# usnistgov/thermoextrap

Hardware: AMD Instinct MI355X
Metric: samples/s for order-4 comoment bootstrap (N_samp x N_obs x nrep resample_vals) (higher is better)
Workload: dtype f64; 1 GPU; north: central-comoment bootstrap, N_samp=1e+08, N_obs=32, order=4, nrep=1000, exact multinomial device sampler; n_samp=100000000, n_obs=32, order=4, nrep=1000, parallelism=state-points x1

## Files before the change

include/txmom.h:

```cpp
#ifndef TXMOM_H
#define TXMOM_H

#include <stddef.h>
#include <stdint.h>

#ifdef __cplusplus
extern "C" {
#endif

#define TXM_ABI_VERSION 2
#define TXM_MAX_ORDER 8
#define TXM_SAMPLER_STREAM_VERSION 3

typedef enum txm_status {
  TXM_OK = 0,
  TXM_ERR_INVALID = -1,
  TXM_ERR_HIP = -2,
  TXM_ERR_WORKSPACE = -3,
  TXM_ERR_UNSUPPORTED = -4,
  TXM_ERR_NO_DEVICE = -5
} txm_status;

typedef void *txm_stream;

int txm_abi_version(void);
int txm_sampler_stream_version(void);
const char *txm_csrc_sha(void);
const char *txm_last_error(void);
int txm_init(int device);
int txm_device_count(int *count_host);
int txm_malloc(void **ptr_host, size_t bytes);
int txm_free(void *ptr);
int txm_memcpy_h2d(void *dst, const void *src_host, size_t bytes, txm_stream stream);
int txm_memcpy_d2h(void *dst_host, const void *src, size_t bytes, txm_stream stream);
int txm_memset(void *dst, int value, size_t bytes, txm_stream stream);
int txm_stream_sync(txm_stream stream);

size_t txm_reduce_vals_ws_bytes(int64_t N, int64_t C, int order);
int txm_reduce_vals(const double *x, int64_t ldx_s, int64_t ldx_c, const double *u,
                    const double *w, int64_t N, int64_t C, int order, double *out, void *ws,
                    size_t ws_bytes, txm_stream stream);

int txm_reduce_vals_pivot(const double *x, int64_t ldx_s, int64_t ldx_c, const double *u, int64_t N, int64_t C,
                          double *pivot, txm_stream stream);
int txm_reduce_vals_sums(const double *x, int64_t ldx_s, int64_t ldx_c, const double *u, const double *w,
                         int64_t N, int64_t C, int order, const double *pivot, double *sums, void *ws,
                         size_t ws_bytes, txm_stream stream);
int txm_sums_to_state(const double *sums, int64_t n, const double *pivot, int64_t C, int order, double *out,
                      txm_stream stream);
size_t txm_push_vals_ws_bytes(int64_t N, int64_t C, int order);
int txm_push_vals(double *state, const double *x, int64_t ldx_s, int64_t ldx_c, const double *u, const double *w,
                  int64_t N, int64_t C, int order, void *ws, size_t ws_bytes, txm_stream stream);

size_t txm_reduce_vals_1d_ws_bytes(int64_t N, int64_t R, int M);
int txm_reduce_vals_1d(const double *u, int64_t ldu_r, int64_t ldu_s, const double *w,
                       int64_t N, int64_t R, int M, double *out, void *ws, size_t ws_bytes,
                       txm_stream stream);

size_t txm_indices_to_freq_ws_bytes(void);
int txm_indices_to_freq(const int64_t *indices, int64_t nrep, int64_t nsamp, int64_t ndat,
                        int64_t *freq, void *ws, size_t ws_bytes, txm_stream stream);

typedef struct txm_sampler_spec {
  uint64_t seed;
  int64_t nrep;
  int64_t ndat;
  int64_t nsamp;
  int64_t rep0;
} txm_sampler_spec;

int64_t txm_sampler_ntiles(int64_t ndat);
size_t txm_sampler_counts_ws_bytes(const txm_sampler_spec *spec_host);
int txm_sampler_tile_counts(const txm_sampler_spec *spec_host, uint32_t *counts, void *ws,
                            size_t ws_bytes, txm_stream stream);
int txm_sampler_freq(const txm_sampler_spec *spec_host, const uint32_t *counts, int64_t *freq,
                     txm_stream stream);

size_t txm_sampler_count_table_bytes(int64_t ndat, int64_t nreps);
int txm_sampler_count_table(const txm_sampler_spec *spec_host, const uint32_t *counts, int64_t rep_begin,
                            int64_t nreps, uint8_t *table, txm_stream stream);

#define TXM_PATH_AUTO (-1)
#define TXM_PATH_FP64 0
#define TXM_PATH_INT8 1
#define TXM_PATH_INT8_FUSED 2
#define TXM_PATH_INT8_TABLE 3
typedef struct txm_resample_opts {
  int32_t path;
  int32_t prep_valid;
  void *prep;
  size_t prep_bytes;
  int64_t *info;
  const double *y;
  int64_t ldy_s;
  double *out_y;
} txm_resample_opts;
int txm_resample_path(int64_t N, int64_t C, int64_t nrep, int order);
#define TXM_KERNEL_WITH_Y 0x100
int txm_resample_kernel(int64_t N, int64_t C, int64_t nrep, int order, int path, int has_y, int aligned);
int txm_resample_operands_aligned(const double *x, int64_t ldx_s, int64_t C, const double *y, int64_t ldy_s);
int txm_set_resample_path(int path);
int txm_resample_vals_info(const void *ws, int64_t N, int64_t C, int64_t nrep, int order,
                           int64_t *info_host, txm_stream stream);
size_t txm_resample_prep_bytes(int64_t N, int64_t C, int64_t nrep, int order);
size_t txm_resample_vals_ws_bytes(int64_t N, int64_t C, int64_t nrep, int order);
size_t txm_resample_vals_ws_bytes_opts(int64_t N, int64_t C, int64_t nrep, int order, int path, int has_y);
size_t txm_resample_y_ws_bytes(int64_t N, int64_t C, int64_t nrep);
int txm_resample_i8_supported(int64_t N, int64_t C, int64_t nrep, int order);
int txm_resample_vals(const double *x, int64_t ldx_s, int64_t ldx_c, const double *u,
                      const double *w, int64_t N, int64_t C, int order, int64_t nrep,
                      const int64_t *freq, const txm_sampler_spec *spec_host,
                      const uint32_t *counts, const double *pivot, double *out,
                      const txm_resample_opts *opts_host, void *ws, size_t ws_bytes, txm_stream stream);

typedef struct txm_state_ptrs {
  const double *x;
  const double *u;
  const double *w;
} txm_state_ptrs;
size_t txm_reduce_vals_batched_ws_bytes(int64_t S, int64_t N, int64_t C, int order);
int txm_reduce_vals_batched(const txm_state_ptrs *states_host, int64_t S, int64_t ldx_s, int64_t N,
                            int64_t C, int order, double *out, void *ws, size_t ws_bytes,
                            txm_stream stream);
size_t txm_resample_vals_batched_ws_bytes(int64_t S, int64_t N, int64_t C, int64_t nrep, int order);
int txm_resample_vals_batched(const txm_state_ptrs *states_host, int64_t S, int64_t ldx_s, int64_t N,
                              int64_t C, int order, int64_t nrep, const int64_t *freq,
                              const txm_sampler_spec *spec_host, const uint32_t *counts, double *out,
                              void *ws, size_t ws_bytes, txm_stream stream);
size_t txm_resample_batched_prep_bytes(int64_t S, int64_t N, int64_t C, int64_t nrep, int order);
int txm_resample_batched_path(int64_t S, int64_t N, int64_t C, int64_t nrep, int order);
int txm_resample_vals_batched_opts(const txm_state_ptrs *states_host, int64_t S, int64_t ldx_s, int64_t N,
                                   int64_t C, int order, int64_t nrep, const int64_t *freq,
                                   const txm_sampler_spec *spec_host, const uint32_t *counts, double *out,
                                   const txm_resample_opts *opts_host, void *ws, size_t ws_bytes, txm_stream stream);

size_t txm_resample_data_ws_bytes(int64_t nrec, int64_t C, int order);
int txm_resample_data(const double *data, const int64_t *freq, int64_t nrec, int64_t C,
                      int64_t nrep, int order, double *out, void *ws, size_t ws_bytes,
                      txm_stream stream);

int txm_convert_cov(const double *in, double *out, int64_t n, int order, int to_central,
                    txm_stream stream);
int txm_convert_1d(const double *in, double *out, int64_t n, int M, int to_central,
                   txm_stream stream);

typedef struct txm_atom {
  int32_t src;
  int32_t pad;
  int64_t offset;
  int64_t s_rep;
  int64_t s_val;
} txm_atom;

#define TXM_FUNC_PLAIN 0
#define TXM_FUNC_MINUS_LOG 1

typedef struct txm_poly_table {
  int32_t n_funcs;
  int32_t n_atoms;
  int32_t n_terms;
  int32_t n_factors;
  int32_t log_atom;
  int32_t pad;
  const txm_atom *atoms;
  const int32_t *func_term0;
  const int32_t *func_flags;
  const double *coef;
  const int32_t *term_fac0;
  const int32_t *fac_atom;
  const int32_t *fac_pow;
} txm_poly_table;

int txm_eval_poly(const txm_poly_table *table_host, const double *const *srcs, int32_t n_srcs,
                  int64_t nrep, int64_t nval, double *out, txm_stream stream);

#define TXM_TAYLOR_SUM 0
#define TXM_TAYLOR_CUMSUM 1
#define TXM_TAYLOR_TERMS 2
int txm_predict_taylor(const double *derivs, int32_t n_ord, int64_t M, const double *dalpha,
                       int64_t n_alpha, int32_t mode, double *out, txm_stream stream);

int txm_cov_over_rep(const double *vals, int32_t n_ord, int64_t nrep, int64_t nval, double *cov,
                     txm_stream stream);

size_t txm_perturb_ws_bytes(int64_t N, int64_t C, int32_t n_alpha, int64_t nrep);
int txm_perturb(const double *x, int64_t ldx_s, const double *u, int64_t N, int64_t C,
                const double *dalpha_host, int32_t n_alpha, const int64_t *freq, int64_t nrep,
                double *out, void *ws, size_t ws_bytes, txm_stream stream);

typedef struct txm_mbar_state {
  const double *x;
  const double *u;
  int64_t n;
  int64_t ldx_s;
} txm_mbar_state;
size_t txm_mbar_ws_bytes(int32_t K, int64_t C, int32_t n_alpha);
int txm_mbar_eval(const txm_mbar_state *states_host, int32_t K, const double *alpha0_host,
                  const double *g_host, double upiv, double *out, double *logD, void *ws,
                  size_t ws_bytes, txm_stream stream);
int txm_mbar_predict(const txm_mbar_state *states_host, int32_t K, int64_t C, double upiv,
                     const double *logD, const double *alpha_host, int32_t n_alpha, double *out,
                     void *ws, size_t ws_bytes, txm_stream stream);

#ifdef __cplusplus
}
#endif
#endif
```

thermoextrap_amd/csrc/txm_resample.hip:

```cpp
#include <type_traits>

#include <stdlib.h>

#include "txm_sampler.h"
#include "txm_pivot.h"
#include "txm_resample_i8.h"
#include "txm_i8g.h"

namespace txm {

typedef double v4f64 __attribute__((ext_vector_type(4)));

constexpr int RS_BLOCK = 256;
constexpr int RS_WAVES = RS_BLOCK / 64;
constexpr int RS_REPS = 16;
constexpr int RS_QUARTER = SM_T / 4;
constexpr int RS_TILE_BYTES = SM_T * RS_REPS;
constexpr int rs_group(int K, int NBLK, bool weighted, bool explicit_, int pack = 1) {
  const int per_step = 2 + 2 * NBLK + (weighted ? 2 : 0) + (explicit_ ? 10 : 0);
  for (int g = 8; g > 2; g >>= 1)
#ifndef TXM_EXP_BUDGET
#define TXM_EXP_BUDGET 160
#endif
    if ((K + pack - 1) / pack * NBLK * 8 + 2 * g * per_step <= TXM_EXP_BUDGET) return g;
// ... 383 lines not shown
  if (colgrp == 0) {
    if constexpr (!WEIGHTED && !EXPLICIT) usum[0] = cnt;
#pragma unroll
    for (int j = 0; j < K; ++j) {
      double v = usum[j];
      v += __shfl_xor(v, 16);
      v += __shfl_xor(v, 32);
      if (kk == 0) PU[((size_t)chunk * a.nrep_pad + rep0 + row) * K + j] = v;
    }
  }
}

template <int K>
__global__ __launch_bounds__(256) void resample_finalize_kernel(
    const double *__restrict__ part_x, const double *__restrict__ part_u, int n_chunks,
    int64_t nrep_pad, int64_t C_pad, int64_t nrep, int64_t C, const double *__restrict__ pivot,
    double *__restrict__ out, int64_t c_off = 0, int64_t C_total = 0) {
  constexpr int NSEG = 8, NOUT = 256 / NSEG;
  __shared__ double sh[NSEG][NOUT][2 * K];
  const int eo = threadIdx.x % NOUT, seg = threadIdx.x / NOUT;
  const int64_t e = (int64_t)blockIdx.x * NOUT + eo;
  const bool live = e < nrep * C;
  const int64_t r = live ? e / C : 0, c = live ? e % C : 0;
  if (C_total == 0) C_total = C;
  const int64_t sidx = blockIdx.y;
  part_x += (size_t)sidx * n_chunks * nrep_pad * C_pad * K;
  part_u += (size_t)sidx * n_chunks * nrep_pad * K;
  pivot += sidx * (1 + C);
  out += (size_t)sidx * nrep * C_total * 2 * K;
  double S0[K], S1[K];
#pragma unroll
  for (int j = 0; j < K; ++j) S0[j] = S1[j] = 0.0;
  if (live)
    for (int ch = seg; ch < n_chunks; ch += NSEG) {
      const double *pu_ = part_u + ((size_t)ch * nrep_pad + r) * K;
      const double *px_ = part_x + (((size_t)ch * nrep_pad + r) * C_pad + c) * K;
#pragma unroll
      for (int j = 0; j < K; ++j) {
        S0[j] += pu_[j];
        S1[j] += px_[j];
      }
    }
#pragma unroll
  for (int j = 0; j < K; ++j) {
    sh[seg][eo][j] = S0[j];
    sh[seg][eo][K + j] = S1[j];
  }
  __syncthreads();
  if (seg != 0 || !live) return;
  for (int g = 1; g < NSEG; ++g)
#pragma unroll
    for (int j = 0; j < K; ++j) {
      S0[j] += sh[g][eo][j];
      S1[j] += sh[g][eo][K + j];
    }
  double st[2 * K];
  pivot_sums_to_state<K>(S0, S1, pivot[0], pivot[1 + c_off + c], st);
  double *o = out + (r * C_total + c_off + c) * 2 * K;
#pragma unroll
  for (int q = 0; q < 2 * K; ++q) o[q] = st[q];
}

template <int K, int CPAD>
__global__ __launch_bounds__(256) void resample_finalize_i8_kernel(
    const double *__restrict__ part_x, const double *__restrict__ part_u, int64_t nwin,
    const uint32_t *__restrict__ wflag, int64_t nrep_pad, int64_t nrep, int64_t C,
    const double *__restrict__ pivot, double *__restrict__ out, int64_t c_off, int64_t C_total,
    const double *__restrict__ fb_x, const double *__restrict__ fb_u, int fb_chunks, int64_t fb_cpad,
    const uint32_t *__restrict__ n_list, const I8State *__restrict__ states = nullptr, const int summed = 0) {
  if (states != nullptr) {
    const I8State e = states[blockIdx.y];
    part_x = e.part_x; part_u = e.part_u; wflag = e.wflag; pivot = e.pivot; out = e.out;
    fb_x = e.fb_x; fb_u = e.fb_u; n_list = e.n_list;
  }
  constexpr int cpad = CPAD;
  __shared__ double sh[256][2 * K];
  constexpr int nseg = 256 / cpad;
  const int64_t r = blockIdx.x;
  const int c = threadIdx.x % cpad, seg = threadIdx.x / cpad;
  double S0[K], S1[K];
#pragma unroll
  for (int j = 0; j < K; ++j) S0[j] = S1[j] = 0.0;
  if (c < C) {
    for (int64_t w = seg; w < nwin; w += nseg) {
      if (wflag[w] != 0u) continue;
      if (summed) {
        const double *px_ = part_x + ((size_t)w * nrep_pad + r) * K * cpad + c;
        if (summed == 1) {
          const double *pu_ = part_u + ((size_t)w * nrep_pad + r) * K;
#pragma unroll
          for (int j = 0; j < K; ++j) {
            S0[j] += pu_[j];
            S1[j] += px_[j * cpad];
          }
        } else {
          const double *pu_ = part_u + ((size_t)w * nrep_pad + r) * K * 8;
#pragma unroll
          for (int j = 0; j < K; ++j) {
            const double4 ua = *reinterpret_cast<const double4 *>(pu_ + j * 8), ub = *reinterpret_cast<const double4 *>(pu_ + j * 8 + 4);
            S0[j] += ((((((ua.x + ua.y) + ua.z) + ua.w) + ub.x) + ub.y) + ub.z);
            S1[j] += px_[j * cpad];
          }
        }
        continue;
      }
      const double *pu_ = part_u + ((size_t)w * nrep_pad + r) * K * 8;
      const double *px_ = part_x + ((size_t)w * nrep_pad + r) * K * 8 * cpad + c;
#pragma unroll
      for (int j = 0; j < K; ++j) {
        const double4 ua = *reinterpret_cast<const double4 *>(pu_ + j * 8), ub = *reinterpret_cast<const double4 *>(pu_ + j * 8 + 4);
        const double *q = px_ + (size_t)j * 8 * cpad;
        S0[j] += ((((((ua.x + ua.y) + ua.z) + ua.w) + ub.x) + ub.y) + ub.z);
        S1[j] += ((((((q[0] + q[cpad]) + q[2 * cpad]) + q[3 * cpad]) + q[4 * cpad]) + q[5 * cpad]) + q[6 * cpad]);
      }
    }
  }
#pragma unroll
  for (int j = 0; j < K; ++j) {
    sh[threadIdx.x][j] = S0[j];
    sh[threadIdx.x][K + j] = S1[j];
  }
  __syncthreads();
  if (seg != 0 || c >= C) return;
  for (int g = 1; g < nseg; ++g)
#pragma unroll
    for (int j = 0; j < K; ++j) {
      S0[j] += sh[g * cpad + c][j];
      S1[j] += sh[g * cpad + c][K + j];
    }
  if (n_list[0] != 0u)
    for (int ch = 0; ch < fb_chunks; ++ch) {
      const double *pu_ = fb_u + ((size_t)ch * nrep_pad + r) * K;
      const double *px_ = fb_x + (((size_t)ch * nrep_pad + r) * fb_cpad + c) * K;
#pragma unroll
      for (int j = 0; j < K; ++j) {
        S0[j] += pu_[j];
        S1[j] += px_[j];
      }
    }
  double st[2 * K];
  pivot_sums_to_state<K>(S0, S1, pivot[0], pivot[1 + c_off + c], st);
  double *o = out + (r * C_total + c_off + c) * 2 * K;
#pragma unroll
  for (int q = 0; q < 2 * K; ++q) o[q] = st[q];
  (void)nrep;
}

__global__ __launch_bounds__(256) void resample_finalize_y_kernel(
    const double *__restrict__ part_y, const double *__restrict__ part_u, int K, int64_t nwin,
    const uint32_t *__restrict__ wflag, int64_t nrep_pad, int64_t C, const double *__restrict__ ypivot,
    double *__restrict__ out_y, int64_t c_off, int64_t C_total, const double *__restrict__ fb_y,
    const double *__restrict__ fb_u, int fb_chunks, int64_t fb_cpad, const uint32_t *__restrict__ n_list) {
  constexpr int NSEG = 8;
  __shared__ double sh[NSEG][32][2];
  const int64_t r = blockIdx.x;
  const int c = threadIdx.x & 31, seg = threadIdx.x >> 5;
  double S0 = 0.0, S1 = 0.0;
  if (c < C) {
    for (int64_t w = seg; w < nwin; w += NSEG) {
      if (wflag[w] != 0u) continue;
      const double *pu_ = part_u + ((size_t)w * nrep_pad + r) * K * 8;
      const double *q = part_y + ((size_t)w * nrep_pad + r) * 8 * I8_CPAD + c;
      const double4 ua = *reinterpret_cast<const double4 *>(pu_), ub = *reinterpret_cast<const double4 *>(pu_ + 4);
      S0 += ((((((ua.x + ua.y) + ua.z) + ua.w) + ub.x) + ub.y) + ub.z);
      S1 += ((((((q[0] + q[I8_CPAD]) + q[2 * I8_CPAD]) + q[3 * I8_CPAD]) + q[4 * I8_CPAD]) + q[5 * I8_CPAD]) + q[6 * I8_CPAD]);
    }
  }
  sh[seg][c][0] = S0;
  sh[seg][c][1] = S1;
  __syncthreads();
  if (seg != 0 || c >= C) return;
  S0 = sh[0][c][0];
  S1 = sh[0][c][1];
  for (int g = 1; g < NSEG; ++g) {
    S0 += sh[g][c][0];
    S1 += sh[g][c][1];
  }
  if (n_list[0] != 0u)
    for (int ch = 0; ch < fb_chunks; ++ch) {
      S0 += fb_u[((size_t)ch * nrep_pad + r) * K];
      S1 += fb_y[((size_t)ch * nrep_pad + r) * fb_cpad + c];
    }
  out_y[r * C_total + c_off + c] = ypivot[1 + c_off + c] + S1 * (1.0 / S0);
}

struct ResamplePlan {
  int nblk, colgroups, n_rbg, n_chunks;
  int64_t tiles_per_chunk, nrep_pad, C_pad, ntiles;
  size_t off_pivot, off_px, off_pu, off_prog, prog_bytes, total;
};

static int64_t resample_chunk_tiles(int64_t ntiles, int64_t div) {
  int64_t nc = ntiles / div;
  if (nc > 1024) nc = 1024;
  if (nc < 8) nc = 8;
  if (nc > ntiles) nc = ntiles;
  nc = cdiv(nc, 8) * 8;
  return cdiv(ntiles, nc);
}

static ResamplePlan plan_resample(int64_t N, int64_t C, int64_t nrep, int K) {
  ResamplePlan p;
  p.nblk = C <= 16 ? 1 : 2;
  p.colgroups = (int)cdiv(C, p.nblk * 16);
  p.C_pad = (int64_t)p.colgroups * p.nblk * 16;
  p.n_rbg = (int)cdiv(nrep, RS_WAVES * RS_REPS);
  p.nrep_pad = (int64_t)p.n_rbg * RS_WAVES * RS_REPS;
  p.ntiles = cdiv(N, SM_T);
  p.tiles_per_chunk = resample_chunk_tiles(p.ntiles, 2);
  const int64_t nc = cdiv(cdiv(p.ntiles, p.tiles_per_chunk), 8) * 8;
  p.n_chunks = (int)nc;
  p.off_pivot = 0;
  p.off_px = align_up((size_t)(1 + C) * sizeof(double), 256);
  p.off_pu = p.off_px + align_up((size_t)p.n_chunks * p.nrep_pad * p.C_pad * K * sizeof(double), 256);
  p.off_prog = p.off_pu + align_up((size_t)p.n_chunks * p.nrep_pad * K * sizeof(double), 256);
  p.prog_bytes = (size_t)p.n_chunks * p.colgroups * 64 * sizeof(uint32_t);
  p.total = p.off_prog + align_up(p.prog_bytes, 256);
  return p;
}

struct I8Plan {
  int n_rbg, n_chunks, ngroups;
  int64_t tiles_per_chunk, nrep_pad, ntiles, nwin, win_tiles;
  size_t off_px, off_pu, total;
  int sub_tiles;
  size_t off_fbx, off_fbu, off_prog, prog_bytes, off_stats, off_prep;
  size_t off_table, table_bytes, off_gprog, total_table;
  size_t off_py, off_fby, prep_ypiv, prep_ywt, prep_yflag;
  size_t prep_wt, prep_flag, prep_list, prep_nlist, prep_group0, prep_group_stride, prep_total;
  ResamplePlan fb;
};

static I8Plan plan_i8(int64_t N, int64_t C, int64_t nrep, int K) {
  I8Plan p;
  p.n_rbg = (int)cdiv(nrep, I8_REPS);
  p.nrep_pad = (int64_t)p.n_rbg * I8_REPS;
  p.ntiles = cdiv(N, SM_T);
  p.ngroups = (int)cdiv(C, I8_CPAD);
  p.win_tiles = I8_WIN_TILES;
#ifndef TXM_WIN_MIN
#define TXM_WIN_MIN 256
#endif
  while (p.win_tiles > 4 && p.ntiles < TXM_WIN_MIN * p.win_tiles) p.win_tiles /= 4;
  p.nwin = cdiv(p.ntiles, p.win_tiles);
  int64_t nc = (int64_t)num_cus() / p.n_rbg / 8 * 8;
  if (nc < 8) nc = 8;
  if (nc > p.nwin) nc = cdiv(p.nwin, 8) * 8;
  p.tiles_per_chunk = cdiv(p.nwin, nc) * p.win_tiles;
  p.n_chunks = (int)(cdiv(cdiv(p.ntiles, p.tiles_per_chunk), 8) * 8);
  p.sub_tiles = p.win_tiles < I8_SUB_TILES ? (int)p.win_tiles : I8_SUB_TILES;
  p.prep_wt = 0;
  p.prep_flag = p.prep_wt + align_up((size_t)p.nwin * I8_WT_STRIDE * sizeof(double) + 2048, 256);
  p.prep_list = p.prep_flag + align_up((size_t)p.nwin * sizeof(uint32_t), 256);
  p.prep_nlist = p.prep_list + align_up((size_t)p.nwin * (size_t)(p.win_tiles / p.sub_tiles) * sizeof(uint32_t), 256);
  p.prep_ywt = p.prep_nlist + 256;
  p.prep_yflag = p.prep_ywt + align_up((size_t)p.nwin * I8_WT_STRIDE * sizeof(double), 256);
  p.prep_group_stride = p.prep_yflag + align_up((size_t)p.nwin * sizeof(uint32_t), 256);
  p.prep_ypiv = align_up((size_t)(1 + C) * sizeof(double), 256);
  p.prep_group0 = 2 * p.prep_ypiv;
  p.prep_total = p.prep_group0 + (size_t)p.ngroups * p.prep_group_stride;
  p.off_px = 0;
  p.off_pu = p.off_px + align_up((size_t)p.nwin * p.nrep_pad * K * I8_CPAD * 8 * sizeof(double), 256);
  p.fb = plan_resample(N, C < I8_CPAD ? C : I8_CPAD, nrep, K);
  p.off_fbx = p.off_pu + align_up((size_t)p.nwin * p.nrep_pad * K * 8 * sizeof(double), 256);
  p.off_fbu = p.off_fbx + align_up((size_t)p.fb.n_chunks * p.fb.nrep_pad * p.fb.C_pad * K * sizeof(double), 256);
  p.off_prog = p.off_fbu + align_up((size_t)p.fb.n_chunks * p.fb.nrep_pad * (K + 1) * sizeof(double), 256);
  p.prog_bytes = (size_t)p.n_chunks * 64 * sizeof(uint32_t);
  p.off_stats = p.off_prog + align_up(p.prog_bytes, 256);
  p.off_py = p.off_stats + align_up((size_t)cdiv(p.ntiles, p.win_tiles < 16 ? p.win_tiles : 16) * 100 * sizeof(double), 256);
  p.off_fby = p.off_py + align_up((size_t)p.nwin * p.nrep_pad * 8 * I8_CPAD * sizeof(double), 256);
  p.off_prep = p.off_fby + align_up((size_t)p.fb.n_chunks * p.fb.nrep_pad * p.fb.C_pad * sizeof(double), 256);
  p.off_gprog = p.off_prep + align_up(p.prep_total, 256);
  p.off_table = p.off_gprog + align_up((size_t)cdiv(p.nwin, 8) * 8 * 16 * sizeof(uint32_t), 256);
  p.table_bytes = (N >= SM_T && (C > 16 || K >= 2)) ? count_table_bytes(p.ntiles, nrep) : 0;
  p.total = p.off_table;
  p.total_table = p.off_table + align_up(p.table_bytes, 256);
  return p;
}

static int g_path_override = -1;
static int path_override() { return g_path_override; }

static constexpr bool throttle_on() {
#ifdef TXM_NO_THROTTLE
  return false;
#else
  return true;
#endif
}

static bool table_kernel_pays(int64_t nrep, int K, bool has_y) {
  const int64_t pad128 = cdiv(nrep, G_REPS) * G_REPS, pad64 = cdiv(nrep, I8_REPS) * I8_REPS;
  if (4 * pad128 > 5 * pad64) return false;
  if (has_y) return true;
  if (K == 4 || K == 5) return pad128 >= 2 * G_REPS;
  return true;
}

static bool narrow_table_pays(int64_t N, int64_t C, int64_t nrep, int K) {
  const int64_t pad128 = cdiv(nrep, G_REPS) * G_REPS, pad64 = cdiv(nrep, I8_REPS) * I8_REPS;
  if (N < 786432 || nrep <= I8_REPS || pad128 > pad64) return false;
  return !(i8t_narrow_nq(C, K) == 4 && K == 5);
}
static bool table_call_rule(size_t table_bytes, int eff, int64_t N, int64_t C, int64_t nrep, int K, bool has_y, bool applicable) {
  if (eff == TXM_PATH_FP64 || eff == TXM_PATH_INT8_FUSED || table_bytes == 0 || !applicable) return false;
  if (eff == TXM_PATH_INT8_TABLE) return true;
  return C > 16 ? table_kernel_pays(nrep, K, has_y) : narrow_table_pays(N, C, nrep, K);
}
static bool table_operands_ok(const double *x, int64_t ldx_s, int64_t C, int K, const double *y, int64_t ldy_s) {
  return C > 16 ? i8g_applicable(x, ldx_s, C, y, ldy_s) : i8gn_applicable(x, ldx_s, C, K);
}

static bool use_i8(int64_t N, int64_t C, int64_t nrep, int K, int call_path = TXM_PATH_AUTO) {
  if (!i8_supported(N, C, nrep, K)) return false;
  const int ov = call_path != TXM_PATH_AUTO ? call_path : path_override();
  if (ov == TXM_PATH_FP64) return false;
  if (ov == TXM_PATH_INT8 || ov == TXM_PATH_INT8_FUSED || ov == TXM_PATH_INT8_TABLE) return true;
  if (C <= 16) return K >= 2 && (N >= 786432 || (N >= 262144 && nrep >= 128));
  const int64_t ctail = C % I8_CPAD;
  const bool long_series = N >= 786432;
  const int64_t min_rep = long_series ? (K >= 2 ? 32 : 100) : (K >= 4 ? 64 : (K >= 2 ? 128 : 384));
  return C > 16 && (ctail == 0 || ctail > 16 || K >= 2) && nrep >= min_rep && N >= 262144;
}

}

using namespace txm;

extern "C" int txm_set_resample_path(int path) {
  TXM_REQUIRE(path == -1 || path == TXM_PATH_FP64 || path == TXM_PATH_INT8 || path == TXM_PATH_INT8_FUSED || path == TXM_PATH_INT8_TABLE, "set_resample_path: %d is not a path", path);
  g_path_override = path;
  return TXM_OK;
}

namespace txm {
__global__ void i8_info_kernel(const unsigned char *prep_groups, size_t group_stride, size_t off_nlist, int ngroups,
                               int64_t nwin, int from_prep, int64_t *info) {
  if (threadIdx.x == 0 && blockIdx.x == 0) {
    int64_t flagged = 0;
    for (int g = 0; g < ngroups; ++g)
      flagged += reinterpret_cast<const uint32_t *>(prep_groups + (size_t)g * group_stride + off_nlist)[1];
    info[0] = TXM_PATH_INT8;
    info[1] = nwin * ngroups;
    info[2] = flagged;
    info[3] = from_prep;
  }
}
__global__ void fp64_info_kernel(int64_t *info) {
  if (threadIdx.x == 0 && blockIdx.x == 0) {
    info[0] = TXM_PATH_FP64;
    info[1] = info[2] = info[3] = 0;
  }
}
}
using namespace txm;

extern "C" int txm_resample_vals_info(const void *ws, int64_t N, int64_t C, int64_t nrep, int order,
                                      int64_t *info_host, txm_stream stream) {
  TXM_REQUIRE(ws && info_host, "resample_vals_info: null pointer");
  TXM_REQUIRE(N >= 1 && C >= 1 && nrep >= 1 && order >= 0 && order <= TXM_MAX_ORDER, "resample_vals_info: bad shape");
  info_host[0] = TXM_PATH_FP64;
  info_host[1] = info_host[2] = 0;
  if (!use_i8(N, C, nrep, order + 1)) return TXM_OK;
  const I8Plan q = plan_i8(N, C, nrep, order + 1);
  int64_t flagged = 0;
  for (int g = 0; g < q.ngroups; ++g) {
    uint32_t nl[2] = {0, 0};
    TXM_HIP(hipMemcpyAsync(nl, (const char *)ws + q.off_prep + q.prep_group0 + (size_t)g * q.prep_group_stride + q.prep_nlist,
                           sizeof(nl), hipMemcpyDeviceToHost, (hipStream_t)stream));
    TXM_HIP(hipStreamSynchronize((hipStream_t)stream));
    flagged += nl[1];
  }
  info_host[0] = TXM_PATH_INT8;
  info_host[1] = q.nwin * q.ngroups;
  info_host[2] = flagged;
  return TXM_OK;
}

extern "C" int txm_resample_path(int64_t N, int64_t C, int64_t nrep, int order) {
  if (N < 1 || C < 1 || nrep < 1 || order < 0 || order > TXM_MAX_ORDER) return TXM_PATH_FP64;
  return use_i8(N, C, nrep, order + 1) ? TXM_PATH_INT8 : TXM_PATH_FP64;
}

extern "C" int txm_resample_kernel(int64_t N, int64_t C, int64_t nrep, int order, int path, int has_y, int aligned) {
  if (N < 1 || C < 1 || nrep < 1 || order < 0 || order > TXM_MAX_ORDER) return TXM_PATH_FP64;
  const int K = order + 1;
  if (!use_i8(N, C, nrep, K, path)) return TXM_PATH_FP64;
  const I8Plan q = plan_i8(N, C, nrep, K);
  const int eff = path != TXM_PATH_AUTO ? path : path_override();
  const bool table = table_call_rule(q.table_bytes, eff, N, C, nrep, K, has_y != 0, aligned != 0);
  const bool with_y = has_y != 0 && ((table && C > 16) || i8t_carries_y(C, K));
  return (table ? TXM_PATH_INT8_TABLE : TXM_PATH_INT8_FUSED) | (with_y ? TXM_KERNEL_WITH_Y : 0);
}

extern "C" int txm_resample_operands_aligned(const double *x, int64_t ldx_s, int64_t C, const double *y, int64_t ldy_s) {
  if (x == nullptr || C < 1) return 0;
  return table_operands_ok(x, ldx_s, C, 2, y, ldy_s) ? 1 : 0;
}

extern "C" size_t txm_resample_prep_bytes(int64_t N, int64_t C, int64_t nrep, int order) {
  if (N < 1 || C < 1 || nrep < 1 || order < 0 || order > TXM_MAX_ORDER) return 0;
  if (!i8_supported(N, C, nrep, order + 1)) return 256;
  return plan_i8(N, C, nrep, order + 1).prep_total;
}

static size_t y_main_bytes(int64_t N, int64_t C, int64_t nrep) {
  size_t n = plan_resample(N, C, nrep, 1).total;
  if (i8_supported(N, C, nrep, 1)) {
    const size_t m = plan_i8(N, C, nrep, 1).total;
    if (m > n) n = m;
  }
  return align_up(n, 256);
}
static size_t y_extra_bytes(int64_t N, int64_t C, int64_t nrep) {
  return align_up((size_t)nrep * C * 2 * sizeof(double), 256) + y_main_bytes(N, C, nrep);
}

extern "C" size_t txm_resample_vals_ws_bytes_opts(int64_t N, int64_t C, int64_t nrep, int order, int path, int has_y) {
  if (N < 1 || C < 1 || nrep < 1 || order < 0 || order > TXM_MAX_ORDER) return 0;
  size_t n = plan_resample(N, C, nrep, order + 1).total;
  if (i8_supported(N, C, nrep, order + 1)) {
    const I8Plan q = plan_i8(N, C, nrep, order + 1);
    const int eff = path != TXM_PATH_AUTO ? path : path_override();
    const bool table = table_call_rule(q.table_bytes, eff, N, C, nrep, order + 1, has_y != 0, true);
    const size_t m = table ? q.total_table : q.total;
    if (m > n) n = m;
  }
  return align_up(n, 256);
}

extern "C" size_t txm_resample_vals_ws_bytes(int64_t N, int64_t C, int64_t nrep, int order) {
  return txm_resample_vals_ws_bytes_opts(N, C, nrep, order, TXM_PATH_AUTO, 0);
}

extern "C" size_t txm_resample_y_ws_bytes(int64_t N, int64_t C, int64_t nrep) {
  if (N < 1 || C < 1 || nrep < 1) return 0;
  return y_extra_bytes(N, C, nrep);
}

extern "C" int txm_resample_i8_supported(int64_t N, int64_t C, int64_t nrep, int order) {
  if (N < 1 || C < 1 || nrep < 1 || order < 0 || order > TXM_MAX_ORDER) return 0;
  return i8_supported(N, C, nrep, order + 1) ? 1 : 0;
}

#define TXM_K_SWITCH(K_, CALL)                          \
  switch (K_) {                                         \
    case 1: { constexpr int KK = 1; CALL; } break;      \
    case 2: { constexpr int KK = 2; CALL; } break;      \
    case 3: { constexpr int KK = 3; CALL; } break;      \
    case 4: { constexpr int KK = 4; CALL; } break;      \
    case 5: { constexpr int KK = 5; CALL; } break;      \
    case 6: { constexpr int KK = 6; CALL; } break;      \
    case 7: { constexpr int KK = 7; CALL; } break;      \
    case 8: { constexpr int KK = 8; CALL; } break;      \
    case 9: { constexpr int KK = 9; CALL; } break;      \
    default: set_error("order out of range"); return TXM_ERR_INVALID; \
  }

namespace txm {
static constexpr bool pack_on() {
#ifdef TXM_NO_PACK
  return false;
#else
  return true;
#endif
}
template <int K>
static int run_resample(ResampleArgs a, const ResamplePlan &p, bool weighted, bool explicit_,
                        double *out, hipStream_t st, int64_t S = 1) {
  dim3 grid((unsigned)(p.n_chunks * p.n_rbg), (unsigned)p.colgroups, (unsigned)S), block(RS_BLOCK);
  const size_t lds = explicit_ ? 0 : (size_t)RS_WAVES * RS_TILE_BYTES;
#define TXM_RS_LAUNCH(NB, WT, EX)                                                                       \
  do {                                                                                                 \
    if (S > 1 || a.batch != nullptr) {                                                                 \
      if (a.N < SM_T)                                                                                  \
        hipLaunchKernelGGL((resample_kernel<K, NB, WT, EX, true, RS_BATCHED>), grid, block, lds, st, a);  \
      else                                                                                             \
        hipLaunchKernelGGL((resample_kernel<K, NB, WT, EX, false, RS_BATCHED>), grid, block, lds, st, a); \
    } else if (a.N < SM_T)                                                                             \
      hipLaunchKernelGGL((resample_kernel<K, NB, WT, EX, true>), grid, block, lds, st, a);             \
    else                                                                                               \
      hipLaunchKernelGGL((resample_kernel<K, NB, WT, EX, false>), grid, block, lds, st, a);            \
  } while (0)
  bool packed = false;
  if constexpr (K >= 2 && K <= 6) {
    if (p.nblk == 1 && p.colgroups == 1 && !explicit_ && a.N >= SM_T && a.C <= 8 && pack_on()) {
      packed = true;
      const bool bat = S > 1 || a.batch != nullptr;
#define TXM_RS_PACKED(PK)                                                                                      \
  do {                                                                                                         \
    if (bat) {                                                                                                 \
      if (weighted) hipLaunchKernelGGL((resample_kernel<K, 1, true, false, false, RS_BATCHED, PK>), grid, block, lds, st, a); \
      else hipLaunchKernelGGL((resample_kernel<K, 1, false, false, false, RS_BATCHED, PK>), grid, block, lds, st, a);         \
    } else {                                                                                                   \
      if (weighted) hipLaunchKernelGGL((resample_kernel<K, 1, true, false, false, RS_PLAIN, PK>), grid, block, lds, st, a);   \
      else hipLaunchKernelGGL((resample_kernel<K, 1, false, false, false, RS_PLAIN, PK>), grid, block, lds, st, a);           \
    }                                                                                                          \
  } while (0)
      if (a.C <= 4 && K >= 3) TXM_RS_PACKED(4);
      else TXM_RS_PACKED(2);
#undef TXM_RS_PACKED
    }
  }
  if (packed) {
  } else if (p.nblk == 1) {
    if (weighted) { if (explicit_) TXM_RS_LAUNCH(1, true, true); else TXM_RS_LAUNCH(1, true, false); }
    else          { if (explicit_) TXM_RS_LAUNCH(1, false, true); else TXM_RS_LAUNCH(1, false, false); }
  } else {
    if (weighted) { if (explicit_) TXM_RS_LAUNCH(2, true, true); else TXM_RS_LAUNCH(2, true, false); }
    else          { if (explicit_) TXM_RS_LAUNCH(2, false, true); else TXM_RS_LAUNCH(2, false, false); }
  }
#undef TXM_RS_LAUNCH
  TXM_LAUNCH_CHECK();
  const int64_t ne = a.nrep * a.C;
  hipLaunchKernelGGL((resample_finalize_kernel<K>), dim3((unsigned)cdiv(ne, 32), (unsigned)S), dim3(256), 0, st,
                     a.part_x, a.part_u, p.n_chunks, p.nrep_pad, p.C_pad, a.nrep, a.C, a.pivot, out);
  TXM_LAUNCH_CHECK();
  return TXM_OK;
}

template <int K>
static int run_listed_k(const ResampleArgs &a, const ResamplePlan &p, bool weighted, hipStream_t st, int64_t S = 1) {
  dim3 grid((unsigned)(p.n_chunks * p.n_rbg), (unsigned)p.colgroups, (unsigned)S), block(RS_BLOCK);
  const size_t lds = (size_t)RS_WAVES * RS_TILE_BYTES;
  if (p.nblk == 1) {
    if (weighted) hipLaunchKernelGGL((resample_kernel<K, 1, true, false, false, RS_LISTED>), grid, block, lds, st, a);
    else hipLaunchKernelGGL((resample_kernel<K, 1, false, false, false, RS_LISTED>), grid, block, lds, st, a);
  } else {
    if (weighted) hipLaunchKernelGGL((resample_kernel<K, 2, true, false, false, RS_LISTED>), grid, block, lds, st, a);
    else hipLaunchKernelGGL((resample_kernel<K, 2, false, false, false, RS_LISTED>), grid, block, lds, st, a);
  }
  TXM_LAUNCH_CHECK();
  return TXM_OK;
}

static int run_listed(const ResampleArgs &a, const ResamplePlan &p0, int K, bool weighted, hipStream_t st, int64_t S = 1) {
  ResamplePlan p = p0;
  if (a.C <= 16) p.nblk = 1;
  p.colgroups = 1;
  TXM_K_SWITCH(K, return run_listed_k<KK>(a, p, weighted, st, S));
  return TXM_OK;
}
}

namespace txm {
__global__ void y_means_kernel(const double *__restrict__ st , int64_t n, double *__restrict__ out) {
  const int64_t e = (int64_t)blockIdx.x * blockDim.x + threadIdx.x;
  if (e < n) out[e] = st[2 * e + 1];
}

static int resample_vals_impl(const double *x, int64_t ldx_s, const double *u, const double *w, int64_t N, int64_t C,
                              int order, int64_t nrep, const int64_t *freq, const txm_sampler_spec *spec,
                              const uint32_t *counts, const double *pivot, double *out, int path, void *prep,
                              size_t prep_bytes, bool prep_valid, int64_t *info, void *ws, size_t ws_bytes,
                              hipStream_t st, const double *y = nullptr, int64_t ldy_s = 0, double *out_y = nullptr,
                              bool *y_done = nullptr) {
  const bool explicit_ = freq != nullptr;
  const int K = order + 1;
  if (y_done) *y_done = false;
  if (!explicit_ && use_i8(N, C, nrep, K, path)) {
    const I8Plan q = plan_i8(N, C, nrep, K);
    const int eff_path = path != TXM_PATH_AUTO ? path : path_override();
    const bool table_call = ws_bytes >= q.total_table &&
                            table_call_rule(q.table_bytes, eff_path, N, C, nrep, K, y != nullptr, table_operands_ok(x, ldx_s, C, K, y, ldy_s));
    const bool with_y = y != nullptr && ((table_call && C > 16) || i8t_carries_y(C, K));
    if (ws_bytes < q.total) {
      set_error("resample_vals: workspace too small (%zu < %zu)", ws_bytes, q.total);
      return TXM_ERR_WORKSPACE;
    }
    TXM_REQUIRE(spec->ndat == N && spec->nrep == nrep, "resample_vals: sampler spec does not match N/nrep");
    TXM_REQUIRE(spec->rep0 >= 0 && spec->rep0 + nrep <= ((int64_t)1 << 32), "resample_vals: sampler rep0 out of range");
    unsigned char *pb = (unsigned char *)ws + q.off_prep;
    bool have_tables = false;
    if (prep != nullptr) {
      if (prep_bytes < q.prep_total) {
        set_error("resample_vals: prep buffer too small (%zu < %zu)", prep_bytes, q.prep_total);
        return TXM_ERR_WORKSPACE;
      }
      pb = (unsigned char *)prep;
      have_tables = prep_valid;
    }
    double *piv = (double *)pb;
    double *ypiv = (double *)(pb + q.prep_ypiv);
    if (!have_tables) {
      if (pivot) {
        TXM_HIP(hipMemcpyAsync(piv, pivot, sizeof(double) * (size_t)(1 + C), hipMemcpyDeviceToDevice, st));
      } else {
        hipLaunchKernelGGL(pivot_kernel, dim3((unsigned)(1 + C)), dim3(256), 0, st, x, ldx_s, (int64_t)1,
                           u, (int64_t)1, N, piv);
        TXM_LAUNCH_CHECK();
      }
      if (with_y) {
        hipLaunchKernelGGL(pivot_kernel, dim3((unsigned)(1 + C)), dim3(256), 0, st, y, ldy_s, (int64_t)1, u, (int64_t)1,
                           N, ypiv);
        TXM_LAUNCH_CHECK();
        TXM_HIP(hipMemcpyAsync(ypiv, piv, sizeof(double), hipMemcpyDeviceToDevice, st));
      }
    }
    I8Args b;
    b.x = x; b.ldx_s = ldx_s; b.u = u; b.w = w; b.N = N; b.nrep = nrep; b.C_call = C;
    b.cpad = i8_cpad(C, K);
    b.counts = counts;
    b.k0 = (uint32_t)spec->seed;
    b.k1 = (uint32_t)(spec->seed >> 32);
    b.rep_base = (uint32_t)spec->rep0;
    b.ntiles = q.ntiles;
    b.last_tile_size = (uint32_t)(N - (q.ntiles - 1) * SM_T);
    b.pivot = piv;
    b.stats = (double *)((char *)ws + q.off_stats);
    b.nwin = q.nwin;
    b.part_x = (double *)((char *)ws + q.off_px);
    b.part_u = (double *)((char *)ws + q.off_pu);
    b.n_chunks = q.n_chunks; b.n_rbg = q.n_rbg; b.tiles_per_chunk = q.tiles_per_chunk;
    b.nrep_pad = q.nrep_pad;
    b.win_tiles = q.win_tiles;
    b.sub_tiles = q.sub_tiles;
    b.y = with_y ? y : nullptr;
    b.ldy_s = ldy_s;
    b.ypivot = ypiv;
    b.part_y = (double *)((char *)ws + q.off_py);
    b.part_summed = i8t_wide_summed(with_y) ? 1 : 0;
    b.progress = (throttle_on() && q.n_rbg > 1) ? (uint32_t *)((char *)ws + q.off_prog) : nullptr;
    ResampleArgs f;
    f.ldx_s = ldx_s; f.u = u; f.w = w; f.N = N; f.nrep = nrep;
    f.freq = nullptr; f.counts = counts;
    f.k0 = b.k0; f.k1 = b.k1; f.rep_base = b.rep_base;
    f.ntiles = q.ntiles; f.last_tile_size = b.last_tile_size;
    f.pivot = piv;
    f.part_x = (double *)((char *)ws + q.off_fbx);
    f.part_u = (double *)((char *)ws + q.off_fbu);
    f.n_chunks = q.fb.n_chunks; f.n_rbg = q.fb.n_rbg; f.tiles_per_chunk = q.fb.tiles_per_chunk;
    f.nrep_pad = q.fb.nrep_pad; f.C_pad = q.fb.C_pad;
    f.sub_tiles = q.sub_tiles; f.batch = nullptr; f.progress = nullptr;
    TXM_REQUIRE(q.fb.nrep_pad == q.nrep_pad, "resample_vals: replicate padding of the two kernels differs");
    int g = 0;
    bool have_table = false;
    for (int64_t col0 = 0; col0 < C; col0 += I8_CPAD, ++g) {
      unsigned char *pg = pb + q.prep_group0 + (size_t)g * q.prep_group_stride;
      b.wtab = (double *)(pg + q.prep_wt);
      b.wflag = (uint32_t *)(pg + q.prep_flag);
      b.list = (uint32_t *)(pg + q.prep_list);
      b.n_list = (uint32_t *)(pg + q.prep_nlist);
      b.ywtab = (double *)(pg + q.prep_ywt);
      b.yflag = (uint32_t *)(pg + q.prep_yflag);
      f.list = b.list; f.n_list = b.n_list;
      b.col0 = col0;
      b.C = C - col0 < I8_CPAD ? C - col0 : I8_CPAD;
      const bool narrow_tail = C > I8_CPAD && b.C <= 16 && K >= 2 && !with_y;
      b.C_call = narrow_tail ? b.C : C;
      b.cpad = i8_cpad(b.C_call, K);
      if (!have_tables) {
        const int rc0 = launch_i8_prepass(b, K, st);
        if (rc0 != TXM_OK) return rc0;
      }
      const bool table_kernel = table_call && !narrow_tail;
      int rc;
      if (table_kernel) {
        unsigned char *table = (unsigned char *)ws + q.off_table;
        if (!have_table) {
          rc = launch_count_table(counts, nrep, N, b.k0, b.k1, b.rep_base, 0, cdiv(nrep, G_REPS), table, st);
          if (rc != TXM_OK) return rc;
          have_table = true;
        }
        I8Args bg = b;
        bg.progress = (throttle_on() && nrep > G_REPS) ? (uint32_t *)((char *)ws + q.off_gprog) : nullptr;
        rc = C > 16 ? launch_resample_i8g(bg, K, w != nullptr, table, 0, (int)cdiv(nrep, G_REPS), st)
                    : launch_resample_i8gn(bg, K, w != nullptr, table, 0, (int)cdiv(nrep, G_REPS), 0, st);
      } else {
        rc = launch_resample_i8(b, K, w != nullptr, q.prog_bytes, st);
      }
      if (rc != TXM_OK) return rc;
      f.x = x + col0; f.C = b.C; f.col_off = col0;
      {
        const int rc2 = run_listed(f, q.fb, K, w != nullptr, st);
        if (rc2 != TXM_OK) return rc2;
      }
      const int fin_summed = table_kernel ? (C <= 16 ? 1 : 2)
                                          : (i8t_narrow_nq(b.C_call, K) != 0 ? (i8t_partials_summed(b.C_call, K) ? 1 : 0) : b.part_summed);
#define TXM_I8_FIN2(KK, CP)                                                                            \
  hipLaunchKernelGGL((resample_finalize_i8_kernel<KK, CP>), dim3((unsigned)nrep), dim3(256), 0, st,      \
                     b.part_x, b.part_u, q.nwin, b.wflag, q.nrep_pad, nrep, b.C, piv, out, col0, C,        \
                     f.part_x, f.part_u, q.fb.n_chunks, q.fb.C_pad, b.n_list, (const I8State *)nullptr, fin_summed)
#define TXM_I8_FIN(KK)                                                                                 \
  do {                                                                                                 \
    if (b.cpad == 32) TXM_I8_FIN2(KK, 32);                                                             \
    else if (b.cpad == 16) TXM_I8_FIN2(KK, 16);                                                        \
    else if (b.cpad == 8) TXM_I8_FIN2(KK, 8);                                                          \
    else TXM_I8_FIN2(KK, 4);                                                                           \
  } while (0)
      switch (K) {
        case 1: TXM_I8_FIN(1); break;
        case 2: TXM_I8_FIN(2); break;
        case 3: TXM_I8_FIN(3); break;
        case 4: TXM_I8_FIN(4); break;
        case 5: TXM_I8_FIN(5); break;
        case 6: TXM_I8_FIN(6); break;
        case 7: TXM_I8_FIN(7); break;
        default: TXM_I8_FIN(8); break;
      }
#undef TXM_I8_FIN
      TXM_LAUNCH_CHECK();
      if (with_y) {
        ResampleArgs fy = f;
        fy.x = y + col0; fy.ldx_s = ldy_s; fy.pivot = ypiv;
        fy.part_x = (double *)((char *)ws + q.off_fby);
        fy.part_u = f.part_u + (size_t)q.fb.n_chunks * q.fb.nrep_pad * K;
        const int rc3 = run_listed(fy, q.fb, 1, w != nullptr, st);
        if (rc3 != TXM_OK) return rc3;
        hipLaunchKernelGGL(resample_finalize_y_kernel, dim3((unsigned)nrep), dim3(256), 0, st, b.part_y, b.part_u, K, q.nwin,
                           b.wflag, q.nrep_pad, b.C, ypiv, out_y, col0, C, fy.part_x, f.part_u, q.fb.n_chunks, q.fb.C_pad,
                           b.n_list);
        TXM_LAUNCH_CHECK();
      }
    }
    if (with_y && y_done) *y_done = true;
    if (prep != nullptr)
      TXM_HIP(hipMemcpyAsync((char *)ws + q.off_prep, pb, q.prep_total, hipMemcpyDeviceToDevice, st));
    if (info != nullptr) {
      hipLaunchKernelGGL(i8_info_kernel, dim3(1), dim3(64), 0, st, pb + q.prep_group0, q.prep_group_stride, q.prep_nlist,
                         q.ngroups, q.nwin, (have_tables ? 1 : 0) | (have_table ? 2 : 0), info);
      TXM_LAUNCH_CHECK();
    }
    return TXM_OK;
  }
  if (info != nullptr) {
    hipLaunchKernelGGL(fp64_info_kernel, dim3(1), dim3(64), 0, st, info);
    TXM_LAUNCH_CHECK();
  }
  const ResamplePlan p = plan_resample(N, C, nrep, K);
  if (ws_bytes < p.total) {
    set_error("resample_vals: workspace too small (%zu < %zu)", ws_bytes, p.total);
    return TXM_ERR_WORKSPACE;
  }
  TXM_REQUIRE((int64_t)p.n_chunks * p.n_rbg < ((int64_t)1 << 31), "resample_vals: grid too large");
  double *piv = (double *)((char *)ws + p.off_pivot);
  if (pivot) {
    TXM_HIP(hipMemcpyAsync(piv, pivot, sizeof(double) * (size_t)(1 + C), hipMemcpyDeviceToDevice, st));
  } else {
    hipLaunchKernelGGL(pivot_kernel, dim3((unsigned)(1 + C)), dim3(256), 0, st, x, ldx_s, (int64_t)1,
                       u, (int64_t)1, N, piv);
    TXM_LAUNCH_CHECK();
  }
  ResampleArgs a;
  a.x = x; a.ldx_s = ldx_s; a.u = u; a.w = w; a.N = N; a.C = C; a.nrep = nrep;
  a.freq = freq; a.counts = counts;
  a.k0 = a.k1 = 0;
  a.rep_base = 0;
  a.ntiles = p.ntiles;
  a.last_tile_size = (uint32_t)(N - (p.ntiles - 1) * SM_T);
  if (!explicit_) {
    TXM_REQUIRE(spec->ndat == N && spec->nrep == nrep, "resample_vals: sampler spec does not match N/nrep");
    TXM_REQUIRE(spec->rep0 >= 0 && spec->rep0 + nrep <= ((int64_t)1 << 32), "resample_vals: sampler rep0 out of range");
    a.k0 = (uint32_t)spec->seed;
    a.k1 = (uint32_t)(spec->seed >> 32);
    a.rep_base = (uint32_t)spec->rep0;
  }
  a.pivot = piv;
  a.part_x = (double *)((char *)ws + p.off_px);
  a.part_u = (double *)((char *)ws + p.off_pu);
  a.n_chunks = p.n_chunks; a.n_rbg = p.n_rbg; a.tiles_per_chunk = p.tiles_per_chunk;
  a.nrep_pad = p.nrep_pad; a.C_pad = p.C_pad;
  a.list = nullptr; a.n_list = nullptr; a.sub_tiles = 0; a.col_off = 0; a.batch = nullptr;
  a.progress = nullptr;
  if (throttle_on() && p.n_rbg > 1 && a.N >= SM_T) {
    a.progress = (uint32_t *)((char *)ws + p.off_prog);
    TXM_HIP(hipMemsetAsync(a.progress, 0, p.prog_bytes, st));
  }
  TXM_K_SWITCH(K, return run_resample<KK>(a, p, w != nullptr, explicit_, out, st));
  return TXM_OK;
}
}

extern "C" int txm_resample_vals(const double *x, int64_t ldx_s, int64_t ldx_c, const double *u,
                                 const double *w, int64_t N, int64_t C, int order, int64_t nrep,
                                 const int64_t *freq, const txm_sampler_spec *spec,
                                 const uint32_t *counts, const double *pivot, double *out,
                                 const txm_resample_opts *opts, void *ws, size_t ws_bytes, txm_stream stream) {
  TXM_REQUIRE(x && u && out && ws, "resample_vals: null pointer");
  TXM_REQUIRE(N >= 1 && C >= 1 && nrep >= 1, "resample_vals: need N, C, nrep >= 1");
  TXM_REQUIRE(order >= 0 && order <= TXM_MAX_ORDER, "resample_vals: order %d outside [0, %d]", order,
              TXM_MAX_ORDER);
  TXM_REQUIRE(ldx_c == 1 && ldx_s >= C, "resample_vals: x must be (rec, val) row-major (ldx_c == 1)");
  const bool explicit_ = freq != nullptr;
  TXM_REQUIRE(explicit_ != (spec != nullptr && counts != nullptr),
              "resample_vals: give either freq or (spec, counts)");
  txm_resample_opts o;
  o.path = TXM_PATH_AUTO; o.prep_valid = 0; o.prep = nullptr; o.prep_bytes = 0; o.info = nullptr;
  o.y = nullptr; o.ldy_s = 0; o.out_y = nullptr;
  if (opts) o = *opts;
  TXM_REQUIRE(o.path == TXM_PATH_AUTO || o.path == TXM_PATH_FP64 || o.path == TXM_PATH_INT8 || o.path == TXM_PATH_INT8_FUSED || o.path == TXM_PATH_INT8_TABLE,
              "resample_vals: opts.path %d is not a path", (int)o.path);
  TXM_REQUIRE((o.y == nullptr) == (o.out_y == nullptr), "resample_vals: opts.y and opts.out_y go together");
  TXM_REQUIRE(o.y == nullptr || o.ldy_s >= C, "resample_vals: opts.ldy_s < C");
  hipStream_t st = (hipStream_t)stream;
  const size_t main_bytes = txm_resample_vals_ws_bytes_opts(N, C, nrep, order, o.path, o.y != nullptr);
  const size_t avail = ws_bytes < main_bytes ? ws_bytes : main_bytes;
  bool y_done = false;
  int rc = resample_vals_impl(x, ldx_s, u, w, N, C, order, nrep, freq, spec, counts, pivot, out, o.path, o.prep,
                              o.prep_bytes, o.prep_valid != 0, o.info, ws, avail, st, o.y, o.ldy_s, o.out_y, &y_done);
  if (rc != TXM_OK || o.y == nullptr || y_done) return rc;
  if (ws_bytes < main_bytes + y_extra_bytes(N, C, nrep)) {
    set_error("resample_vals: workspace too small for opts.y (%zu < %zu)", ws_bytes, main_bytes + y_extra_bytes(N, C, nrep));
    return TXM_ERR_WORKSPACE;
  }
  double *ystates = (double *)((char *)ws + main_bytes);
  void *yws = (char *)ws + main_bytes + align_up((size_t)nrep * C * 2 * sizeof(double), 256);
  rc = resample_vals_impl(o.y, o.ldy_s, u, w, N, C, 0, nrep, freq, spec, counts, nullptr, ystates, o.path, nullptr, 0,
                          false, nullptr, yws, y_main_bytes(N, C, nrep), st);
  if (rc != TXM_OK) return rc;
  hipLaunchKernelGGL(y_means_kernel, dim3((unsigned)cdiv(nrep * C, 256)), dim3(256), 0, st, ystates, nrep * C, o.out_y);
  TXM_LAUNCH_CHECK();
  return TXM_OK;
}

namespace txm {
struct BatchPlan {
  ResamplePlan one;
  size_t off_tab, off_pivot, off_px, off_pu, total;
};
static BatchPlan plan_batched(int64_t S, int64_t N, int64_t C, int64_t nrep, int K) {
  BatchPlan b;
  ResamplePlan &p = b.one;
  p = plan_resample(N, C, nrep, K);
  (void)S;
  p.tiles_per_chunk = resample_chunk_tiles(p.ntiles, 8);
  p.n_chunks = (int)(cdiv(cdiv(p.ntiles, p.tiles_per_chunk), 8) * 8);
  b.off_tab = 0;
  b.off_pivot = align_up((size_t)S * sizeof(txm_state_ptrs), 256);
  b.off_px = b.off_pivot + align_up((size_t)S * (1 + C) * sizeof(double), 256);
  b.off_pu = b.off_px + align_up((size_t)S * p.n_chunks * p.nrep_pad * p.C_pad * K * sizeof(double), 256);
  b.total = b.off_pu + align_up((size_t)S * p.n_chunks * p.nrep_pad * K * sizeof(double), 256);
  return b;
}
}

namespace txm {
struct I8StateLayout {
  size_t stride, s_px, s_pu, s_fbx, s_fbu, s_stats;
  size_t p_stride, p_wt, p_flag, p_list, p_nlist;
};
struct BatchI8Plan {
  I8Plan q;
  int cpad, n_chunks;
  int64_t tiles_per_chunk;
  I8StateLayout L;
  size_t off_tab, off_states, off_bargs, off_state0, off_prep, total;
  size_t prep_piv, prep_state0, prep_total;
};
static BatchI8Plan plan_batched_i8(int64_t S, int64_t N, int64_t C, int64_t nrep, int K) {
  BatchI8Plan b;
  b.q = plan_i8(N, C, nrep, K);
  const I8Plan &q = b.q;
  b.cpad = i8_cpad(C, K);
  int64_t nc = (int64_t)num_cus() / ((int64_t)q.n_rbg * S) / 8 * 8;
  if (nc < 8) nc = 8;
  if (nc > q.nwin) nc = cdiv(q.nwin, 8) * 8;
  b.tiles_per_chunk = cdiv(q.nwin, nc) * q.win_tiles;
  b.n_chunks = (int)(cdiv(cdiv(q.ntiles, b.tiles_per_chunk), 8) * 8);
  I8StateLayout &L = b.L;
  L.s_px = 0;
  L.s_pu = L.s_px + align_up((size_t)q.nwin * q.nrep_pad * K * 8 * b.cpad * sizeof(double), 256);
  L.s_fbx = L.s_pu + align_up((size_t)q.nwin * q.nrep_pad * K * 8 * sizeof(double), 256);
  L.s_fbu = L.s_fbx + align_up((size_t)q.fb.n_chunks * q.fb.nrep_pad * q.fb.C_pad * K * sizeof(double), 256);
  L.s_stats = L.s_fbu + align_up((size_t)q.fb.n_chunks * q.fb.nrep_pad * (K + 1) * sizeof(double), 256);
  L.stride = L.s_stats + align_up((size_t)cdiv(q.ntiles, q.win_tiles < 16 ? q.win_tiles : 16) * 100 * sizeof(double), 256);
  L.p_wt = 0;
  L.p_flag = L.p_wt + align_up((size_t)q.nwin * I8_WT_STRIDE * sizeof(double) + 2048, 256);
  L.p_list = L.p_flag + align_up((size_t)q.nwin * sizeof(uint32_t), 256);
  L.p_nlist = L.p_list + align_up((size_t)q.nwin * (size_t)(q.win_tiles / q.sub_tiles) * sizeof(uint32_t), 256);
  L.p_stride = L.p_nlist + 256;
  b.prep_piv = 0;
  b.prep_state0 = align_up((size_t)S * (1 + C) * sizeof(double), 256);
  b.prep_total = b.prep_state0 + (size_t)S * L.p_stride;
  b.off_tab = 0;
  b.off_states = align_up((size_t)S * sizeof(txm_state_ptrs), 256);
  b.off_bargs = b.off_states + align_up((size_t)S * sizeof(I8State), 256);
  b.off_state0 = b.off_bargs + align_up((size_t)S * sizeof(I8Args), 256);
  b.off_prep = b.off_state0 + (size_t)S * L.stride;
  b.total = b.off_prep + align_up(b.prep_total, 256);
  return b;
}

static bool use_i8_batched(int64_t S, int64_t N, int64_t C, int64_t nrep, int K, int call_path = TXM_PATH_AUTO) {
  if (!i8_supported(N, C, nrep, K) || i8t_narrow_nq(C, K) == 0) return false;
  const int ov = call_path != TXM_PATH_AUTO ? call_path : path_override();
  if (ov == TXM_PATH_FP64) return false;
  if (ov == TXM_PATH_INT8 || ov == TXM_PATH_INT8_FUSED || ov == TXM_PATH_INT8_TABLE) return true;
  (void)S;
  return K >= 2 && (N >= 786432 || (N >= 262144 && nrep >= 128));
}

__global__ void i8_states_kernel(const txm_state_ptrs *__restrict__ tab, int64_t S, unsigned char *base, unsigned char *pbase,
                                 I8StateLayout L, const double *piv, int64_t C, const uint32_t *counts, int64_t nrep, int64_t ntiles,
                                 double *out, int K, uint32_t rep_base, I8State *__restrict__ states) {
  const int64_t s = (int64_t)blockIdx.x * blockDim.x + threadIdx.x;
  if (s >= S) return;
  unsigned char *b = base + (size_t)s * L.stride, *pb = pbase + (size_t)s * L.p_stride;
  I8State e;
  e.x = tab[s].x; e.u = tab[s].u; e.w = tab[s].w;
  e.pivot = piv + s * (1 + C);
  e.stats = (double *)(b + L.s_stats);
  e.wtab = (double *)(pb + L.p_wt);
  e.wflag = (uint32_t *)(pb + L.p_flag);
  e.list = (uint32_t *)(pb + L.p_list);
  e.n_list = (uint32_t *)(pb + L.p_nlist);
  e.part_x = (double *)(b + L.s_px);
  e.part_u = (double *)(b + L.s_pu);
  e.fb_x = (double *)(b + L.s_fbx);
  e.fb_u = (double *)(b + L.s_fbu);
  e.counts = counts + (size_t)s * nrep * ntiles;
  e.out = out + (size_t)s * nrep * C * 2 * K;
  e.rep_base = rep_base + (uint32_t)(s * nrep);
  e.pad_ = 0;
  states[s] = e;
}

__global__ void i8_batch_args_kernel(const I8Args base, int64_t S, I8Args *__restrict__ out) {
  const int64_t s = (int64_t)blockIdx.x * blockDim.x + threadIdx.x;
  if (s >= S) return;
  const I8State e = base.states[s];
  I8Args r = base;
  r.x = e.x; r.u = e.u; r.w = e.w; r.pivot = e.pivot; r.wtab = e.wtab; r.wflag = e.wflag;
  r.part_x = e.part_x; r.part_u = e.part_u; r.counts = e.counts; r.rep_base = e.rep_base;
  out[s] = r;
}

static int resample_batched_i8(const txm_state_ptrs *states_host, int64_t S, int64_t ldx_s, int64_t N, int64_t C, int K,
                               int64_t nrep, bool weighted, const txm_sampler_spec *spec, const uint32_t *counts, double *out,
                               void *prep, size_t prep_bytes, bool prep_valid, int64_t *info, void *ws, size_t ws_bytes,
                               hipStream_t st) {
  const BatchI8Plan b = plan_batched_i8(S, N, C, nrep, K);
  const I8Plan &q = b.q;
  if (ws_bytes < b.total) {
    set_error("resample_vals_batched: workspace too small (%zu < %zu)", ws_bytes, b.total);
    return TXM_ERR_WORKSPACE;
  }
  TXM_REQUIRE(spec->ndat == N && spec->nrep == S * nrep, "resample_vals_batched: the sampler must span S * nrep replicates of N samples");
  TXM_REQUIRE(spec->rep0 >= 0 && spec->rep0 + spec->nrep <= ((int64_t)1 << 32), "resample_vals_batched: sampler replicates outside [0, 2^32)");
  TXM_REQUIRE((int64_t)b.n_chunks * q.n_rbg < ((int64_t)1 << 31) && S <= 65535, "resample_vals_batched: grid too large");
  txm_state_ptrs *tab = (txm_state_ptrs *)((char *)ws + b.off_tab);
  TXM_HIP(hipMemcpyAsync(tab, states_host, (size_t)S * sizeof(txm_state_ptrs), hipMemcpyHostToDevice, st));
  unsigned char *pb = (unsigned char *)ws + b.off_prep;
  bool have_tables = false;
  if (prep != nullptr) {
    if (prep_bytes < b.prep_total) {
      set_error("resample_vals_batched: prep buffer too small (%zu < %zu)", prep_bytes, b.prep_total);
      return TXM_ERR_WORKSPACE;
    }
    pb = (unsigned char *)prep;
    have_tables = prep_valid;
  }
  double *piv = (double *)(pb + b.prep_piv);
  if (!have_tables) {
    hipLaunchKernelGGL(pivot_batch_kernel, dim3((unsigned)(1 + C), (unsigned)S), dim3(256), 0, st, tab, ldx_s, N, C, piv);
    TXM_LAUNCH_CHECK();
  }
  I8State *states = (I8State *)((char *)ws + b.off_states);
  hipLaunchKernelGGL(i8_states_kernel, dim3((unsigned)cdiv(S, 64)), dim3(64), 0, st, tab, S, (unsigned char *)ws + b.off_state0,
                     pb + b.prep_state0, b.L, piv, C, counts, nrep, q.ntiles, out, K, (uint32_t)spec->rep0, states);
  TXM_LAUNCH_CHECK();
  bool vec_ok = ldx_s % 2 == 0;
  for (int64_t s = 0; s < S; ++s) vec_ok = vec_ok && (reinterpret_cast<uintptr_t>(states_host[s].x) & 15) == 0;
  I8Args a;
  a.states = states;
  a.S = S;
  a.x = vec_ok ? states_host[0].x : reinterpret_cast<const double *>((uintptr_t)8);
  a.ldx_s = ldx_s; a.u = states_host[0].u; a.w = states_host[0].w; a.N = N; a.C = C; a.nrep = nrep;
  a.col0 = 0; a.C_call = C;
  a.part_summed = 1;
  a.counts = counts;
  a.k0 = (uint32_t)spec->seed;
  a.k1 = (uint32_t)(spec->seed >> 32);
  a.rep_base = (uint32_t)spec->rep0;
  a.ntiles = q.ntiles;
  a.last_tile_size = (uint32_t)(N - (q.ntiles - 1) * SM_T);
  a.pivot = piv; a.wtab = nullptr; a.stats = nullptr; a.nwin = q.nwin;
  a.part_x = nullptr; a.cpad = b.cpad; a.part_u = nullptr;
  a.y = nullptr; a.ldy_s = 0; a.ypivot = nullptr; a.ywtab = nullptr; a.yflag = nullptr; a.part_y = nullptr;
  a.n_chunks = b.n_chunks; a.n_rbg = q.n_rbg; a.tiles_per_chunk = b.tiles_per_chunk; a.win_tiles = q.win_tiles;
  a.nrep_pad = q.nrep_pad;
  a.wflag = nullptr; a.list = nullptr; a.n_list = nullptr; a.sub_tiles = q.sub_tiles;
  a.progress = nullptr;
  I8Args *bargs = (I8Args *)((char *)ws + b.off_bargs);
  hipLaunchKernelGGL(i8_batch_args_kernel, dim3((unsigned)cdiv(S, 64)), dim3(64), 0, st, a, S, bargs);
  TXM_LAUNCH_CHECK();
  a.batch_args = bargs;
  int rc = have_tables ? TXM_OK : launch_i8_prepass(a, K, st);
  if (rc != TXM_OK) return rc;
  rc = launch_resample_i8t(a, K, weighted, 0, st);
  if (rc != TXM_OK) return rc;
  ResampleArgs f;
  f.x = states_host[0].x; f.ldx_s = ldx_s; f.u = states_host[0].u; f.w = states_host[0].w; f.N = N; f.C = C; f.nrep = nrep;
  f.freq = nullptr; f.counts = counts;
  f.k0 = a.k0; f.k1 = a.k1; f.rep_base = a.rep_base;
  f.ntiles = q.ntiles; f.last_tile_size = a.last_tile_size;
  f.pivot = piv; f.part_x = nullptr; f.part_u = nullptr;
  f.n_chunks = q.fb.n_chunks; f.n_rbg = q.fb.n_rbg; f.tiles_per_chunk = q.fb.tiles_per_chunk;
  f.nrep_pad = q.fb.nrep_pad; f.C_pad = q.fb.C_pad;
  f.list = nullptr; f.n_list = nullptr; f.sub_tiles = q.sub_tiles; f.col_off = 0; f.batch = nullptr; f.progress = nullptr;
  f.i8states = states;
  TXM_REQUIRE(q.fb.nrep_pad == q.nrep_pad, "resample_vals_batched: replicate padding of the two kernels differs");
  rc = run_listed(f, q.fb, K, weighted, st, S);
  if (rc != TXM_OK) return rc;
  const int bfin_summed = i8t_partials_summed(C, K) ? 1 : 0;
#define TXM_I8_BFIN2(KK, CP)                                                                                        \
  hipLaunchKernelGGL((resample_finalize_i8_kernel<KK, CP>), dim3((unsigned)nrep, (unsigned)S), dim3(256), 0, st, nullptr, \
                     nullptr, q.nwin, nullptr, q.nrep_pad, nrep, C, nullptr, nullptr, (int64_t)0, C, nullptr, nullptr,      \
                     q.fb.n_chunks, q.fb.C_pad, nullptr, states, bfin_summed)
#define TXM_I8_BFIN(KK)                                  \
  do {                                                   \
    if (b.cpad == 16) TXM_I8_BFIN2(KK, 16);              \
    else if (b.cpad == 8) TXM_I8_BFIN2(KK, 8);           \
    else TXM_I8_BFIN2(KK, 4);                            \
  } while (0)
  switch (K) {
    case 2: TXM_I8_BFIN(2); break;
    case 3: TXM_I8_BFIN(3); break;
    case 4: TXM_I8_BFIN(4); break;
    case 5: TXM_I8_BFIN(5); break;
    case 6: TXM_I8_BFIN(6); break;
    case 7: TXM_I8_BFIN(7); break;
    default: TXM_I8_BFIN(8); break;
  }
#undef TXM_I8_BFIN
#undef TXM_I8_BFIN2
  TXM_LAUNCH_CHECK();
  if (info != nullptr) {
    hipLaunchKernelGGL(i8_info_kernel, dim3(1), dim3(64), 0, st, pb + b.prep_state0, b.L.p_stride, b.L.p_nlist, (int)S, q.nwin,
                       have_tables ? 1 : 0, info);
    TXM_LAUNCH_CHECK();
  }
  return TXM_OK;
}
}

extern "C" size_t txm_resample_vals_batched_ws_bytes(int64_t S, int64_t N, int64_t C, int64_t nrep, int order) {
  if (S < 1 || N < 1 || C < 1 || nrep < 1 || order < 0 || order > TXM_MAX_ORDER) return 0;
  const size_t f = plan_batched(S, N, C, nrep, order + 1).total;
  if (!i8_supported(N, C, nrep, order + 1) || i8t_narrow_nq(C, order + 1) == 0) return f;
  const size_t i = plan_batched_i8(S, N, C, nrep, order + 1).total;
  return i > f ? i : f;
}

extern "C" int txm_resample_batched_path(int64_t S, int64_t N, int64_t C, int64_t nrep, int order) {
  if (S < 1 || N < 1 || C < 1 || nrep < 1 || order < 0 || order > TXM_MAX_ORDER) return TXM_PATH_FP64;
  return use_i8_batched(S, N, C, nrep, order + 1) ? TXM_PATH_INT8 : TXM_PATH_FP64;
}

extern "C" size_t txm_resample_batched_prep_bytes(int64_t S, int64_t N, int64_t C, int64_t nrep, int order) {
  if (S < 1 || N < 1 || C < 1 || nrep < 1 || order < 0 || order > TXM_MAX_ORDER) return 0;
  if (!i8_supported(N, C, nrep, order + 1) || i8t_narrow_nq(C, order + 1) == 0) return 0;
  return plan_batched_i8(S, N, C, nrep, order + 1).prep_total;
}

extern "C" int txm_resample_vals_batched(const txm_state_ptrs *states_host, int64_t S, int64_t ldx_s, int64_t N,
                                         int64_t C, int order, int64_t nrep, const int64_t *freq,
                                         const txm_sampler_spec *spec, const uint32_t *counts, double *out,
                                         void *ws, size_t ws_bytes, txm_stream stream) {
  return txm_resample_vals_batched_opts(states_host, S, ldx_s, N, C, order, nrep, freq, spec, counts, out, nullptr, ws, ws_bytes,
                                        stream);
}

extern "C" int txm_resample_vals_batched_opts(const txm_state_ptrs *states_host, int64_t S, int64_t ldx_s, int64_t N,
                                              int64_t C, int order, int64_t nrep, const int64_t *freq,
                                              const txm_sampler_spec *spec, const uint32_t *counts, double *out,
                                              const txm_resample_opts *opts, void *ws, size_t ws_bytes, txm_stream stream) {
  const int call_path = opts ? opts->path : TXM_PATH_AUTO;
  TXM_REQUIRE(call_path == TXM_PATH_AUTO || call_path == TXM_PATH_FP64 || call_path == TXM_PATH_INT8 || call_path == TXM_PATH_INT8_FUSED || call_path == TXM_PATH_INT8_TABLE,
              "resample_vals_batched: opts.path %d is not a path", call_path);
  TXM_REQUIRE(!(opts && (opts->y || opts->out_y)), "resample_vals_batched: no second sample matrix on the batched entry");
  TXM_REQUIRE(states_host && out && ws, "resample_vals_batched: null pointer");
  TXM_REQUIRE(S >= 1 && S <= 65535 && N >= 1 && C >= 1 && nrep >= 1, "resample_vals_batched: need S, N, C, nrep >= 1");
  TXM_REQUIRE(order >= 0 && order <= TXM_MAX_ORDER, "resample_vals_batched: order %d outside [0, %d]", order, TXM_MAX_ORDER);
  TXM_REQUIRE(ldx_s >= C, "resample_vals_batched: row pitch ldx_s < C");
  const bool explicit_ = freq != nullptr;
  TXM_REQUIRE(explicit_ != (spec != nullptr && counts != nullptr), "resample_vals_batched: give either freq or (spec, counts)");
  const bool weighted = states_host[0].w != nullptr;
  for (int64_t s = 0; s < S; ++s) {
    TXM_REQUIRE(states_host[s].x && states_host[s].u, "resample_vals_batched: state %lld has a null pointer", (long long)s);
    TXM_REQUIRE((states_host[s].w != nullptr) == weighted, "resample_vals_batched: weights for all states or for none");
  }
  const int K = order + 1;
  if (!explicit_ && use_i8_batched(S, N, C, nrep, K, call_path))
    return resample_batched_i8(states_host, S, ldx_s, N, C, K, nrep, weighted, spec, counts, out, opts ? opts->prep : nullptr,
                               opts ? opts->prep_bytes : 0, opts && opts->prep_valid != 0, opts ? opts->info : nullptr, ws, ws_bytes,
                               (hipStream_t)stream);
  if (opts && opts->info != nullptr) {
    hipLaunchKernelGGL(fp64_info_kernel, dim3(1), dim3(64), 0, (hipStream_t)stream, opts->info);
    TXM_LAUNCH_CHECK();
  }
  const BatchPlan b = plan_batched(S, N, C, nrep, K);
  if (ws_bytes < b.total) {
    set_error("resample_vals_batched: workspace too small (%zu < %zu)", ws_bytes, b.total);
    return TXM_ERR_WORKSPACE;
  }
  hipStream_t st = (hipStream_t)stream;
  txm_state_ptrs *tab = (txm_state_ptrs *)((char *)ws + b.off_tab);
  TXM_HIP(hipMemcpyAsync(tab, states_host, (size_t)S * sizeof(txm_state_ptrs), hipMemcpyHostToDevice, st));
  double *piv = (double *)((char *)ws + b.off_pivot);
  hipLaunchKernelGGL(pivot_batch_kernel, dim3((unsigned)(1 + C), (unsigned)S), dim3(256), 0, st, tab, ldx_s, N, C, piv);
  TXM_LAUNCH_CHECK();
  const ResamplePlan &p = b.one;
  ResampleArgs a;
  a.x = nullptr; a.ldx_s = ldx_s; a.u = nullptr; a.w = nullptr; a.N = N; a.C = C; a.nrep = nrep;
  a.freq = freq; a.counts = counts;
  a.k0 = a.k1 = 0;
  a.rep_base = 0;
  a.ntiles = p.ntiles;
  a.last_tile_size = (uint32_t)(N - (p.ntiles - 1) * SM_T);
  if (!explicit_) {
    TXM_REQUIRE(spec->ndat == N && spec->nrep == S * nrep, "resample_vals_batched: the sampler must span S * nrep replicates of N samples");
    TXM_REQUIRE(spec->rep0 >= 0 && spec->rep0 + spec->nrep <= ((int64_t)1 << 32), "resample_vals_batched: sampler replicates outside [0, 2^32)");
    a.k0 = (uint32_t)spec->seed;
    a.k1 = (uint32_t)(spec->seed >> 32);
    a.rep_base = (uint32_t)spec->rep0;
  }
  a.pivot = piv;
  a.part_x = (double *)((char *)ws + b.off_px);
  a.part_u = (double *)((char *)ws + b.off_pu);
  a.n_chunks = p.n_chunks; a.n_rbg = p.n_rbg; a.tiles_per_chunk = p.tiles_per_chunk;
  a.nrep_pad = p.nrep_pad; a.C_pad = p.C_pad;
  a.list = nullptr; a.n_list = nullptr; a.sub_tiles = 0; a.col_off = 0;
  a.batch = tab;
  a.progress = nullptr;
  TXM_K_SWITCH(K, return run_resample<KK>(a, p, weighted, explicit_, out, st, S));
  return TXM_OK;
}
```

thermoextrap_amd/csrc/txm_resample_i8.h:

```cpp
#pragma once
#include "txm_common.h"

namespace txm {

constexpr int I8_REPS = 64;
constexpr int I8_NSL = 7;
constexpr int I8_WIN_TILES = 256;
constexpr int I8_CPAD = 32;
constexpr int I8_WT_STRIDE = 80;
constexpr int I8_SUB_TILES = 8;

constexpr double I8_GUARD = 275.0;

constexpr int I8_WT_INVDU = 0, I8_WT_INVW = 1, I8_WT_DSP = 2, I8_WT_SC = 12, I8_WT_DSC = 44;

struct I8State {
  const double *x, *u, *w;
  const double *pivot;
  double *stats;
  double *wtab;
  uint32_t *wflag;
  uint32_t *list, *n_list;
  double *part_x, *part_u;
  double *fb_x, *fb_u;
  const uint32_t *counts;
  double *out;
  uint32_t rep_base;
  uint32_t pad_;
};

struct I8Args;
struct I8Args {
  const I8State *states = nullptr;
  const I8Args *batch_args = nullptr;
  int64_t S = 1;
  const double *x;
  int64_t ldx_s;
  const double *u;
  const double *w;
  int64_t N, C, nrep;
  int64_t col0;
  int64_t C_call;
  const uint32_t *counts;
  uint32_t k0, k1;
  uint32_t rep_base;
  int64_t ntiles;
  uint32_t last_tile_size;
  const double *pivot;
  double *wtab;
  double *stats;
  int64_t nwin;
  double *part_x;
  int cpad;
  double *part_u;
  int part_summed;
  const double *y;
  int64_t ldy_s;
  const double *ypivot;
  double *ywtab;
  uint32_t *yflag;
  double *part_y;
  int n_chunks, n_rbg;
  int64_t tiles_per_chunk;
  int64_t win_tiles;
  int64_t nrep_pad;
  uint32_t *wflag;
  uint32_t *list;
  uint32_t *n_list;
  int sub_tiles;
  uint32_t *progress;
};
#ifndef TXM_I8_LEAD
#define TXM_I8_LEAD 2
#endif
constexpr uint32_t I8_LEAD = TXM_I8_LEAD;
constexpr int I8_THROTTLE_SPINS = 48;

bool i8_supported(int64_t N, int64_t C, int64_t nrep, int K);
int launch_i8_prepass(const I8Args &a, int K, hipStream_t st);
int launch_resample_i8(const I8Args &a, int K, bool weighted, size_t prog_bytes, hipStream_t st);
int launch_resample_i8t(const I8Args &a, int K, bool weighted, size_t prog_bytes, hipStream_t st);
bool i8t_carries_y(int64_t C, int K);
bool i8t_applicable(const double *x, int64_t ldx_s, int64_t C);
int i8t_narrow_nq(int64_t C_call, int K);
int i8_cpad(int64_t C_call, int K);
bool i8t_partials_summed(int64_t C_call, int K);
bool i8t_wide_summed(bool call_carries_y);

}
```

thermoextrap_amd/csrc/txm_resample_i8.hip:

```cpp
#include "txm_resample_i8.h"

#include <stdlib.h>
#include "txm_sampler.h"

namespace txm {

constexpr int I8_ST_MAXDU = 0, I8_ST_MAXW = 1, I8_ST_UMIN = 2, I8_ST_BADU = 3, I8_ST_MAXX = 4, I8_ST_GMIN = 36,
              I8_ST_BADX = 68, I8_ST_STRIDE = 100;
constexpr int I8_STAT_TILES = 16;

template <bool VEC2>
__global__ __launch_bounds__(256) void i8_stats_kernel(const double *__restrict__ x, int64_t ldx,
                                                       const double *__restrict__ u,
                                                       const double *__restrict__ w, int64_t N, int64_t C,
                                                       int64_t col0, int64_t sub_samples, int fine_groups,
                                                       const double *__restrict__ pivot, int J,
                                                       double *__restrict__ stats, const I8State *__restrict__ states) {
  if (states != nullptr) {
    const I8State e = states[blockIdx.y];
    x = e.x; u = e.u; w = e.w; pivot = e.pivot; stats = e.stats;
  }
  const int64_t sb = blockIdx.x;
  const int64_t i0 = sb * sub_samples;
  const int64_t i1 = (i0 + sub_samples < N) ? i0 + sub_samples : N;
  const int tid = threadIdx.x, cp = tid & 15, r = tid >> 4;
  const int cpw = C > 16 ? 16 : C > 8 ? 8 : C > 4 ? 4 : C > 2 ? 2 : 1, nsubq = 16 / cpw;
  const int cpa = cp % cpw, qsub = cp / cpw;
  __shared__ double shq[4][2][256];
  __shared__ int shqn[4][256];
  __shared__ double shx[2][256], shg[2][256], shu[256], shw[256], shs[256];
  __shared__ int shn[256];
  __shared__ int badx[32], badu;
  if (tid < 32) badx[tid] = 0;
  if (tid == 0) badu = 0;
  __syncthreads();
  const double pu = pivot[0];
  const double kInf = __longlong_as_double(0x7ff0000000000000ll);
  double mx[2] = {0.0, 0.0}, gmin[2] = {kInf, kInf}, mu = 0.0, mw = 0.0;
  bool bx[2] = {false, false}, bu = false;
  const int c0 = 2 * cpa;
  const int slot = r * 16 + cpa;
#pragma unroll
  for (int g = 0; g < 4; ++g) {
    shq[g][0][tid] = shq[g][1][tid] = 0.0;
    shqn[g][tid] = 0;
  }
  __syncthreads();
  if (c0 < C && qsub < 4) {
    const bool two = c0 + 1 < C;
    const double px0 = pivot[1 + col0 + c0], px1 = two ? pivot[1 + col0 + c0 + 1] : 0.0;
    const int64_t gs = sub_samples / 4;
    for (int g = qsub; g < 4; g += nsubq) {
      const int64_t ia = i0 + g * gs;
      const int64_t ib = (ia + gs < i1) ? ia + gs : i1;
      double s0 = 0.0, s1 = 0.0;
      int n = 0;
      auto body = [&](double x0, double x1, double ui, double wi) {
        double a = fabs(wi);
        const double du = fabs(ui - pu);
        for (int q = 0; q < J; ++q) a *= du;
        const double v0 = fabs(x0 - px0), v1 = fabs(x1 - px1);
        bx[0] |= !(v0 <= 1.7976931348623157e308);
        bx[1] |= !(v1 <= 1.7976931348623157e308);
        mx[0] = fmax(mx[0], v0);
        mx[1] = fmax(mx[1], v1);
        s0 += a * v0;
        s1 += a * v1;
        ++n;
      };
      auto load = [&](int64_t i, double &x0, double &x1, double &ui, double &wi) {
        x1 = px1;
        if constexpr (VEC2) {
          if (two) {
            const double2 t2 = *reinterpret_cast<const double2 *>(x + i * ldx + col0 + c0);
            x0 = t2.x;
            x1 = t2.y;
          } else {
            x0 = x[i * ldx + col0 + c0];
          }
        } else {
          x0 = x[i * ldx + col0 + c0];
          if (two) x1 = x[i * ldx + col0 + c0 + 1];
        }
        ui = u[i];
        wi = w ? w[i] : 1.0;
      };
      int64_t i = ia + r;
      constexpr int UNR = 4;
      for (; i + (UNR - 1) * 16 < ib; i += UNR * 16) {
        double x0[UNR], x1[UNR], ui[UNR], wi[UNR];
#pragma unroll
        for (int q = 0; q < UNR; ++q) load(i + q * 16, x0[q], x1[q], ui[q], wi[q]);
#pragma unroll
        for (int q = 0; q < UNR; ++q) body(x0[q], x1[q], ui[q], wi[q]);
      }
      for (; i < ib; i += 16) {
        double x0, x1, ui, wi;
        load(i, x0, x1, ui, wi);
        body(x0, x1, ui, wi);
      }
      shq[g][0][slot] = s0;
      shq[g][1][slot] = s1;
      shqn[g][slot] = n;
      if (n > 0) {
        gmin[0] = fmin(gmin[0], s0 / (double)n);
        gmin[1] = fmin(gmin[1], s1 / (double)n);
      }
    }
  }
  double su = 0.0;
  int nu = 0;
  for (int64_t i = i0 + tid; i < i1; i += 256) {
    const double v = fabs(u[i] - pu);
    bu |= !(v <= 1.7976931348623157e308);
    mu = fmax(mu, v);
    double a = 1.0;
    if (w) {
      const double vw = fabs(w[i]);
      bu |= !(vw <= 1.7976931348623157e308);
      mw = fmax(mw, vw);
      a = vw;
    }
    for (int q = 0; q < J; ++q) a *= v;
    su += a;
    ++nu;
  }
  if (bx[0]) atomicOr(&badx[c0], 1);
  if (bx[1]) atomicOr(&badx[c0 + 1], 1);
  if (bu) atomicOr(&badu, 1);
#pragma unroll
  for (int v = 0; v < 2; ++v) {
    shx[v][tid] = mx[v];
    shg[v][tid] = gmin[v];
  }
  shu[tid] = mu;
  shw[tid] = mw;
  shs[tid] = su;
  shn[tid] = nu;
  __syncthreads();
  if (!fine_groups) {
#pragma unroll
    for (int v = 0; v < 2; ++v) shg[v][tid] = kInf;
    __syncthreads();
    if (tid < 128) {
      const int g = tid >> 5, col = tid & 31, ccp = col >> 1, v = col & 1;
      double sg = 0.0;
      int ng = 0;
      for (int rr = 0; rr < 16; ++rr) {
        sg += shq[g][v][rr * 16 + ccp];
        ng += shqn[g][rr * 16 + ccp];
      }
      if (ng > 0) shg[v][g * 16 + ccp] = sg / (double)ng;
    }
    __syncthreads();
  }
  double umin = kInf;
  const int gw = fine_groups ? 4 : 64;
  if (tid < 256 / gw) {
    double sg = 0.0;
    int ng = 0;
    for (int k = 0; k < gw; ++k) {
      sg += shs[gw * tid + k];
      ng += shn[gw * tid + k];
    }
    if (ng > 0) umin = sg / (double)ng;
  }
  __syncthreads();
  shs[tid] = umin;
  __syncthreads();
  for (int off = 128; off > 0; off >>= 1) {
    if (tid < off) {
      shu[tid] = fmax(shu[tid], shu[tid + off]);
      shw[tid] = fmax(shw[tid], shw[tid + off]);
      shs[tid] = fmin(shs[tid], shs[tid + off]);
      if (off >= 16) {
#pragma unroll
        for (int v = 0; v < 2; ++v) {
          shx[v][tid] = fmax(shx[v][tid], shx[v][tid + off]);
          shg[v][tid] = fmin(shg[v][tid], shg[v][tid + off]);
        }
      }
    }
    __syncthreads();
  }
  if (nsubq > 1) {
    if (tid < cpw)
      for (int q = 1; q < nsubq; ++q)
#pragma unroll
        for (int v = 0; v < 2; ++v) {
          shx[v][tid] = fmax(shx[v][tid], shx[v][tid + q * cpw]);
          shg[v][tid] = fmin(shg[v][tid], shg[v][tid + q * cpw]);
        }
    __syncthreads();
  }
  double *st = stats + sb * I8_ST_STRIDE;
  if (tid == 0) {
    st[I8_ST_MAXDU] = shu[0];
    st[I8_ST_MAXW] = shw[0];
    st[I8_ST_UMIN] = shs[0];
    st[I8_ST_BADU] = (double)badu;
  }
  if (tid < 32) {
    st[I8_ST_MAXX + tid] = shx[tid & 1][tid >> 1];
    st[I8_ST_GMIN + tid] = shg[tid & 1][tid >> 1];
    st[I8_ST_BADX + tid] = (double)badx[tid];
  }
}

__global__ __launch_bounds__(64) void i8_table_kernel(const double *__restrict__ stats, int nsub, int64_t nsub_total,
                                                      int64_t N, int64_t C, int64_t win_samples, bool weighted,
                                                      int J, double *__restrict__ wtab,
                                                      uint32_t *__restrict__ wflag, const I8State *__restrict__ states) {
  if (states != nullptr) {
    const I8State e = states[blockIdx.y];
    stats = e.stats; wtab = e.wtab; wflag = e.wflag;
  }
  const int64_t win = blockIdx.x;
  const int tid = threadIdx.x;
  const int64_t i0 = win * win_samples;
  const int64_t i1 = (i0 + win_samples < N) ? i0 + win_samples : N;
  const double kInf = __longlong_as_double(0x7ff0000000000000ll);
  __shared__ int flagged;
  if (tid == 0) flagged = 0;
  __syncthreads();
  double dumax = 0.0, wmaxv = 0.0, umin = kInf, mx = 0.0, gmin = kInf;
  bool badu = false, badx = false;
  for (int k = 0; k < nsub; ++k) {
    const int64_t sb = win * nsub + k;
    if (sb >= nsub_total) break;
    const double *st = stats + sb * I8_ST_STRIDE;
    dumax = fmax(dumax, st[I8_ST_MAXDU]);
    wmaxv = fmax(wmaxv, st[I8_ST_MAXW]);
    umin = fmin(umin, st[I8_ST_UMIN]);
    badu |= st[I8_ST_BADU] != 0.0;
    if (tid < 32) {
      mx = fmax(mx, st[I8_ST_MAXX + tid]);
      gmin = fmin(gmin, st[I8_ST_GMIN + tid]);
      badx |= st[I8_ST_BADX + tid] != 0.0;
    }
  }
  const double wmax = weighted ? wmaxv : 1.0;
  double *wt = wtab + win * I8_WT_STRIDE;
  double mtop = wmax;
  for (int q = 0; q < J; ++q) mtop *= dumax;
  const double theta = I8_GUARD * sqrt((double)(i1 - i0));
  if (tid == 0) {
    wt[I8_WT_INVDU] = dumax > 0.0 ? 1.0 / dumax : 0.0;
    wt[I8_WT_INVW] = wmax > 0.0 ? 1.0 / wmax : 0.0;
    double d = badu ? __longlong_as_double(0x7ff8000000000000ll) : wmax;
    for (int j = 0; j < 10; ++j) {
      wt[I8_WT_DSP + j] = d;
      d *= dumax;
    }
    if (mtop > theta * umin) atomicOr(&flagged, 1);
  }
  if (tid < 32) {
    wt[I8_WT_SC + tid] = mx > 0.0 ? 0x1p50 / mx : 0.0;
    wt[I8_WT_DSC + tid] = badx ? __longlong_as_double(0x7ff8000000000000ll) : mx * 0x1p-50;
    if (tid < C && mtop * mx > theta * gmin) atomicOr(&flagged, 1);
  }
  __syncthreads();
  if (tid == 0) wflag[win] = (uint32_t)flagged;
}

__global__ __launch_bounds__(256) void i8_list_kernel(const uint32_t *__restrict__ wflag, int64_t nwin,
                                                      int64_t win_tiles, int sub_tiles,
                                                      uint32_t *__restrict__ list,
                                                      uint32_t *__restrict__ n_list, const I8State *__restrict__ states) {
  if (states != nullptr) {
    const I8State e = states[blockIdx.x];
    wflag = e.wflag; list = e.list; n_list = e.n_list;
  }
  __shared__ uint32_t sh[256];
  __shared__ uint32_t running;
  const int tid = threadIdx.x;
  if (tid == 0) running = 0;
  __syncthreads();
  const int per = (int)(win_tiles / sub_tiles);
  for (int64_t base = 0; base < nwin; base += 256) {
    const int64_t wi = base + tid;
    const uint32_t f = (wi < nwin && wflag[wi] != 0u) ? 1u : 0u;
    sh[tid] = f;
    __syncthreads();
    for (int off = 1; off < 256; off <<= 1) {
      const uint32_t v = tid >= off ? sh[tid - off] : 0u;
      __syncthreads();
      sh[tid] += v;
      __syncthreads();
    }
    const uint32_t pos = running + sh[tid] - f;
    if (f)
      for (int k = 0; k < per; ++k) list[(size_t)pos * per + k] = (uint32_t)(wi * win_tiles + (int64_t)k * sub_tiles);
    __syncthreads();
    if (tid == 255) running += sh[255];
    __syncthreads();
  }
  if (tid == 0) {
    n_list[0] = running * (uint32_t)per;
    n_list[1] = running;
  }
}

bool i8_supported(int64_t N, int64_t C, int64_t nrep, int K) {
  (void)nrep;
  return N >= SM_T && C >= 1 && C <= 64 * I8_CPAD && K >= 1 && K <= 8;
}

__global__ void i8_or_flags_kernel(uint32_t *__restrict__ wflag, const uint32_t *__restrict__ yflag, int64_t nwin) {
  const int64_t w = (int64_t)blockIdx.x * blockDim.x + threadIdx.x;
  if (w < nwin) wflag[w] |= yflag[w];
}

int launch_i8_prepass(const I8Args &a, int K, hipStream_t st) {
  const int64_t sub_tiles = a.win_tiles < I8_STAT_TILES ? a.win_tiles : I8_STAT_TILES;
  const int nsub = (int)(a.win_tiles / sub_tiles);
  const int64_t nsub_total = cdiv(a.ntiles, sub_tiles);
  const bool vec2 = ((reinterpret_cast<uintptr_t>(a.x + a.col0) & 15) == 0) && (a.ldx_s % 2 == 0);
  const unsigned S = (unsigned)a.S;
  if (vec2)
    hipLaunchKernelGGL(i8_stats_kernel<true>, dim3((unsigned)nsub_total, S), dim3(256), 0, st, a.x, a.ldx_s, a.u, a.w,
                       a.N, a.C, a.col0, sub_tiles * SM_T, nsub == 1 ? 1 : 0, a.pivot, K - 1, a.stats, a.states);
  else
    hipLaunchKernelGGL(i8_stats_kernel<false>, dim3((unsigned)nsub_total, S), dim3(256), 0, st, a.x, a.ldx_s, a.u, a.w,
                       a.N, a.C, a.col0, sub_tiles * SM_T, nsub == 1 ? 1 : 0, a.pivot, K - 1, a.stats, a.states);
  TXM_LAUNCH_CHECK();
  hipLaunchKernelGGL(i8_table_kernel, dim3((unsigned)a.nwin, S), dim3(64), 0, st, a.stats, nsub, nsub_total, a.N, a.C,
                     a.win_tiles * SM_T, a.w != nullptr, K - 1, a.wtab, a.wflag, a.states);
  TXM_LAUNCH_CHECK();
  if (a.y != nullptr) {
    const bool vy = ((reinterpret_cast<uintptr_t>(a.y + a.col0) & 15) == 0) && (a.ldy_s % 2 == 0);
    if (vy)
      hipLaunchKernelGGL(i8_stats_kernel<true>, dim3((unsigned)nsub_total), dim3(256), 0, st, a.y, a.ldy_s, a.u, a.w,
                         a.N, a.C, a.col0, sub_tiles * SM_T, nsub == 1 ? 1 : 0, a.ypivot, 0, a.stats, nullptr);
    else
      hipLaunchKernelGGL(i8_stats_kernel<false>, dim3((unsigned)nsub_total), dim3(256), 0, st, a.y, a.ldy_s, a.u, a.w,
                         a.N, a.C, a.col0, sub_tiles * SM_T, nsub == 1 ? 1 : 0, a.ypivot, 0, a.stats, nullptr);
    TXM_LAUNCH_CHECK();
    hipLaunchKernelGGL(i8_table_kernel, dim3((unsigned)a.nwin), dim3(64), 0, st, a.stats, nsub, nsub_total, a.N, a.C,
                       a.win_tiles * SM_T, a.w != nullptr, 0, a.ywtab, a.yflag, nullptr);
    TXM_LAUNCH_CHECK();
    hipLaunchKernelGGL(i8_or_flags_kernel, dim3((unsigned)cdiv(a.nwin, 256)), dim3(256), 0, st, a.wflag, a.yflag, a.nwin);
    TXM_LAUNCH_CHECK();
  }
  if (a.states == nullptr) TXM_HIP(hipMemsetAsync(a.n_list, 0, 256, st));
  hipLaunchKernelGGL(i8_list_kernel, dim3(S), dim3(256), 0, st, a.wflag, a.nwin, a.win_tiles, a.sub_tiles, a.list,
                     a.n_list, a.states);
  TXM_LAUNCH_CHECK();
  return TXM_OK;
}

int launch_resample_i8(const I8Args &a, int K, bool weighted, size_t prog_bytes, hipStream_t st) {
  return launch_resample_i8t(a, K, weighted, prog_bytes, st);
}

}
```

thermoextrap_amd/csrc/txm_resample_i8g.hip:

```cpp
#include "txm_i8g.h"

namespace txm {

constexpr int G_XR = 4;
static_assert(G_XR == G_BS && G_BS == 4, "the wait counts below are written for blocks of four k-steps");
constexpr int G_XRB = 8;
constexpr int G_FU = 2176;

#ifdef TXM_G_FOUR_QUARTERS
template <int NS> constexpr int G_QUARTERS = 4;
#elif defined(TXM_G_SIX_QUARTERS)
template <int NS> constexpr int G_QUARTERS = NS == 1 ? 8 : NS == 2 ? 6 : 4;
#else
template <int NS> constexpr int G_QUARTERS = NS == 1 ? 8 : 4;
#endif

template <int J0, int JN, bool WEIGHTED, bool YS>
constexpr int G_NQ = (J0 == 0 && JN == 1 && WEIGHTED && YS) ? 4 : G_QUARTERS<JN + (YS ? 1 : 0)>;

template <int J0, int JN, bool WEIGHTED, bool YS>
__global__ __launch_bounds__(T_BLOCK) __attribute__((amdgpu_waves_per_eu(2, 2))) void resample_i8g_kernel(
    const I8Args a, const int K, const unsigned char *__restrict__ table, const int64_t rep_begin, const int n_grp) {
  constexpr int NS = JN + (YS ? 1 : 0);
  static_assert(JN >= 1 && NS <= 3 && J0 + JN <= 8, "row sets");
  constexpr int NPT = JN + ((YS && WEIGHTED && J0 > 0) ? 1 : 0);
  constexpr int NX = YS ? 2 : 1;
  constexpr int WREG = NS * T_PB;
  constexpr int NQ = G_NQ<J0, JN, WEIGHTED, YS>;
  constexpr int A_STEP = NQ * 1024;
  constexpr int PPW = G_BS * NQ / T_WAVES;
  static_assert(G_BS * NQ % T_WAVES == 0, "count pieces per wave");
  constexpr int OFF_A = T_WAVES * WREG;
  constexpr bool XBLK = !YS;
#ifdef TXM_G_ADIR
  constexpr bool ADIR = XBLK && NS == 2;
#else
  constexpr bool ADIR = false;
#endif
  constexpr int XRN = XBLK ? G_XRB : G_XR;
  constexpr int OFF_X = OFF_A + 2 * G_BS * A_STEP;
  constexpr int OFF_Y = OFF_X + T_WAVES * XRN * 1024;
  constexpr int OFF_RAW = OFF_Y + (YS ? T_WAVES * XRN * 1024 : 0);
  constexpr int OFF_F = OFF_RAW + 3 * G_RAW;
  constexpr int OFF_FS = OFF_F + 3 * 2 * G_FU;
  static_assert(G_BS * 16 * NPT * 8 <= G_FU, "factor lines");
  extern __shared__ __attribute__((aligned(16))) unsigned char lds[];
  uint32_t *fsum = reinterpret_cast<uint32_t *>(lds + OFF_FS);

  const int wave = __builtin_amdgcn_readfirstlane((int)(threadIdx.x >> 6)), lane = threadIdx.x & 63;
  const int n32 = lane & 31, half = lane >> 5;
  const uint32_t wreg = (uint32_t)(wave * WREG);

  const int b = blockIdx.x;
  const int n_wgg = (4 * n_grp + NQ - 1) / NQ;
  const int64_t win = (int64_t)((b >> 3) / n_wgg) * 8 + (b & 7);
  const int grp = (b >> 3) % n_wgg;
  if (win >= a.nwin) return;
  if (a.wflag[win] != 0u) return;
  const int64_t rep0 = rep_begin + (int64_t)grp * (32 * NQ);
  const int64_t WT = a.win_tiles;
  const int64_t t0 = win * WT;
  const int64_t t1 = t0 + WT < a.ntiles ? t0 + WT : a.ntiles;
  const int nsteps = (int)(t1 - t0) * T_STEPS;
  const int nblk = nsteps / G_BS;
  const unsigned char *tab = table + (size_t)t0 * G_TILE_BYTES;
  auto q_off = [&](int Q) -> size_t {
    int gq = grp * NQ + Q;
    if (gq >= 4 * n_grp) gq = grp * NQ;
    return (size_t)(gq >> 2) * (size_t)a.ntiles * G_TILE_BYTES + (size_t)(gq & 3) * 1024;
  };

  const int ps = lane >> 2, cl = lane & 3;
  const int col = 4 * wave + cl;
  const int ccol = col < a.C ? col : 0;
  const int qsrc = 4 * wave < a.C ? wave : 0;
  const uint32_t rd_off = wreg + (uint32_t)(((lane >> 4) & 1) * (T_PLANE + 128) + (16 * half + ((lane & 15) >> 1)) * 16 + (lane & 1) * 8);
  const int tcl = (n32 >> 2) & 3, tdg = 4 * (n32 >> 4) + (n32 & 3);
  const int ofi = wave >> 1;
  const int odig = 4 * (wave & 1) + cl;
  const uint32_t osel = odig < 7 ? (((uint32_t)odig << 24) | 0x000c0c0cu) : 0x0c0c0c0cu;
  const uint32_t oxor = odig < 6 ? 0x80000000u : 0u;

  const double *wt = a.wtab + win * I8_WT_STRIDE;
  const double pu = a.pivot[0];
  const double inv_du = wt[I8_WT_INVDU];
  const double inv_w = WEIGHTED ? wt[I8_WT_INVW] : 1.0;
  const double sc = wt[I8_WT_SC + ccol];
  const double px = a.pivot[1 + a.col0 + ccol];
  const double *wty = YS ? a.ywtab + win * I8_WT_STRIDE : wt;
  const double scy = YS ? wty[I8_WT_SC + ccol] : 0.0;
  const double py = YS ? a.ypivot[1 + a.col0 + ccol] : 0.0;

  v16i acc[NS][NQ];
#pragma unroll
  for (int e = 0; e < NS; ++e)
#pragma unroll
    for (int q = 0; q < NQ; ++q) acc[e][q] = (v16i)(0);

#ifdef TXM_G_CLOCKS
  const long long gc0 = clock64(), gr0 = wall_clock64();
#endif
#ifdef TXM_G_TIMING
  long long tm[8] = {0, 0, 0, 0, 0, 0, 0, 0};
  long long tk0 = clock64();
#define G_TICK(k) do { const long long t1_ = clock64(); tm[k] += t1_ - tk0; tk0 = t1_; } while (0)
#else
#define G_TICK(k) do {} while (0)
#endif
  auto chunk_sample = [&](int c) -> int64_t {
    int64_t b0 = (t0 + (c >> 5)) * SM_T;
    if (b0 > a.N - SM_T) b0 = a.N - SM_T;
    return b0 + 32 * (c & 31);
  };
  const uint32_t xring = (uint32_t)(OFF_X + wave * XRN * 1024), yring = (uint32_t)(OFF_Y + wave * XRN * 1024);
  int cq = 0;
  const char *xq = reinterpret_cast<const char *>(a.x + chunk_sample(0) * a.ldx_s);
  const char *yq = YS ? reinterpret_cast<const char *>(a.y + chunk_sample(0) * a.ldy_s) : nullptr;
  const int64_t xstep = 32 * a.ldx_s * 8, ystep = YS ? 32 * a.ldy_s * 8 : 0;
  const bool loader = !XBLK || wave < 4;
  const int qsrc2 = 4 * (wave + 4) < a.C ? wave + 4 : 0;
  const int64_t xcol1 = (a.col0 + 4 * qsrc) * 8, xcol2 = (a.col0 + 4 * qsrc2) * 8;
  size_t qoff[NQ];
#pragma unroll
  for (int Q = 0; Q < NQ; ++Q) qoff[Q] = q_off(Q);
  auto x_request = [&](int slot) {
#ifdef TXM_G_NO_XDMA
    if (slot >= 0) { ++cq; return; }
#endif
    if constexpr (XBLK) {
      if (loader) {
        const uint32_t ln = g_lane_now();
        const uint32_t row = (ln >> 1) * (uint32_t)(a.ldx_s * 8) + (ln & 1) * 16u + (uint32_t)(a.col0 * 8);
        g_dma16(xq, row + (uint32_t)(32 * qsrc), xring + (uint32_t)slot * 1024u);
        g_dma16(xq, row + (uint32_t)(32 * qsrc2), xring + (uint32_t)(4 * XRN * 1024) + (uint32_t)slot * 1024u);
      }
    } else {
      const uint32_t ln = g_lane_now();
      const uint32_t cb = (ln & 1) * 16u + (uint32_t)((a.col0 + 4 * qsrc) * 8);
      g_dma16(xq, (ln >> 1) * (uint32_t)(a.ldx_s * 8) + cb, xring + (uint32_t)slot * 1024u);
      if constexpr (YS) g_dma16(yq, (ln >> 1) * (uint32_t)(a.ldy_s * 8) + cb, yring + (uint32_t)slot * 1024u);
    }
    ++cq;
    if (cq < nsteps) {
      if ((cq & 31) == 0) {
        const int64_t i0 = chunk_sample(cq);
        xq = reinterpret_cast<const char *>(a.x + i0 * a.ldx_s);
        if constexpr (YS) yq = reinterpret_cast<const char *>(a.y + i0 * a.ldy_s);
      } else {
        xq += xstep;
        if constexpr (YS) yq += ystep;
      }
    }
  };
  auto a_request = [&](int B, int piece = -1) {
    const int Bc = B < nblk ? B : nblk - 1;
#ifdef TXM_G_NO_ADMA
    if (Bc >= 0) return;
#endif
    if constexpr (XBLK) {
      if (!loader) return;
      const unsigned char *src = tab + (size_t)(Bc * G_BS + wave) * G_KSTEP_BYTES;
      const uint32_t dst = (uint32_t)(OFF_A + (B & 1) * (G_BS * A_STEP) + wave * A_STEP);
#pragma unroll
      for (int Q = 0; Q < NQ; ++Q)
        if (piece < 0 || piece == Q) g_dma16_stream(src + q_off(Q), g_lane_now() * 16u, dst + (uint32_t)(Q * 1024));
    } else {
      const uint32_t l16 = g_lane_now() * 16u;
#pragma unroll
      for (int k = 0; k < PPW; ++k) {
        const int i = wave * PPW + k, st = i / NQ, Q = i % NQ;
        g_dma16_stream(tab + (size_t)(Bc * G_BS + st) * G_KSTEP_BYTES + q_off(Q), l16,
                (uint32_t)(OFF_A + (B & 1) * (G_BS * A_STEP) + st * A_STEP + Q * 1024));
      }
    }
  };
  auto raw_request = [&](int B) {
    int c = B * G_BS + 1 + (wave & 3);
    if (c > nsteps - 1) c = nsteps - 1;
    if constexpr (XBLK) {
      if (!loader) return;
      const int64_t i0 = chunk_sample(c);
      const uint32_t l4 = g_lane_now() * 4u;
      g_dma4(a.u + i0, l4, (uint32_t)(OFF_RAW + (B % 3) * G_RAW + wave * 256));
      if constexpr (WEIGHTED) g_dma4(a.w + i0, l4, (uint32_t)(OFF_RAW + (B % 3) * G_RAW + G_BS * 256 + wave * 256));
    } else {
      const double *src = ((WEIGHTED && wave >= 4) ? a.w : a.u) + chunk_sample(c);
      g_dma4(src, g_lane_now() * 4u, (uint32_t)(OFF_RAW + (B % 3) * G_RAW + (wave >> 2) * (G_BS * 256) + (wave & 3) * 256));
    }
  };
  auto stage_factors = [&](int B) {
#ifndef TXM_G_SW
#define TXM_G_SW 6
#endif
    constexpr int SW = TXM_G_SW;
    if (wave < SW || wave >= SW + 2) return;
    const int e = (int)g_lane_now() + (wave - SW) * 64;
    const double *raw = reinterpret_cast<const double *>(lds + OFF_RAW + (B % 3) * G_RAW);
#ifdef TXM_G_TIMING
    G_TICK(1);
    double r0 = raw[e];
    asm volatile("s_waitcnt lgkmcnt(0)" : "+v"(r0));
    G_TICK(5);
    const double du = (r0 - pu) * inv_du;
#else
    const double du = (raw[e] - pu) * inv_du;
#endif
    double pw = WEIGHTED ? raw[G_BS * 32 + e] * inv_w : 1.0;
    double *f = reinterpret_cast<double *>(lds + OFF_F + (B % 3) * (2 * G_FU) + ((e >> 4) & 1) * G_FU) + (((e >> 5) * 16 + (e & 15)) * NPT);
    if constexpr (NPT > JN) f[JN] = pw;
#pragma unroll
    for (int k = 0; k < J0; ++k) pw *= du;
#pragma unroll
    for (int jj = 0; jj < JN; ++jj) {
      if (WEIGHTED || J0 + jj > 0) f[jj] = pw;
      pw *= du;
    }
  };

  auto store_x2 = [&](uint32_t lo0, uint32_t hi0, uint32_t lo1, uint32_t hi1, int off) {
#ifdef TXM_G_PLAIN_STORES
    typedef __attribute__((address_space(3))) uint32_t *lds_u32;
    const uint32_t base = wreg + g_lane_now() * 4u;
    *(lds_u32)(lds + base + off) = lo0;
    *(lds_u32)(lds + base + off + T_PLANE + 128) = hi0;
    *(lds_u32)(lds + base + off + 256) = lo1;
    *(lds_u32)(lds + base + off + 256 + T_PLANE + 128) = hi1;
    return;
#endif
#ifdef TXM_G_PLAIN_STORES_ASM
    {
      const uint32_t base = wreg + g_lane_now() * 4u + (uint32_t)off;
      asm volatile("ds_write2st64_b32 %0, %1, %2 offset0:0 offset1:1\n\t"
                   "ds_write2st64_b32 %3, %4, %5 offset0:0 offset1:1"
                   :
                   : "v"(base), "v"(lo0), "v"(lo1), "v"(base + (uint32_t)(T_PLANE + 128)), "v"(hi0), "v"(hi1)
                   : "memory");
      return;
    }
#endif
    asm volatile("s_mov_b32 m0, %4\n\ts_nop 0\n\t"
                 "ds_write_addtid_b32 %0 offset:%5\n\t"
                 "ds_write_addtid_b32 %1 offset:%6\n\t"
                 "ds_write_addtid_b32 %2 offset:%7\n\t"
                 "ds_write_addtid_b32 %3 offset:%8"
                 :
                 : "v"(lo0), "v"(hi0), "v"(lo1), "v"(hi1), "s"(wreg), "n"(off), "n"(off + T_PLANE + 128), "n"(off + 256),
                   "n"(off + 256 + T_PLANE + 128)
                 : "memory", "m0");
  };
  auto produce_row = [&](auto fic, double (&f)[2], const double (&d)[2], auto &&ahead) {
    constexpr int fi = decltype(fic)::value;
    uint32_t lo[2], hi[2];
#pragma unroll
    for (int uu = 0; uu < 2; ++uu) {
      const uint64_t bits = (uint64_t)__double_as_longlong(fma(f[uu], d[uu], T_MAGIC));
      lo[uu] = (uint32_t)bits ^ 0x80808080u;
      hi[uu] = (uint32_t)(bits >> 32) ^ 0x00008080u;
    }
#ifdef TXM_G_NO_OVERLAY
    if (false) {
#else
    if (fi < JN && ofi == fi) {
#endif
#pragma unroll
      for (int uu = 0; uu < 2; ++uu) {
        const uint64_t ub = (uint64_t)__double_as_longlong(__builtin_ldexp(f[uu], 50) + T_MAGIC);
        uint32_t dig;
        asm volatile("v_perm_b32 %0, %1, %2, %3" : "=v"(dig) : "v"((uint32_t)(ub >> 32)), "v"((uint32_t)ub), "v"(osel));
        hi[uu] = (hi[uu] & 0x00ffffffu) | (dig ^ oxor);
      }
    }
    ahead();
    store_x2(lo[0], hi[0], lo[1], hi[1], fi * T_PB);
  };

  typedef __attribute__((address_space(3))) const double *lds_cd;
  typedef __attribute__((address_space(3))) const v4i *lds_cv4;

  if (threadIdx.x < 32 * NQ) {
    const int64_t r = rep0 + threadIdx.x;
    uint32_t s = 0;
    if (r < a.nrep)
      for (int64_t t = t0; t < t1; ++t) s += a.counts[(size_t)r * a.ntiles + t];
    fsum[threadIdx.x] = s;
  }
  for (int e = threadIdx.x; e < T_WAVES * WREG / 16; e += T_BLOCK) reinterpret_cast<uint4 *>(lds)[e] = make_uint4(0, 0, 0, 0);
  double d_du[2], d_w[2] = {1.0, 1.0};
  {
    const int64_t i0 = chunk_sample(0);
#pragma unroll
    for (int uu = 0; uu < 2; ++uu) {
      d_du[uu] = (a.u[i0 + 16 * uu + ps] - pu) * inv_du;
      if constexpr (WEIGHTED) d_w[uu] = a.w[i0 + 16 * uu + ps] * inv_w;
    }
  }
  asm volatile("s_waitcnt vmcnt(0)" ::: "memory");
  raw_request(0);
  raw_request(1);
  if constexpr (!ADIR) a_request(0);
  if constexpr (XBLK) {
    x_request(7);
#pragma unroll
    for (int c = 0; c < G_BS; ++c) x_request(c);
  } else {
#pragma unroll
    for (int c = 0; c < G_XR; ++c) x_request(c);
  }
  v4i AD[
#ifdef TXM_G_ADIR
      (XBLK && NS == 2) ? G_BS : 1
#else
      1
#endif
  ][NQ];
#ifdef TXM_G_ADIR
  if constexpr (XBLK && NS == 2) {
    const uint32_t l16 = g_lane_now() * 16u;
#pragma unroll
    for (int pp = 0; pp < G_BS; ++pp)
#pragma unroll
      for (int q = 0; q < NQ; ++q) g_load16(AD[pp][q], tab + (size_t)pp * G_KSTEP_BYTES + qoff[q], l16);
  }
#endif
  asm volatile("s_waitcnt vmcnt(0) lgkmcnt(0)\n\ts_barrier" ::: "memory");
  stage_factors(0);
  {
    const uint32_t xa = xring + (uint32_t)(ps * 32 + cl * 8) + (XBLK ? 7u * 1024u : 0u);
    double dx[2], dy[2] = {0.0, 0.0};
#pragma unroll
    for (int uu = 0; uu < 2; ++uu) {
      dx[uu] = (*(lds_cd)(lds + xa + uu * 512) - px) * sc;
      if constexpr (YS) dy[uu] = (*(lds_cd)(lds + xa + (yring - xring) + uu * 512) - py) * scy;
    }
    t_static_for<NS>([&](auto fic) {
      constexpr int fi = decltype(fic)::value;
      double f[2];
#pragma unroll
      for (int uu = 0; uu < 2; ++uu) {
        if constexpr (YS && fi == JN) {
          f[uu] = WEIGHTED ? d_w[uu] : 1.0;
        } else {
          double pw = WEIGHTED ? d_w[uu] : 1.0;
          for (int q = 0; q < J0 + fi; ++q) pw *= d_du[uu];
          f[uu] = pw;
        }
      }
      if constexpr (YS && fi == JN) produce_row(fic, f, dy, [] {});
      else produce_row(fic, f, dx, [] {});
    });
  }
  asm volatile("s_waitcnt lgkmcnt(0)\n\ts_barrier" ::: "memory");
  if constexpr (!XBLK) x_request(0);
  G_TICK(0);

  uint32_t *pg = a.progress != nullptr ? a.progress + (size_t)win * 16 : nullptr;
#ifdef TXM_G_PRIO
  if (wave >= 4) __builtin_amdgcn_s_setprio(TXM_G_PRIO);
#endif
  auto read_factors = [&](auto pnc, auto finc, uint32_t fb, double (&f)[2]) {
    constexpr int pn = decltype(pnc)::value, fin = decltype(finc)::value;
#pragma unroll
    for (int uu = 0; uu < 2; ++uu) {
      if constexpr (YS && fin == JN) {
        if constexpr (WEIGHTED) f[uu] = *(lds_cd)(lds + fb + uu * G_FU + (pn * 16 * NPT + (J0 == 0 ? 0 : JN)) * 8);
        else f[uu] = 1.0;
      } else if constexpr (!WEIGHTED && J0 == 0 && fin == 0) {
        f[uu] = 1.0;
      } else {
        f[uu] = *(lds_cd)(lds + fb + uu * G_FU + (pn * 16 * NPT + fin) * 8);
      }
    }
  };
  v4i A[NQ];
  constexpr bool BT2 = NS >= 2;
  v2i Bt[BT2 ? 2 : 1][2];
  double f[2], xr[2], yr[2] = {0.0, 0.0};
  uint32_t f_va = (uint32_t)(OFF_F + ps * NPT * 8);
  uint32_t x_va = xring + (uint32_t)(ps * 32 + cl * 8);
  {
    const uint32_t a_va0 = (uint32_t)OFF_A + (uint32_t)lane * 16u;
#pragma unroll
    for (int q = 0; q < NQ; ++q) {
      if constexpr (!ADIR) A[q] = *(lds_cv4)(lds + a_va0 + q * 1024);
    }
    Bt[0][0] = T_TRREAD((lds_v2i)(lds + rd_off));
    Bt[0][1] = T_TRREAD((lds_v2i)(lds + rd_off + 128));
    read_factors(std::integral_constant<int, 0>{}, std::integral_constant<int, 0>{}, f_va, f);
#pragma unroll
    for (int uu = 0; uu < 2; ++uu) xr[uu] = *(lds_cd)(lds + x_va + (XBLK ? 0 : 1024) + uu * 512);
  }
#pragma unroll 1
  for (int B = 0; B < nblk; ++B) {
    if (pg != nullptr && wave == 0 && (B & 7) == 0) {
      const uint32_t done = (uint32_t)(B >> 3) + 1u;
      if (lane == 0) __hip_atomic_store(&pg[grp & 15], done, __ATOMIC_RELAXED, __HIP_MEMORY_SCOPE_AGENT);
#pragma unroll 1
      for (int spin = 0; spin < I8_THROTTLE_SPINS; ++spin) {
        if (done <= g_min_progress(pg) + G_LEAD) break;
        __builtin_amdgcn_s_sleep(32);
      }
    }
    G_TICK(1);
    stage_factors(B + 1);
    G_TICK(7);
    raw_request(B + 2);
    const unsigned char *blk_asrc = nullptr;
    uint32_t blk_adst = 0, blk_l16 = 0, blk_xrow = 0;
    if constexpr (XBLK) {
      if (loader) {
        const int Bn = B + 1 < nblk ? B + 1 : nblk - 1;
        blk_asrc = tab + (size_t)(Bn * G_BS + wave) * G_KSTEP_BYTES;
        blk_adst = (uint32_t)(OFF_A + ((B + 1) & 1) * (G_BS * A_STEP) + wave * A_STEP);
        const uint32_t ln = g_lane_now();
        blk_l16 = ln * 16u;
        blk_xrow = (ln >> 1) * (uint32_t)(a.ldx_s * 8) + (ln & 1) * 16u;
      }
    }
    auto a_piece = [&](int Q) {
#ifndef TXM_G_NO_ADMA
      if constexpr (!ADIR)
        if (loader) g_dma16_stream(blk_asrc + qoff[Q], blk_l16, blk_adst + (uint32_t)(Q * 1024));
#endif
    };
    const unsigned char *nb_src = nullptr;
    uint32_t nb_l16 = 0;
    if constexpr (ADIR) {
      const int Bn = B + 1 < nblk ? B + 1 : nblk - 1;
      nb_src = tab + (size_t)(Bn * G_BS) * G_KSTEP_BYTES;
      nb_l16 = g_lane_now() * 16u;
    }
    auto x_chunk = [&](int i) {
#ifndef TXM_G_NO_XDMA
      if (loader) {
        const uint32_t dst = xring + (uint32_t)((4 * ((B + 1) & 1) + i) * 1024);
        g_dma16(xq + xcol1, blk_xrow, dst);
        g_dma16(xq + xcol2, blk_xrow, dst + (uint32_t)(4 * XRN * 1024));
      }
#endif
      ++cq;
      if (cq < nsteps) {
        if ((cq & 31) == 0) xq = reinterpret_cast<const char *>(a.x + chunk_sample(cq) * a.ldx_s);
        else xq += xstep;
      }
    };
#ifdef TXM_G_BURST
    constexpr bool SPREAD = false;
#else
    constexpr bool SPREAD = XBLK && NS >= 2;
#endif
    if constexpr (!SPREAD) {
      if constexpr (XBLK) {
#pragma unroll
        for (int Q = 0; Q < NQ; ++Q) a_piece(Q);
#pragma unroll
        for (int i = 0; i < G_BS; ++i) x_chunk(i);
      } else {
        a_request(B + 1);
      }
    }
    constexpr int ISSUE_SLOTS = 2 * NS;
    auto issue_items = [&](auto kc) {
      constexpr int k = decltype(kc)::value;
      if constexpr (SPREAD && k < ISSUE_SLOTS) {
        if constexpr (ADIR) {
          static_assert(!ADIR || ISSUE_SLOTS == G_BS, "one x chunk a slot");
          x_chunk(k);
        } else {
#pragma unroll
          for (int j = 0; j < NQ + 4; ++j)
            if (j * ISSUE_SLOTS / (NQ + 4) == k) {
              if (j < 8 && (j & 1) == 0) a_piece(j >> 1);
              else if (j < 8) x_chunk(j >> 1);
              else a_piece(j - 4);
            }
        }
      }
    };
    G_TICK(2);
    uint32_t a_va = (uint32_t)(OFF_A + (B & 1) * (G_BS * A_STEP)) + (uint32_t)lane * 16u;
    asm volatile("" : "+v"(f_va), "+v"(x_va), "+v"(a_va));
#ifdef TXM_G_NO_PIN
#define G_PIN() do {} while (0)
#else
#define G_PIN() __builtin_amdgcn_sched_barrier(0)
#endif
    t_static_for<G_BS>([&](auto pc) {
      constexpr int p = decltype(pc)::value;
      double dx[2], dy[2] = {0.0, 0.0};
      if constexpr (ADIR) {
        constexpr int R = WEIGHTED ? 2 : 1;
        constexpr int NL = 12 + (p < 2 ? 4 : 8) + R;
        G_PIN();
        if (loader) asm volatile("s_waitcnt vmcnt(%0)" ::"n"(NL) : "memory");
        else asm volatile("s_waitcnt vmcnt(12)" ::: "memory");
        G_PIN();
      }
      t_static_for<NS>([&](auto fic) {
        constexpr int fi = decltype(fic)::value;
        constexpr bool last = fi == NS - 1;
        if constexpr (p == G_BS - 1 && last) {
          G_TICK(3);
          if constexpr (ADIR) {
            if (loader) asm volatile("s_waitcnt vmcnt(7) lgkmcnt(0)" ::: "memory");
            else asm volatile("s_waitcnt lgkmcnt(0)" ::: "memory");
          } else {
            asm volatile("s_waitcnt vmcnt(%0) lgkmcnt(0)" ::"n"(XBLK ? 0 : 3 * NX) : "memory");
          }
#ifndef TXM_G_NO_BARRIER
          asm volatile("s_barrier" ::: "memory");
#endif
          G_TICK(6);
        }
        auto ahead = [&]() {
          if constexpr (!last) {
            read_factors(pc, std::integral_constant<int, fi + 1>{}, f_va, f);
          } else if constexpr (p < G_BS - 1) {
            read_factors(std::integral_constant<int, p + 1>{}, std::integral_constant<int, 0>{}, f_va, f);
          } else {
            f_va = (uint32_t)(OFF_F + ((B + 1) % 3) * (2 * G_FU) + ps * NPT * 8);
            asm volatile("" : "+v"(f_va));
            read_factors(std::integral_constant<int, 0>{}, std::integral_constant<int, 0>{}, f_va, f);
          }
          if constexpr (YS && fi == JN - 1) {
#pragma unroll
            for (int uu = 0; uu < 2; ++uu) yr[uu] = *(lds_cd)(lds + x_va + (OFF_Y - OFF_X) + ((p + 1) & 3) * 1024 + uu * 512);
          }
          if constexpr (last) {
            if constexpr (XBLK) {
              if constexpr (p == G_BS - 1) {
                x_va = xring + (uint32_t)(ps * 32 + cl * 8) + (uint32_t)(((B + 1) & 1) * 4096);
                asm volatile("" : "+v"(x_va));
              }
#pragma unroll
              for (int uu = 0; uu < 2; ++uu) xr[uu] = *(lds_cd)(lds + x_va + (p == G_BS - 1 ? 0 : p + 1) * 1024 + uu * 512);
            } else {
              g_wait_vm<2 * NX + (p == G_BS - 1 ? 0 : PPW + 1)>();
#pragma unroll
              for (int uu = 0; uu < 2; ++uu) xr[uu] = *(lds_cd)(lds + x_va + ((p + 2) & 3) * 1024 + uu * 512);
            }
          }
        };
        constexpr int bcur = BT2 ? ((p * NS + fi) & 1) : 0;
        const v4i Bv = {Bt[bcur][0][0], Bt[bcur][0][1], Bt[bcur][1][0], Bt[bcur][1][1]};
        auto mfma_q = [&](auto qc) {
          constexpr int q = decltype(qc)::value;
          if constexpr (ADIR) t_mfma<true>(acc[fi][q], AD[p][q], Bv);
          else t_mfma<true>(acc[fi][q], A[q], Bv);
#ifndef TXM_G_NO_AREAD
          if constexpr (last && ADIR) {
            g_load16(AD[p][q], nb_src + (size_t)p * G_KSTEP_BYTES + qoff[q], nb_l16);
          } else if constexpr (last) {
            if constexpr (p == G_BS - 1) {
              const uint32_t a_vn = (uint32_t)(OFF_A + ((B + 1) & 1) * (G_BS * A_STEP)) + g_lane_now() * 16u;
              A[q] = *(lds_cv4)(lds + a_vn + q * 1024);
            } else {
              A[q] = *(lds_cv4)(lds + a_va + (p + 1) * A_STEP + q * 1024);
            }
          }
#endif
        };
        G_PIN();
        t_static_for<(0 + 1) * NQ / 4 - 0 * NQ / 4>([&](auto jc) { mfma_q(std::integral_constant<int, 0 * NQ / 4 + decltype(jc)::value>{}); });
        G_PIN();
        issue_items(std::integral_constant<int, p * NS + fi>{});
        if constexpr (BT2) {
          constexpr int fn = (fi + 1) % NS;
          Bt[bcur ^ 1][0] = T_TRREAD((lds_v2i)(lds + rd_off + fn * T_PB));
          Bt[bcur ^ 1][1] = T_TRREAD((lds_v2i)(lds + rd_off + fn * T_PB + 128));
        }
        G_PIN();
        if constexpr (fi == 0) {
#pragma unroll
          for (int uu = 0; uu < 2; ++uu) dx[uu] = (xr[uu] - px) * sc;
        }
        if constexpr (YS && fi == JN) {
#pragma unroll
          for (int uu = 0; uu < 2; ++uu) dy[uu] = (yr[uu] - py) * scy;
        }
        uint32_t lo[2], hi[2];
#pragma unroll
        for (int uu = 0; uu < 2; ++uu) {
#ifdef TXM_G_NO_SLICE
          lo[uu] = 0x01020304u + uu;
          hi[uu] = 0x04030201u + uu;
          asm volatile("" : "+v"(lo[uu]), "+v"(hi[uu]));
#else
          const double dd = (YS && fi == JN) ? dy[uu] : dx[uu];
          const uint64_t bits = (uint64_t)__double_as_longlong(fma(f[uu], dd, T_MAGIC));
          lo[uu] = (uint32_t)bits;
          hi[uu] = (uint32_t)(bits >> 32);
#endif
        }
        G_PIN();
        t_static_for<(1 + 1) * NQ / 4 - 1 * NQ / 4>([&](auto jc) { mfma_q(std::integral_constant<int, 1 * NQ / 4 + decltype(jc)::value>{}); });
        G_PIN();
#ifndef TXM_G_NO_SLICE
#pragma unroll
        for (int uu = 0; uu < 2; ++uu) {
          lo[uu] ^= 0x80808080u;
          hi[uu] ^= 0x00008080u;
        }
#endif
        G_PIN();
#if !defined(TXM_G_NO_OVERLAY) && !defined(TXM_G_NO_SLICE)
        if (fi < JN && ofi == fi) {
#ifdef TXM_G_OVERLAY_RECOMPUTE
          const uint32_t od_l = 4u * (uint32_t)(wave & 1) + (g_lane_now() & 3u);
          const uint32_t osel_l = od_l < 7u ? ((od_l << 24) | 0x000c0c0cu) : 0x0c0c0c0cu;
          const uint32_t oxor_l = od_l < 6u ? 0x80000000u : 0u;
#else
          const uint32_t osel_l = osel, oxor_l = oxor;
#endif
#pragma unroll
          for (int uu = 0; uu < 2; ++uu) {
            const uint64_t ub = (uint64_t)__double_as_longlong(__builtin_ldexp(f[uu], 50) + T_MAGIC);
            uint32_t dig;
            asm volatile("v_perm_b32 %0, %1, %2, %3" : "=v"(dig) : "v"((uint32_t)(ub >> 32)), "v"((uint32_t)ub), "v"(osel_l));
            hi[uu] = (hi[uu] & 0x00ffffffu) | (dig ^ oxor_l);
          }
        }
#endif
        G_PIN();
#ifndef TXM_G_NO_AHEAD
        ahead();
#endif
        G_PIN();
        t_static_for<(2 + 1) * NQ / 4 - 2 * NQ / 4>([&](auto jc) { mfma_q(std::integral_constant<int, 2 * NQ / 4 + decltype(jc)::value>{}); });
        G_PIN();
#ifndef TXM_G_NO_PRODUCE
        store_x2(lo[0], hi[0], lo[1], hi[1], fi * T_PB);
#else
        asm volatile("" ::"v"(lo[0]), "v"(hi[0]), "v"(lo[1]), "v"(hi[1]));
#endif
        G_PIN();
        t_static_for<(3 + 1) * NQ / 4 - 3 * NQ / 4>([&](auto jc) { mfma_q(std::integral_constant<int, 3 * NQ / 4 + decltype(jc)::value>{}); });
        G_PIN();
#ifndef TXM_G_NO_TRREAD
        if constexpr (!BT2) {
          Bt[0][0] = T_TRREAD((lds_v2i)(lds + rd_off));
          Bt[0][1] = T_TRREAD((lds_v2i)(lds + rd_off + 128));
        }
#endif
        G_PIN();
      });
      if constexpr (!XBLK) x_request((p + 1) & 3);
    });
  }

  constexpr int XS = 65, XT = 16 * XS;
  static_assert(OFF_A + T_WAVES * XT * 4 <= OFF_RAW, "flush scratch inside the count and x rings");
  asm volatile("s_waitcnt vmcnt(0) lgkmcnt(0)\n\ts_barrier" ::: "memory");
  if (pg != nullptr && threadIdx.x == 0) __hip_atomic_store(&pg[grp & 15], 0xfffffff0u, __ATOMIC_RELAXED, __HIP_MEMORY_SCOPE_AGENT);
  auto odig_of = [](int w, int c) { return 4 * (w & 1) + c; };
  uint32_t *xw = reinterpret_cast<uint32_t *>(lds + OFF_A) + wave * XT;
  auto flush_tile = [&](v16i &T, int q, int rs) {
    uint32_t z = 0;
    asm volatile("" : "+v"(z));
    const int64_t opq = (int64_t)z;
    const bool is_y = YS && rs == JN;
    if (is_y) {
      const int64_t rrow = rep0 + 32 * q + 4 * half;
      const int c = 4 * wave + tcl;
      const bool valid = tdg < I8_NSL && c < a.C;
      const int dgt = tdg < I8_NSL ? tdg : 0;
      double dsc = wty[I8_WT_DSP + 0] * wty[I8_WT_DSC + (c < a.C ? c : 0)];
      double *base = a.part_y + (((size_t)win * a.nrep_pad + rrow) * 8 + dgt) * a.cpad + c + opq;
      const size_t stride = (size_t)8 * a.cpad;
      dsc *= (double)((int64_t)1 << (8 * dgt));
      const int bias = dgt == I8_NSL - 1 ? T_D6_BIAS : 0;
      if (valid) {
#pragma unroll
        for (int r = 0; r < 16; ++r) {
          const int m = (r >> 2) * 8 + (r & 3);
          if (rrow + m < a.nrep) {
            const int v = T[r] - bias * (int)fsum[32 * q + m + 4 * half];
            base[(size_t)m * stride] = (double)v * dsc;
          }
        }
      }
      return;
    }
#pragma unroll
    for (int r = 0; r < 16; ++r) xw[r * XS + lane] = (uint32_t)T[r];
    const int j = J0 + rs;
#pragma unroll
    for (int i = 0; i < 2; ++i) {
      const int o = lane + 64 * i, m = o >> 2, q4 = o & 3;
      const int rr = ((m >> 3) << 2) | (m & 3), hh = (m >> 2) & 1;
      const int64_t rrow = rep0 + 32 * q + m;
      if (rrow < a.nrep) {
        const uint32_t *src = xw + rr * XS + 32 * hh + 4 * q4;
        const int fs = (int)fsum[32 * q + m];
        const int c = 4 * wave + q4;
        if (c < a.C) {
          int v[I8_NSL];
#pragma unroll
          for (int d = 0; d < I8_NSL; ++d) v[d] = (int)src[16 * (d >> 2) + (d & 3)];
          v[I8_NSL - 1] -= T_D6_BIAS * fs;
          const double dsc0 = wt[I8_WT_DSP + j] * wt[I8_WT_DSC + c];
          double sum = 0.0;
#pragma unroll
          for (int d = 0; d < I8_NSL; ++d) {
            double pd = (double)v[d] * (dsc0 * (double)((int64_t)1 << (8 * d)));
            asm volatile("" : "+v"(pd));
            sum = d == 0 ? pd : sum + pd;
          }
          a.part_x[(((size_t)win * a.nrep_pad + rrow) * K + j) * a.cpad + c + opq] = sum;
        }
        const int dgt = odig_of(wave, q4);
        if (ofi == rs && dgt < 7) {
          const int v7 = (int)src[16 + 3] - (dgt == I8_NSL - 1 ? T_D6_BIAS * fs : 0);
          const double dsc = (wt[I8_WT_DSP + j] * 0x1p-50) * (double)((int64_t)1 << (8 * dgt));
          a.part_u[((size_t)win * a.nrep_pad + rrow) * K * 8 + (size_t)j * 8 + dgt + opq] = (double)v7 * dsc;
        }
      }
    }
  };
#pragma unroll
  for (int fi = 0; fi < NS; ++fi)
#pragma unroll
    for (int q = 0; q < NQ; ++q) flush_tile(acc[fi][q], q, fi);
#ifdef TXM_G_CLOCKS
  if (lane == 0 && (blockIdx.x == 0 || blockIdx.x == 1064)) {
    double *o = a.wtab + a.nwin * I8_WT_STRIDE + ((blockIdx.x ? 1 : 0) * T_WAVES + wave) * 8;
    o[0] = (double)(clock64() - gc0);
    o[1] = (double)(wall_clock64() - gr0);
  }
#endif
#ifdef TXM_G_TIMING
  G_TICK(0);
  if (lane == 0 && (blockIdx.x == 0 || blockIdx.x == 1064))
    for (int k = 0; k < 8; ++k) a.wtab[a.nwin * I8_WT_STRIDE + ((blockIdx.x ? 1 : 0) * T_WAVES + wave) * 8 + k] = (double)tm[k];
#endif
}

template <int J0, int JN, bool WEIGHTED, bool YS>
static int launch_pass_g(const I8Args &a, int K, const unsigned char *table, int64_t rep_begin, int n_grp, hipStream_t st) {
  constexpr int NS = JN + (YS ? 1 : 0);
  constexpr int NQ = G_NQ<J0, JN, WEIGHTED, YS>;
  const size_t lds = (size_t)T_WAVES * NS * T_PB + 2 * G_BS * NQ * 1024 + (size_t)(YS ? 2 * G_XR : G_XRB) * T_WAVES * 1024 + 3 * G_RAW +
                     3 * 2 * G_FU + 32 * NQ * sizeof(uint32_t);
  const dim3 grid((unsigned)(cdiv(a.nwin, 8) * 8 * cdiv(4 * (int64_t)n_grp, NQ)));
  if (a.progress != nullptr) TXM_HIP(hipMemsetAsync(a.progress, 0, (size_t)cdiv(a.nwin, 8) * 8 * 16 * sizeof(uint32_t), st));
  TXM_SET_MAX_LDS((&resample_i8g_kernel<J0, JN, WEIGHTED, YS>), lds);
  hipLaunchKernelGGL((resample_i8g_kernel<J0, JN, WEIGHTED, YS>), grid, dim3(T_BLOCK), lds, st, a, K, table, rep_begin, n_grp);
  TXM_LAUNCH_CHECK();
  return TXM_OK;
}

bool i8g_applicable(const double *x, int64_t ldx_s, int64_t C, const double *y, int64_t ldy_s) {
  if (C <= 16) return false;
  const int64_t cq = (C + 3) / 4 * 4;
  if (((uintptr_t)x & 15) != 0 || (ldx_s & 1) != 0 || cq > ldx_s) return false;
  if (y != nullptr && (((uintptr_t)y & 15) != 0 || (ldy_s & 1) != 0 || cq > ldy_s)) return false;
  return true;
}

int launch_resample_i8g(const I8Args &a, int K, bool weighted, const unsigned char *table, int64_t rep_begin, int n_grp,
                        hipStream_t st) {
  const bool ys = a.y != nullptr;
  const int rows = K + (ys ? 1 : 0), np = (rows + 2) / 3;
#ifdef TXM_G_EVEN_SPLIT
  const bool greedy = false;
#else
  const bool greedy = !ys && rows > 3 && rows % 3 == 1;
#endif
  int j0 = 0;
  for (int i = 0; i < np; ++i) {
    const int n = greedy ? (i < np - 1 ? 3 : 1) : rows / np + (i < rows % np ? 1 : 0);
    const bool last = i == np - 1;
    const int jn = n - ((last && ys) ? 1 : 0);
    const bool y_here = last && ys;
    int rc = TXM_ERR_INVALID;
#define G_CASE(J0_, JN_)                                                                                         \
  if (j0 == J0_ && jn == JN_) {                                                                                  \
    if (y_here) {                                                                                                \
      if constexpr (JN_ <= 2) rc = weighted ? launch_pass_g<J0_, JN_, true, true>(a, K, table, rep_begin, n_grp, st) \
                                            : launch_pass_g<J0_, JN_, false, true>(a, K, table, rep_begin, n_grp, st); \
    } else rc = weighted ? launch_pass_g<J0_, JN_, true, false>(a, K, table, rep_begin, n_grp, st)                \
                       : launch_pass_g<J0_, JN_, false, false>(a, K, table, rep_begin, n_grp, st);              \
  }
#ifdef TXM_G_ONLY03
    if (j0 == 0 && jn == 3 && !y_here && !weighted) rc = launch_pass_g<0, 3, false, false>(a, K, table, rep_begin, n_grp, st);
#elif defined(TXM_G_ONLY32)
    if (j0 == 3 && jn == 2 && !y_here && !weighted) rc = launch_pass_g<3, 2, false, false>(a, K, table, rep_begin, n_grp, st);
#elif defined(TXM_G_ONLY02)
    if (j0 == 0 && jn == 2 && !y_here && !weighted) rc = launch_pass_g<0, 2, false, false>(a, K, table, rep_begin, n_grp, st);
#elif defined(TXM_G_ONLY01)
    if (j0 == 0 && jn == 1 && !y_here && !weighted) rc = launch_pass_g<0, 1, false, false>(a, K, table, rep_begin, n_grp, st);
#else
    G_CASE(0, 1) G_CASE(0, 2) G_CASE(0, 3) G_CASE(2, 1) G_CASE(2, 2) G_CASE(3, 1) G_CASE(3, 2) G_CASE(3, 3)
    G_CASE(5, 1) G_CASE(5, 2) G_CASE(6, 1) G_CASE(6, 2)
#endif
#undef G_CASE
    if (rc != TXM_OK) {
      if (rc == TXM_ERR_INVALID) set_error("resample_i8g: no pass for powers %d..%d", j0, j0 + jn - 1);
      return rc;
    }
    j0 += jn;
  }
  return TXM_OK;
}

}
```

thermoextrap_amd/engine.py:

```python

from __future__ import annotations

import contextlib
import ctypes as ct
from typing import NamedTuple

import numpy as np
import torch

from . import _lib
from ._lib import ResampleOpts, SamplerSpec, check

F64 = torch.float64
_last_info: dict[tuple[int, int], torch.Tensor] = {}
_ws_cache: dict[tuple[int, int, str], torch.Tensor] = {}


def _L():
    if not _lib.gpu_ready():
        _lib.require_gpu()
    return _lib.load()


def _stream():
# ... 12 lines not shown
        _ws_cache.pop(key, None)
        buf = torch.empty(max(int(nbytes), 1 << 20), dtype=torch.uint8, device="cuda")
        _ws_cache[key] = buf
    return buf


_const_cache: "dict" = {}


def const_tensor(values, dtype=F64) -> torch.Tensor:
    key = (tuple(values), dtype, torch.cuda.current_device(), torch.cuda.current_stream().cuda_stream)
    hit = _const_cache.get(key)
    if hit is None:
        if len(_const_cache) >= 512:
            _const_cache.pop(next(iter(_const_cache)))
        host = torch.tensor(list(values), dtype=dtype).pin_memory()
        hit = _const_cache[key] = (host.to("cuda", non_blocking=True), host)
    return hit[0]


def to_device(a, dtype=F64) -> torch.Tensor:
    if isinstance(a, torch.Tensor):
        return a.to(device="cuda", dtype=dtype)
    return torch.as_tensor(np.asarray(a), dtype=dtype).to("cuda")


def _check_f64_cuda(t, name):
    if not (isinstance(t, torch.Tensor) and t.is_cuda and t.dtype == F64):
        raise TypeError(f"{name} must be a float64 CUDA tensor")


def reduce_vals(x: torch.Tensor, u: torch.Tensor, order: int, w: torch.Tensor | None = None) -> torch.Tensor:
    L = _L()
    _check_f64_cuda(x, "x")
    _check_f64_cuda(u, "u")
    squeeze = x.dim() == 1
    x2 = x.unsqueeze(1) if squeeze else x
    if x2.dim() != 2:
        raise ValueError("x must be (N,) or (N, C)")
    N, C = x2.shape
    if u.shape != (N,):
        raise ValueError(f"u must have shape ({N},), got {tuple(u.shape)}")
    u = u.contiguous()
    if w is not None:
        _check_f64_cuda(w, "w")
        if w.shape != (N,):
            raise ValueError("w must have shape (N,)")
        w = w.contiguous()
    if C == 1:
        x2 = x2.contiguous()
        ls, lc = 1, 1
    elif x2.stride(1) == 1 and (N == 1 or x2.stride(0) >= C):
        ls, lc = (x2.stride(0) if N > 1 else C), 1
    elif x2.stride(0) == 1 and (C == 1 or x2.stride(1) >= N):
        ls, lc = 1, x2.stride(1)
    else:
        x2 = x2.contiguous()
        ls, lc = C, 1
    out = torch.empty((C, 2, order + 1), dtype=F64, device="cuda")
    nws = L.txm_reduce_vals_ws_bytes(N, C, order)
    ws = workspace(nws)
    check(
        L.txm_reduce_vals(_ptr(x2), ls, lc, _ptr(u), _ptr(w), N, C, order, _ptr(out), _ptr(ws), ws.numel(), _stream()),
        "txm_reduce_vals",
    )
    return out[0] if squeeze else out


def _rowmajor_operands(x, u, w):
    _check_f64_cuda(x, "x")
    _check_f64_cuda(u, "u")
    squeeze = x.dim() == 1
    x2 = x.unsqueeze(1) if squeeze else x
    if x2.dim() != 2:
        raise ValueError("x must be (N,) or (N, C)")
    N, C = x2.shape
    if u.shape != (N,):
        raise ValueError(f"u must have shape ({N},), got {tuple(u.shape)}")
    u = u.contiguous()
    if w is not None:
        _check_f64_cuda(w, "w")
        if w.shape != (N,):
            raise ValueError("w must have shape (N,)")
        w = w.contiguous()
    if C == 1:
        x2 = x2.contiguous()
        ls, lc = 1, 1
    elif x2.stride(1) == 1 and (N == 1 or x2.stride(0) >= C):
        ls, lc = (x2.stride(0) if N > 1 else C), 1
    elif x2.stride(0) == 1 and (C == 1 or x2.stride(1) >= N):
        ls, lc = 1, x2.stride(1)
    else:
        x2 = x2.contiguous()
        ls, lc = C, 1
    return x2, ls, lc, u, w, N, C, squeeze


def reduce_pivot(x: torch.Tensor, u: torch.Tensor) -> torch.Tensor:
    L = _L()
    x2, ls, lc, u, _, N, C, _ = _rowmajor_operands(x, u, None)
    piv = torch.empty(1 + C, dtype=F64, device="cuda")
    check(L.txm_reduce_vals_pivot(_ptr(x2), ls, lc, _ptr(u), N, C, _ptr(piv), _stream()), "txm_reduce_vals_pivot")
    return piv


def reduce_sums(x: torch.Tensor, u: torch.Tensor, order: int, pivot: torch.Tensor, w: torch.Tensor | None = None) -> torch.Tensor:
    L = _L()
    x2, ls, lc, u, w, N, C, _ = _rowmajor_operands(x, u, w)
    _check_f64_cuda(pivot, "pivot")
    pivot = pivot.contiguous()
    if pivot.numel() != 1 + C:
        raise ValueError("pivot must have 1 + C entries")
    out = torch.empty((C, 2, order + 1), dtype=F64, device="cuda")
    ws = workspace(L.txm_reduce_vals_ws_bytes(N, C, order))
    check(L.txm_reduce_vals_sums(_ptr(x2), ls, lc, _ptr(u), _ptr(w), N, C, order, _ptr(pivot), _ptr(out), _ptr(ws), ws.numel(),
                                 _stream()), "txm_reduce_vals_sums")
    return out


def sums_to_state(sums: torch.Tensor, pivot: torch.Tensor) -> torch.Tensor:
    L = _L()
    _check_f64_cuda(sums, "sums")
    s = sums.contiguous()
    if s.dim() == 3:
        s = s.unsqueeze(0)
    n, C, two, K = s.shape
    if two != 2 or pivot.numel() != 1 + C:
        raise ValueError("sums must be (n, C, 2, K) with a (1 + C,) pivot")
    out = torch.empty((C, 2, K), dtype=F64, device="cuda")
    check(L.txm_sums_to_state(_ptr(s), n, _ptr(pivot.contiguous()), C, K - 1, _ptr(out), _stream()), "txm_sums_to_state")
    return out


def push_vals(state: torch.Tensor, x: torch.Tensor, u: torch.Tensor, w: torch.Tensor | None = None) -> torch.Tensor:
    L = _L()
    _check_f64_cuda(state, "state")
    x2, ls, lc, u, w, N, C, squeeze = _rowmajor_operands(x, u, w)
    st = state.unsqueeze(0) if (squeeze and state.dim() == 2) else state
    if st.dim() != 3 or st.shape[0] != C or st.shape[1] != 2 or not st.is_contiguous():
        raise ValueError(f"state must be a contiguous ({C}, 2, K) tensor, got {tuple(state.shape)}")
    order = st.shape[2] - 1
    ws = workspace(L.txm_push_vals_ws_bytes(N, C, order))
    check(L.txm_push_vals(_ptr(st), _ptr(x2), ls, lc, _ptr(u), _ptr(w), N, C, order, _ptr(ws), ws.numel(), _stream()),
          "txm_push_vals")
    return state


def reduce_vals_1d(u: torch.Tensor, mom: int, w: torch.Tensor | None = None) -> torch.Tensor:
    L = _L()
    _check_f64_cuda(u, "u")
    squeeze = u.dim() == 1
    u2 = u.unsqueeze(0) if squeeze else u
    if u2.stride(1) != 1:
        u2 = u2.contiguous()
    R, N = u2.shape
    if w is not None:
        _check_f64_cuda(w, "w")
        w = w.contiguous()
    M = mom + 1
    out = torch.empty((R, M), dtype=F64, device="cuda")
    ws = workspace(L.txm_reduce_vals_1d_ws_bytes(N, R, M))
    check(
        L.txm_reduce_vals_1d(_ptr(u2), u2.stride(0) if R > 1 else N, 1, _ptr(w), N, R, M, _ptr(out), _ptr(ws),
                             ws.numel(), _stream()),
        "txm_reduce_vals_1d",
    )
    return out[0] if squeeze else out


def indices_to_freq(indices: torch.Tensor, ndat: int | None = None) -> torch.Tensor:
    L = _L()
    idx = indices.to(device="cuda", dtype=torch.int64).contiguous()
    nrep, nsamp = idx.shape
    ndat = nsamp if ndat is None else int(ndat)
    freq = torch.empty((nrep, ndat), dtype=torch.int64, device="cuda")
    ws = workspace(L.txm_indices_to_freq_ws_bytes(), "indices")
    check(L.txm_indices_to_freq(_ptr(idx), nrep, nsamp, ndat, _ptr(freq), _ptr(ws), ws.numel(), _stream()),
          "txm_indices_to_freq")
    return freq


class DeviceSampler:

    def __init__(self, seed: int, nrep: int, ndat: int, nsamp: int = 0, rep0: int = 0):
        L = _L()
        self.spec = SamplerSpec(seed=0, nrep=int(nrep), ndat=int(ndat), nsamp=int(nsamp), rep0=int(rep0))
        self.ntiles = int(L.txm_sampler_ntiles(ndat))
        self.counts = torch.empty((nrep, self.ntiles), dtype=torch.int32, device="cuda")
        self._nws = L.txm_sampler_counts_ws_bytes(ct.byref(self.spec))
        if self._nws == 0:
            raise _lib.TxmError(f"sampler spec rejected: {_lib.last_error()}")
        self.draw(seed)

    def draw(self, seed: int) -> "DeviceSampler":
        L = _L()
        self.spec.seed = int(seed) & (2**64 - 1)
        ws = workspace(self._nws, "sampler")
        check(
            L.txm_sampler_tile_counts(ct.byref(self.spec), _ptr(self.counts), _ptr(ws), ws.numel(), _stream()),
            "txm_sampler_tile_counts",
        )
        return self

    @property
    def seed(self):
        return self.spec.seed

    @property
    def nrep(self):
        return self.spec.nrep

    @property
    def ndat(self):
        return self.spec.ndat

    @property
    def rep0(self):
        return self.spec.rep0

    def rows(self, a: int, b: int) -> "DeviceSampler":
        if not 0 <= a < b <= self.spec.nrep:
            raise ValueError(f"rows [{a}, {b}) outside [0, {self.spec.nrep})")
        v = object.__new__(DeviceSampler)
        v.spec = SamplerSpec(seed=self.spec.seed, nrep=b - a, ndat=self.spec.ndat, nsamp=self.spec.nsamp, rep0=self.spec.rep0 + a)
        v.ntiles, v.counts, v._nws = self.ntiles, self.counts[a:b], self._nws
        return v

    def freq(self) -> torch.Tensor:
        L = _L()
        out = torch.empty((self.spec.nrep, self.spec.ndat), dtype=torch.int64, device="cuda")
        check(L.txm_sampler_freq(ct.byref(self.spec), _ptr(self.counts), _ptr(out), _stream()), "txm_sampler_freq")
        return out


class ResamplePrep:

    def __init__(self):
        self.buf: torch.Tensor | None = None
        self.key = None
        self.refs = None
        self.tensors = None
        self.hits = 0
        self.misses = 0

    def lookup(self, key):
        return self.tensors if (key is not None and self.key == key and self.buf is not None) else None

    def bind(self, key, nbytes: int) -> tuple[torch.Tensor, bool]:
        valid = self.key == key and self.buf is not None and self.buf.numel() >= nbytes
        if not valid:
            if self.buf is None or self.buf.numel() < nbytes:
                self.buf = torch.empty(int(nbytes), dtype=torch.uint8, device="cuda")
            self.key = None
            self.refs = self.tensors = None
            self.misses += 1
        else:
            self.hits += 1
        return self.buf, valid

    def commit(self, key, refs=None, tensors=None):
        self.key = key
        self.refs, self.tensors = refs, tensors

    def invalidate(self):
        self.key = None
        self.refs = self.tensors = None


def _tkey(t):
    return None if t is None else (t.data_ptr(), t._version, tuple(t.shape), tuple(t.stride()))


WORKSPACE_BUDGET_BYTES: int | None = None
_budget_default: dict[int, int] = {}


def workspace_budget() -> int:
    if WORKSPACE_BUDGET_BYTES is not None:
        return int(WORKSPACE_BUDGET_BYTES)
    dev = torch.cuda.current_device()
    if dev not in _budget_default:
        free, total = torch.cuda.mem_get_info(dev)
        _budget_default[dev] = int(min(0.45 * total, 0.8 * free))
    return _budget_default[dev]


def _slab_size(L, N, C, nrep, order, path, has_y) -> int:
    need = lambda n: L.txm_resample_vals_ws_bytes_opts(N, C, n, order, path, int(has_y)) + (L.txm_resample_y_ws_bytes(N, C, n) if has_y else 0)
    budget = workspace_budget()
    if need(nrep) <= budget or nrep <= 128:
        return nrep
    lo, hi = 1, (nrep + 127) // 128
    while lo < hi:
        mid = (lo + hi + 1) // 2
        if need(min(mid * 128, nrep)) <= budget:
            lo = mid
        else:
            hi = mid - 1
    return min(lo * 128, nrep)


def _call_path(path) -> int:
    eff = path if path is not None else _forced
    if eff in ("fp64", "int8", "int8_fused", "int8_table"):
        return _PATHS[eff]
    return -1


def _table_operands_ok(x2: torch.Tensor, ls: int, C: int, y: torch.Tensor | None) -> bool:
    L = _L()
    yp, ldy = None, 0
    if y is not None:
        y2 = y.unsqueeze(1) if y.dim() == 1 else y
        if y2.dim() != 2 or y2.stride(1) != 1 or (y2.shape[0] > 1 and y2.stride(0) < C):
            yp, ldy = ct.c_void_p(256), C
        else:
            yp, ldy = ct.c_void_p(y2.data_ptr()), max(y2.stride(0) if y2.shape[0] > 1 else C, C)
    return L.txm_resample_operands_aligned(ct.c_void_p(x2.data_ptr()), ls, C, yp, ldy) == 1


def resample_vals(
    x: torch.Tensor,
    u: torch.Tensor,
    order: int,
    *,
    freq: torch.Tensor | None = None,
    sampler: DeviceSampler | None = None,
    w: torch.Tensor | None = None,
    pivot: torch.Tensor | None = None,
    out: torch.Tensor | None = None,
    path: str | None = None,
    prep: ResamplePrep | None = None,
    info: torch.Tensor | None = None,
    y: torch.Tensor | None = None,
    prep_src: tuple | None = None,
    _slab: int | None = None,
):
    L = _L()
    _check_f64_cuda(x, "x")
    _check_f64_cuda(u, "u")
    squeeze = x.dim() == 1
    x2 = x.unsqueeze(1) if squeeze else x
    if x2.dim() != 2:
        raise ValueError("x must be (N,) or (N, C)")
    N, C = x2.shape
    src = tuple(prep_src) if prep_src is not None else (x, u, w, pivot, y)
    src_key = tuple(_tkey(t) for t in src)
    if not (x2.stride(1) == 1 or C == 1) or (N > 1 and x2.stride(0) < C):
        x2 = x2.contiguous()
    if C == 1 and x2.stride(1) != 1:
        x2 = x2.contiguous()
    ls = max(x2.stride(0) if N > 1 else C, C)
    if u.shape != (N,):
        raise ValueError(f"u must have shape ({N},), got {tuple(u.shape)}")
    u = u.contiguous()
    if w is not None:
        _check_f64_cuda(w, "w")
        if w.shape != (N,):
            raise ValueError(f"w must have shape ({N},), got {tuple(w.shape)}")
        w = w.contiguous()
    if (freq is None) == (sampler is None):
        raise ValueError("give exactly one of freq= or sampler=")
    if freq is not None:
        freq = freq.to(device="cuda", dtype=torch.int64).contiguous()
        if freq.dim() != 2 or freq.shape[1] != N:
            raise ValueError(f"freq must be (nrep, {N}), got {tuple(freq.shape)}")
        nrep = freq.shape[0]
        spec_p, counts_p = None, None
    else:
        if sampler.ndat != N:
            raise ValueError(f"sampler.ndat={sampler.ndat} must equal N={N}")
        nrep = sampler.nrep
        spec_p, counts_p = ct.byref(sampler.spec), _ptr(sampler.counts)
    if pivot is not None:
        _check_f64_cuda(pivot, "pivot")
        pivot = pivot.contiguous()
        if pivot.numel() != 1 + C:
            raise ValueError("pivot must have 1 + C entries")
    if out is None:
        out = torch.empty((nrep, C, 2, order + 1), dtype=F64, device="cuda")
    else:
        _check_f64_cuda(out, "out")
        if tuple(out.shape) != (nrep, C, 2, order + 1) or not out.is_contiguous():
            raise ValueError(f"out must be a contiguous ({nrep}, {C}, 2, {order + 1}) tensor, got {tuple(out.shape)}")
    opts = ResampleOpts()
    opts.path = _slab if _slab is not None else _call_path(path)
    kern = -1
    if sampler is not None:
        kern = L.txm_resample_kernel(N, C, nrep, order, opts.path, int(y is not None), int(_table_operands_ok(x2, ls, C, y)))
    if sampler is not None and _slab is None:
        slab = _slab_size(L, N, C, nrep, order, kern & 0xFF, y is not None)
        if slab < nrep:
            ym = torch.empty((nrep, C), dtype=F64, device="cuda") if y is not None else None
            for a in range(0, nrep, slab):
                b = min(nrep, a + slab)
                r = resample_vals(x, u, order, sampler=sampler.rows(a, b), w=w, pivot=pivot, out=out[a:b], prep=prep,
                                  info=info, y=y, prep_src=prep_src if prep_src is not None else (x, u, w, pivot, y),
                                  _slab=kern & 0xFF)
                if y is not None:
                    ym[a:b] = r[1] if y.dim() > 1 else r[1][:, None]
            res = out[:, 0] if squeeze else out
            return (res, (ym[:, 0] if y.dim() == 1 else ym)) if y is not None else res
    ymean = y2 = None
    if y is not None:
        _check_f64_cuda(y, "y")
        y2 = y.unsqueeze(1) if y.dim() == 1 else y
        if tuple(y2.shape) != (N, C):
            raise ValueError(f"y must have the shape of x, ({N}, {C}); got {tuple(y2.shape)}")
        if y2.stride(1) != 1 or (N > 1 and y2.stride(0) < C):
            y2 = y2.contiguous()
        ymean = torch.empty((nrep, C), dtype=F64, device="cuda")
        opts.y, opts.ldy_s, opts.out_y = y2.data_ptr(), max(y2.stride(0) if N > 1 else C, C), ymean.data_ptr()
    key = None
    if prep is not None and freq is None:
        if (kern & 0xFF) != _PATHS["fp64"]:
            key = (src_key, N, C, order, kern)
            kept = prep.lookup(key)
            if kept is not None:
                x2, u, w, pivot, y2 = kept
                ls = max(x2.stride(0) if N > 1 else C, C)
                if y2 is not None:
                    opts.y, opts.ldy_s = y2.data_ptr(), max(y2.stride(0) if N > 1 else C, C)
            buf, valid = prep.bind(key, L.txm_resample_prep_bytes(N, C, nrep, order))
            opts.prep, opts.prep_bytes, opts.prep_valid = buf.data_ptr(), buf.numel(), int(valid)
    if info is None:
        ikey = (torch.cuda.current_device(), torch.cuda.current_stream().cuda_stream)
        info = _last_info.get(ikey)
        if info is None:
            info = _last_info[ikey] = torch.zeros(4, dtype=torch.int64, device="cuda")
    if not (info.is_cuda and info.dtype == torch.int64 and info.numel() >= 4 and info.is_contiguous()):
        raise TypeError("info must be a contiguous int64 CUDA tensor with >= 4 elements")
    opts.info = info.data_ptr()
    ws = workspace(L.txm_resample_vals_ws_bytes_opts(N, C, nrep, order, opts.path, int(y is not None))
                   + (L.txm_resample_y_ws_bytes(N, C, nrep) if y is not None else 0))
    check(
        L.txm_resample_vals(_ptr(x2), ls, 1, _ptr(u), _ptr(w), N, C, order, nrep, _ptr(freq), spec_p, counts_p,
                            _ptr(pivot), _ptr(out), ct.byref(opts), _ptr(ws), ws.numel(), _stream()),
        "txm_resample_vals",
    )
    if key is not None:
        prep.commit(key, refs=src, tensors=(x2, u, w, pivot, y2))
    res = out[:, 0] if squeeze else out
    if y is not None:
        return res, (ymean[:, 0] if y.dim() == 1 else ymean)
    return res


def _state_table(xs, us, ws):
    S = len(xs)
    if S < 1 or len(us) != S or (ws is not None and len(ws) != S):
        raise ValueError("need the same number (>= 1) of x, u (and w) tensors")
    x2 = []
    for x in xs:
        _check_f64_cuda(x, "x")
        x = x.unsqueeze(1) if x.dim() == 1 else x
        if x.dim() != 2:
            raise ValueError("every x must be (N,) or (N, C)")
        x2.append(x if x.is_contiguous() else x.contiguous())
    N, C = x2[0].shape
    if any(tuple(x.shape) != (N, C) for x in x2):
        raise ValueError("the batched path needs states of one shape (N, C)")
    u2 = []
    for u in us:
        _check_f64_cuda(u, "u")
        if u.shape != (N,):
            raise ValueError(f"every u must have shape ({N},)")
        u2.append(u.contiguous())
    w2 = None
    if ws is not None:
        w2 = []
        for w in ws:
            _check_f64_cuda(w, "w")
            if w.shape != (N,):
                raise ValueError(f"every w must have shape ({N},)")
            w2.append(w.contiguous())
    tab = (_lib.StatePtrs * S)()
    for s in range(S):
        tab[s].x, tab[s].u = x2[s].data_ptr(), u2[s].data_ptr()
        tab[s].w = w2[s].data_ptr() if w2 is not None else None
    return tab, (x2, u2, w2), S, N, C


def reduce_vals_batched(xs, us, order: int, ws=None) -> torch.Tensor:
    L = _L()
    tab, keep, S, N, C = _state_table(xs, us, ws)
    out = torch.empty((S, C, 2, order + 1), dtype=F64, device="cuda")
    wsb = workspace(L.txm_reduce_vals_batched_ws_bytes(S, N, C, order))
    check(L.txm_reduce_vals_batched(tab, S, C, N, C, order, _ptr(out), _ptr(wsb), wsb.numel(), _stream()),
          "txm_reduce_vals_batched")
    del keep
    return out[:, 0] if xs[0].dim() == 1 else out


def resample_vals_batched(xs, us, order: int, *, nrep: int, sampler: DeviceSampler | None = None,
                          freq: torch.Tensor | None = None, ws=None, path: str | None = None,
                          prep: ResamplePrep | None = None) -> torch.Tensor:
    L = _L()
    src = (tuple(xs), tuple(us), None if ws is None else tuple(ws))
    tab, keep, S, N, C = _state_table(xs, us, ws)
    if (freq is None) == (sampler is None):
        raise ValueError("give exactly one of freq= or sampler=")
    spec_p = counts_p = None
    if freq is not None:
        freq = freq.to(device="cuda", dtype=torch.int64).contiguous()
        if tuple(freq.shape) != (S * nrep, N):
            raise ValueError(f"freq must be ({S * nrep}, {N}), got {tuple(freq.shape)}")
    else:
        if sampler.ndat != N or sampler.nrep != S * nrep:
            raise ValueError(f"the sampler must span {S} x {nrep} replicates of {N} samples")
        spec_p, counts_p = ct.byref(sampler.spec), _ptr(sampler.counts)
    out = torch.empty((S, nrep, C, 2, order + 1), dtype=F64, device="cuda")
    opts = _lib.ResampleOpts()
    opts.path = _call_path(path)
    key = None
    if prep is not None and freq is None:
        nb = L.txm_resample_batched_prep_bytes(S, N, C, nrep, order)
        takes_i8 = bool(nb) and (opts.path in (1, 2, 3) or (opts.path == -1 and L.txm_resample_batched_path(S, N, C, nrep, order) == 1))
        if takes_i8:
            key = (tuple(_tkey(t) for t in src[0]), tuple(_tkey(t) for t in src[1]),
                   None if src[2] is None else tuple(_tkey(t) for t in src[2]), S, N, C, nrep, order)
            kept = prep.lookup(key)
            if kept is not None:
                tab, keep = kept
            buf, valid = prep.bind(key, nb)
            opts.prep, opts.prep_bytes, opts.prep_valid = buf.data_ptr(), buf.numel(), int(valid)
    ikey = (torch.cuda.current_device(), torch.cuda.current_stream().cuda_stream)
    info = _last_batched_info.get(ikey)
    if info is None:
        info = _last_batched_info[ikey] = torch.zeros(4, dtype=torch.int64, device="cuda")
    opts.info = info.data_ptr()
    wsb = workspace(L.txm_resample_vals_batched_ws_bytes(S, N, C, nrep, order))
    check(L.txm_resample_vals_batched_opts(tab, S, C, N, C, order, nrep, _ptr(freq), spec_p, counts_p, _ptr(out), ct.byref(opts),
                                           _ptr(wsb), wsb.numel(), _stream()), "txm_resample_vals_batched_opts")
    if key is not None:
        prep.commit(key, refs=src, tensors=(tab, keep))
    del keep
    return out[:, :, 0] if xs[0].dim() == 1 else out


_last_batched_info: dict = {}


def batched_info() -> dict:
    info = _last_batched_info.get((torch.cuda.current_device(), torch.cuda.current_stream().cuda_stream))
    if info is None:
        return {}
    v = info.cpu().tolist()
    return {"path": "int8" if v[0] == 1 else "fp64", "windows": int(v[1]), "windows_fp64": int(v[2]), "prep_reused": bool(v[3] & 1)}


def resample_path(N: int, C: int, nrep: int, order: int) -> str:
    L = _L()
    if _forced == "fp64":
        return "fp64"
    if _forced in ("int8", "int8_fused", "int8_table"):
        return "int8" if L.txm_resample_i8_supported(int(N), int(C), int(nrep), int(order)) == 1 else "fp64"
    return "int8" if L.txm_resample_path(int(N), int(C), int(nrep), int(order)) == 1 else "fp64"


_PATHS = {None: -1, "auto": -1, "fp64": 0, "int8": 1, "int8_fused": 2, "int8_table": 3}
_forced: str | None = None


@contextlib.contextmanager
def forced_path(path: str | None):
    global _forced
    if path not in _PATHS:
        raise ValueError(f"path must be one of {sorted(k for k in _PATHS if k)} or None")
    _L()
    prev = _forced
    _forced = None if path == "auto" else path
    try:
        yield
    finally:
        _forced = prev


def resample_info(N: int | None = None, C: int | None = None, nrep: int | None = None, order: int | None = None) -> dict:
    _L()
    info = _last_info.get((torch.cuda.current_device(), torch.cuda.current_stream().cuda_stream))
    if info is None:
        raise RuntimeError("no resample_vals call has been made on this stream")
    v = info.cpu().tolist()
    return {"path": "int8" if v[0] == 1 else "fp64", "windows": int(v[1]), "windows_fp64": int(v[2]),
            "prep_reused": bool(v[3] & 1), "kernel": ("fp64" if v[0] != 1 else "int8_table" if v[3] & 2 else "int8_fused")}


def resample_data(data: torch.Tensor, freq: torch.Tensor | None, order: int) -> torch.Tensor:
    L = _L()
    _check_f64_cuda(data, "data")
    data = data.contiguous()
    nrec, C = data.shape[:2]
    if data.shape[2:] != (2, order + 1):
        raise ValueError("data must be (nrec, C, 2, order+1)")
    if freq is not None:
        freq = freq.to(device="cuda", dtype=torch.int64).contiguous()
        if freq.shape[1] != nrec:
            raise ValueError("freq must be (nrep, nrec)")
        nrep = freq.shape[0]
    else:
        nrep = 1
    out = torch.empty((nrep, C, 2, order + 1), dtype=F64, device="cuda")
    ws = workspace(L.txm_resample_data_ws_bytes(nrec, C, order))
    check(
        L.txm_resample_data(_ptr(data), _ptr(freq), nrec, C, nrep, order, _ptr(out), _ptr(ws), ws.numel(), _stream()),
        "txm_resample_data",
    )
    return out


def convert_cov(states: torch.Tensor, to_central: bool) -> torch.Tensor:
    L = _L()
    _check_f64_cuda(states, "states")
    s = states.contiguous()
    K = s.shape[-1]
    if s.shape[-2] != 2:
        raise ValueError("states must be (..., 2, K)")
    out = torch.empty_like(s)
    check(L.txm_convert_cov(_ptr(s), _ptr(out), s.numel() // (2 * K), K - 1, int(to_central), _stream()),
          "txm_convert_cov")
    return out


def convert_1d(states: torch.Tensor, to_central: bool) -> torch.Tensor:
    L = _L()
    _check_f64_cuda(states, "states")
    s = states.contiguous()
    M = s.shape[-1]
    out = torch.empty_like(s)
    check(L.txm_convert_1d(_ptr(s), _ptr(out), s.numel() // M, M, int(to_central), _stream()), "txm_convert_1d")
    return out


def cov_over_rep(vals: torch.Tensor) -> torch.Tensor:
    L = _L()
    _check_f64_cuda(vals, "vals")
    v = vals.contiguous()
    n_ord, nrep, nval = v.shape
    out = torch.empty((nval, n_ord, n_ord), dtype=F64, device="cuda")
    check(L.txm_cov_over_rep(_ptr(v), n_ord, nrep, nval, _ptr(out), _stream()), "txm_cov_over_rep")
    return out


TAYLOR_MODES = {"sum": 0, "cumsum": 1, "terms": 2}


def predict_taylor(derivs: torch.Tensor, dalphas, mode: str = "sum") -> torch.Tensor:
    L = _L()
    _check_f64_cuda(derivs, "derivs")
    if mode not in TAYLOR_MODES:
        raise ValueError(f"mode must be one of {sorted(TAYLOR_MODES)}")
    d = derivs.contiguous()
    n_ord = d.shape[0]
    if not 1 <= n_ord <= 16:
        raise ValueError("predict_taylor: 1 <= n_ord <= 16")
    M = d[0].numel()
    da = to_device(np.atleast_1d(np.asarray(dalphas, dtype=np.float64)).ravel())
    na = da.numel()
    if na < 1 or M < 1:
        raise ValueError("predict_taylor: empty input")
    shape = (na, *d.shape[1:]) if mode == "sum" else (na, n_ord, *d.shape[1:])
    out = torch.empty(shape, dtype=F64, device="cuda")
    step = 65535
    for a0 in range(0, na, step):
        a1 = min(na, a0 + step)
        check(L.txm_predict_taylor(_ptr(d), n_ord, M, _ptr(da[a0:a1]), a1 - a0, TAYLOR_MODES[mode], _ptr(out[a0:a1]),
                                   _stream()), "txm_predict_taylor")
    return out


def perturb(x: torch.Tensor, u: torch.Tensor, dalphas, freq: torch.Tensor | None = None) -> torch.Tensor:
    L = _L()
    _check_f64_cuda(x, "x")
    _check_f64_cuda(u, "u")
    squeeze = x.dim() == 1
    x2 = x.unsqueeze(1) if squeeze else x
    if x2.stride(1) != 1 or (x2.shape[0] > 1 and x2.stride(0) < x2.shape[1]):
        x2 = x2.contiguous()
    N, C = x2.shape
    if u.shape != (N,):
        raise ValueError(f"u must have shape ({N},), got {tuple(u.shape)}")
    u = u.contiguous()
    da = np.atleast_1d(np.asarray(dalphas, dtype=np.float64))
    nrep = 1
    if freq is not None:
        freq = freq.to(device="cuda", dtype=torch.int64).contiguous()
        if freq.dim() != 2 or freq.shape[1] != N:
            raise ValueError(f"freq must be (nrep, {N}), got {tuple(freq.shape)}")
        nrep = freq.shape[0]
    outs = []
    for a0 in range(0, len(da), 8):
        chunk = np.ascontiguousarray(da[a0 : a0 + 8])
        na = len(chunk)
        out = torch.empty((nrep, na, C), dtype=F64, device="cuda")
        ws = workspace(L.txm_perturb_ws_bytes(N, C, na, nrep))
        check(
            L.txm_perturb(_ptr(x2), max(x2.stride(0), C) if N > 1 else C, _ptr(u), N, C,
                          chunk.ctypes.data_as(ct.POINTER(ct.c_double)), na, _ptr(freq), nrep, _ptr(out), _ptr(ws),
                          ws.numel(), _stream()),
            "txm_perturb",
        )
        outs.append(out)
    res = torch.cat(outs, dim=1)
    if freq is None:
        res = res[0]
    return res[..., 0] if squeeze else res


class MbarSolution(NamedTuple):

    f: np.ndarray
    logD: torch.Tensor
    upiv: float
    iterations: int
    evaluations: int
    gradient: float


def _mbar_table(us, xs=None):
    K = len(us)
    if not 1 <= K <= 64:
        raise ValueError(f"MBAR needs 1 <= K <= 64 states, got {K}")
    if xs is not None and len(xs) != K:
        raise ValueError("need one x per u")
    u2, x2, ns, C = [], [], [], 1
    for s in range(K):
        u = us[s]
        _check_f64_cuda(u, "u")
        if u.dim() != 1 or u.shape[0] < 1:
            raise ValueError("every u must be (n,) with n >= 1")
        u2.append(u.contiguous())
        ns.append(u.shape[0])
        if xs is not None:
            x = xs[s]
            _check_f64_cuda(x, "x")
            x = x.unsqueeze(1) if x.dim() == 1 else x
            if x.dim() != 2 or x.shape[0] != u.shape[0]:
                raise ValueError(f"x of state {s} must be ({u.shape[0]},) or ({u.shape[0]}, C)")
            if x.stride(1) != 1 or (x.shape[0] > 1 and x.stride(0) < x.shape[1]):
                x = x.contiguous()
            if s == 0:
                C = x.shape[1]
            elif x.shape[1] != C:
                raise ValueError("every state's x must have the same number of columns")
            x2.append(x)
    tab = (_lib.MbarState * K)()
    for s in range(K):
        tab[s].u = u2[s].data_ptr()
        tab[s].n = ns[s]
        if xs is not None:
            tab[s].x = x2[s].data_ptr()
            tab[s].ldx_s = max(x2[s].stride(0), C) if ns[s] > 1 else C
    return tab, (u2, x2), np.asarray(ns, dtype=np.float64), C


def mbar_pivot(us) -> float:
    tot = sum(float(u.sum()) for u in us)
    return tot / sum(u.shape[0] for u in us)


def mbar_eval(us, alpha0, g, upiv: float, logD: torch.Tensor | None = None):
    L = _L()
    tab, keep, ns, _ = _mbar_table(us)
    K = len(us)
    a0 = np.ascontiguousarray(alpha0, dtype=np.float64)
    gg = np.ascontiguousarray(g, dtype=np.float64)
    if a0.shape != (K,) or gg.shape != (K,):
        raise ValueError("alpha0 and g need one entry per state")
    if logD is not None:
        _check_f64_cuda(logD, "logD")
        if logD.shape != (int(ns.sum()),) or not logD.is_contiguous():
            raise ValueError("logD must be a contiguous (sum n,) tensor")
    nh = K * (K + 1) // 2
    out = torch.empty(K + nh + 1, dtype=F64, device="cuda")
    ws = workspace(L.txm_mbar_ws_bytes(K, 1, 1), tag="mbar")
    dp = ct.POINTER(ct.c_double)
    check(L.txm_mbar_eval(tab, K, a0.ctypes.data_as(dp), gg.ctypes.data_as(dp), float(upiv), _ptr(out), _ptr(logD), _ptr(ws),
                          ws.numel(), _stream()), "txm_mbar_eval")
    v = out.cpu().numpy()
    del keep
    H = np.zeros((K, K))
    H[np.triu_indices(K)] = v[K:K + nh]
    H = H + np.triu(H, 1).T
    return v[:K].copy(), H, float(v[K + nh])


_MBAR_MAX_STEP = 50.0


def mbar_newton(evaluate, N, b, *, f0=None, tol: float = 1e-12, max_iter: int = 100):
    N = np.asarray(N, dtype=np.float64)
    b = np.asarray(b, dtype=np.float64)
    K = len(N)
    Ntot = float(N.sum())
    f = np.zeros(K) if f0 is None else np.asarray(f0, dtype=np.float64) - float(f0[0])
    eps = np.finfo(np.float64).eps

    def point(f):
        g = b + f
        c = -float(g.max())
        g = g + c
        S, H, obj = evaluate(g)
        S, H = np.asarray(S, dtype=np.float64), np.asarray(H, dtype=np.float64)
        F = obj - c * Ntot - float(N @ f)
        rnd = 64 * eps * (abs(obj) + abs(c) * Ntot + float(N @ np.abs(f)) + Ntot)
        return S, H, F, rnd, g

    S, H, F, rnd, g = point(f)
    n_eval = 1
    for it in range(max_iter + 1):
        grad = S - N
        err = float(np.max(np.abs(grad) / N))
        if not np.isfinite(err):
            raise _lib.TxmError(f"MBAR solve: the gradient is not finite (max |S_k - N_k| / N_k = {err})")
        if err <= tol:
            return f, g, it, n_eval, err
        if it == max_iter:
            break
        Hr = (np.diag(S) - H)[1:, 1:]
        gr = grad[1:]
        lam, V = np.linalg.eigh(0.5 * (Hr + Hr.T))
        floor = 1e-12 * max(float(lam.max()), float(N.min()))
        good = lam > floor
        proj = V.T @ gr
        step = -(V[:, good] @ (proj[good] / lam[good]))
        if not good.all():
            flat = -(V[:, ~good] @ (proj[~good] / floor))
            big = float(np.max(np.abs(flat)))
            if big > _MBAR_MAX_STEP:
                flat *= _MBAR_MAX_STEP / big
            step = step + flat
        slope = float(gr @ step)
        t = 1.0
        while True:
            fn = f.copy()
            fn[1:] += t * step
            Sn, Hn, Fn, rn, gn = point(fn)
            n_eval += 1
            errn = float(np.max(np.abs(Sn - N) / N))
            if Fn <= F + 1e-4 * t * slope or (abs(Fn - F) <= max(rnd, rn) and errn < err):
                break
            t *= 0.5
            if t < 1e-10:
                raise _lib.TxmError(f"MBAR solve: the line search found no decrease at iteration {it}; "
                                    f"max |S_k - N_k| / N_k = {err:.3e}")
        f, S, H, F, rnd, g = fn, Sn, Hn, Fn, rn, gn
    raise _lib.TxmError(f"MBAR solve did not converge in {max_iter} Newton iterations: "
                        f"max |S_k - N_k| / N_k = {err:.3e} > tol {tol:.1e}")


def mbar_initial_f(us, alpha0) -> np.ndarray:
    a0 = np.asarray(alpha0, dtype=np.float64)
    means = np.array([float(u.mean()) for u in us])
    order = np.argsort(a0, kind="stable")
    f = np.zeros(len(a0))
    for i in range(1, len(order)):
        p, q = order[i - 1], order[i]
        f[q] = f[p] + (a0[q] - a0[p]) * 0.5 * (means[p] + means[q])
    return f - f[0]


def mbar_solve(us, alpha0, *, tol: float = 1e-12, max_iter: int = 100) -> MbarSolution:
    K = len(us)
    a0 = np.asarray(alpha0, dtype=np.float64).reshape(-1)
    if a0.shape != (K,):
        raise ValueError("need one alpha0 per state")
    ns = np.array([u.shape[0] for u in us], dtype=np.float64)
    upiv = mbar_pivot(us)
    logD = torch.empty(int(ns.sum()), dtype=F64, device="cuda")
    b = np.log(ns) - a0 * upiv

    def evaluate(g):
        return mbar_eval(us, a0, g, upiv, logD)

    f, _, it, n_eval, err = mbar_newton(evaluate, ns, b, f0=mbar_initial_f(us, a0), tol=tol, max_iter=max_iter)
    return MbarSolution(f, logD, upiv, it, n_eval, err)


def mbar_predict(xs, us, alpha0, f, logD, alphas, *, upiv: float | None = None) -> torch.Tensor:
    L = _L()
    tab, keep, ns, C = _mbar_table(us, xs)
    K = len(us)
    if upiv is None:
        upiv = mbar_pivot(us)
    if logD is None:
        a0 = np.asarray(alpha0, dtype=np.float64).reshape(-1)
        g = np.log(ns) + np.asarray(f, dtype=np.float64) - a0 * upiv
        logD = torch.empty(int(ns.sum()), dtype=F64, device="cuda")
# ... 18 lines not shown
```

Before: 626.7 million samples/s.

## Add six-digit int8 table path for order-4, 32-column resampling

```diff
diff --git a/include/txmom.h b/include/txmom.h
--- a/include/txmom.h
+++ b/include/txmom.h
@@ -85,6 +85,7 @@
 #define TXM_PATH_INT8 1
 #define TXM_PATH_INT8_FUSED 2
 #define TXM_PATH_INT8_TABLE 3
+#define TXM_PATH_INT8_TABLE6 4
 typedef struct txm_resample_opts {
   int32_t path;
   int32_t prep_valid;
diff --git a/thermoextrap_amd/csrc/txm_resample.hip b/thermoextrap_amd/csrc/txm_resample.hip
--- a/thermoextrap_amd/csrc/txm_resample.hip
+++ b/thermoextrap_amd/csrc/txm_resample.hip
@@ -709,9 +709,13 @@
   if (N < 786432 || nrep <= I8_REPS || pad128 > pad64) return false;
   return !(i8t_narrow_nq(C, K) == 4 && K == 5);
 }
+static bool six_digit_shape(int64_t N, int64_t C, int K, bool has_y) {
+  return K == 5 && !has_y && C >= I8_CPAD && cdiv(N, SM_T) >= (int64_t)TXM_WIN_MIN * I8_WIN_TILES;
+}
 static bool table_call_rule(size_t table_bytes, int eff, int64_t N, int64_t C, int64_t nrep, int K, bool has_y, bool applicable) {
   if (eff == TXM_PATH_FP64 || eff == TXM_PATH_INT8_FUSED || table_bytes == 0 || !applicable) return false;
-  if (eff == TXM_PATH_INT8_TABLE) return true;
+  if (eff == TXM_PATH_INT8_TABLE || eff == TXM_PATH_INT8_TABLE6) return true;
+  if (six_digit_shape(N, C, K, has_y)) return true;
   return C > 16 ? table_kernel_pays(nrep, K, has_y) : narrow_table_pays(N, C, nrep, K);
 }
 static bool table_operands_ok(const double *x, int64_t ldx_s, int64_t C, int K, const double *y, int64_t ldy_s) {
@@ -722,7 +726,7 @@
   if (!i8_supported(N, C, nrep, K)) return false;
   const int ov = call_path != TXM_PATH_AUTO ? call_path : path_override();
   if (ov == TXM_PATH_FP64) return false;
-  if (ov == TXM_PATH_INT8 || ov == TXM_PATH_INT8_FUSED || ov == TXM_PATH_INT8_TABLE) return true;
+  if (ov == TXM_PATH_INT8 || ov == TXM_PATH_INT8_FUSED || ov == TXM_PATH_INT8_TABLE || ov == TXM_PATH_INT8_TABLE6) return true;
   if (C <= 16) return K >= 2 && (N >= 786432 || (N >= 262144 && nrep >= 128));
   const int64_t ctail = C % I8_CPAD;
   const bool long_series = N >= 786432;
@@ -735,7 +739,7 @@
 using namespace txm;
 
 extern "C" int txm_set_resample_path(int path) {
-  TXM_REQUIRE(path == -1 || path == TXM_PATH_FP64 || path == TXM_PATH_INT8 || path == TXM_PATH_INT8_FUSED || path == TXM_PATH_INT8_TABLE, "set_resample_path: %d is not a path", path);
+  TXM_REQUIRE(path == -1 || path == TXM_PATH_FP64 || path == TXM_PATH_INT8 || path == TXM_PATH_INT8_FUSED || path == TXM_PATH_INT8_TABLE || path == TXM_PATH_INT8_TABLE6, "set_resample_path: %d is not a path", path);
   g_path_override = path;
   return TXM_OK;
 }
@@ -745,12 +749,16 @@
                                int64_t nwin, int from_prep, int64_t *info) {
   if (threadIdx.x == 0 && blockIdx.x == 0) {
     int64_t flagged = 0;
-    for (int g = 0; g < ngroups; ++g)
-      flagged += reinterpret_cast<const uint32_t *>(prep_groups + (size_t)g * group_stride + off_nlist)[1];
+    bool six = (from_prep & 4) != 0;
+    for (int g = 0; g < ngroups; ++g) {
+      const uint32_t *nl = reinterpret_cast<const uint32_t *>(prep_groups + (size_t)g * group_stride + off_nlist);
+      flagged += nl[1];
+      if (nl[2] != 0u) six = false;
+    }
     info[0] = TXM_PATH_INT8;
     info[1] = nwin * ngroups;
     info[2] = flagged;
-    info[3] = from_prep;
+    info[3] = (from_prep & 3) | (six ? 4 : 0);
   }
 }
 __global__ void fp64_info_kernel(int64_t *info) {
@@ -1041,7 +1049,7 @@
     f.sub_tiles = q.sub_tiles; f.batch = nullptr; f.progress = nullptr;
     TXM_REQUIRE(q.fb.nrep_pad == q.nrep_pad, "resample_vals: replicate padding of the two kernels differs");
     int g = 0;
-    bool have_table = false;
+    bool have_table = false, six_plan = true;
     for (int64_t col0 = 0; col0 < C; col0 += I8_CPAD, ++g) {
       unsigned char *pg = pb + q.prep_group0 + (size_t)g * q.prep_group_stride;
       b.wtab = (double *)(pg + q.prep_wt);
@@ -1071,9 +1079,15 @@
         }
         I8Args bg = b;
         bg.progress = (throttle_on() && nrep > G_REPS) ? (uint32_t *)((char *)ws + q.off_gprog) : nullptr;
+        const bool six = C > 16 && K == 5 && !with_y && b.C == I8_CPAD &&
+                         (eff_path == TXM_PATH_INT8_TABLE6 ||
+                          ((eff_path == TXM_PATH_AUTO || eff_path == TXM_PATH_INT8) && six_digit_shape(N, C, K, with_y)));
+        if (six) bg.plan6 = b.n_list + 2;
+        else six_plan = false;
         rc = C > 16 ? launch_resample_i8g(bg, K, w != nullptr, table, 0, (int)cdiv(nrep, G_REPS), st)
                     : launch_resample_i8gn(bg, K, w != nullptr, table, 0, (int)cdiv(nrep, G_REPS), 0, st);
       } else {
+        six_plan = false;
         rc = launch_resample_i8(b, K, w != nullptr, q.prog_bytes, st);
       }
       if (rc != TXM_OK) return rc;
@@ -1125,7 +1139,7 @@
       TXM_HIP(hipMemcpyAsync((char *)ws + q.off_prep, pb, q.prep_total, hipMemcpyDeviceToDevice, st));
     if (info != nullptr) {
       hipLaunchKernelGGL(i8_info_kernel, dim3(1), dim3(64), 0, st, pb + q.prep_group0, q.prep_group_stride, q.prep_nlist,
-                         q.ngroups, q.nwin, (have_tables ? 1 : 0) | (have_table ? 2 : 0), info);
+                         q.ngroups, q.nwin, (have_tables ? 1 : 0) | (have_table ? 2 : 0) | (six_plan ? 4 : 0), info);
       TXM_LAUNCH_CHECK();
     }
     return TXM_OK;
@@ -1195,7 +1209,7 @@
   o.path = TXM_PATH_AUTO; o.prep_valid = 0; o.prep = nullptr; o.prep_bytes = 0; o.info = nullptr;
   o.y = nullptr; o.ldy_s = 0; o.out_y = nullptr;
   if (opts) o = *opts;
-  TXM_REQUIRE(o.path == TXM_PATH_AUTO || o.path == TXM_PATH_FP64 || o.path == TXM_PATH_INT8 || o.path == TXM_PATH_INT8_FUSED || o.path == TXM_PATH_INT8_TABLE,
+  TXM_REQUIRE(o.path == TXM_PATH_AUTO || o.path == TXM_PATH_FP64 || o.path == TXM_PATH_INT8 || o.path == TXM_PATH_INT8_FUSED || o.path == TXM_PATH_INT8_TABLE || o.path == TXM_PATH_INT8_TABLE6,
               "resample_vals: opts.path %d is not a path", (int)o.path);
   TXM_REQUIRE((o.y == nullptr) == (o.out_y == nullptr), "resample_vals: opts.y and opts.out_y go together");
   TXM_REQUIRE(o.y == nullptr || o.ldy_s >= C, "resample_vals: opts.ldy_s < C");
@@ -1292,7 +1306,7 @@
   if (!i8_supported(N, C, nrep, K) || i8t_narrow_nq(C, K) == 0) return false;
   const int ov = call_path != TXM_PATH_AUTO ? call_path : path_override();
   if (ov == TXM_PATH_FP64) return false;
-  if (ov == TXM_PATH_INT8 || ov == TXM_PATH_INT8_FUSED || ov == TXM_PATH_INT8_TABLE) return true;
+  if (ov == TXM_PATH_INT8 || ov == TXM_PATH_INT8_FUSED || ov == TXM_PATH_INT8_TABLE || ov == TXM_PATH_INT8_TABLE6) return true;
   (void)S;
   return K >= 2 && (N >= 786432 || (N >= 262144 && nrep >= 128));
 }
@@ -1473,7 +1487,7 @@
                                               const txm_sampler_spec *spec, const uint32_t *counts, double *out,
                                               const txm_resample_opts *opts, void *ws, size_t ws_bytes, txm_stream stream) {
   const int call_path = opts ? opts->path : TXM_PATH_AUTO;
-  TXM_REQUIRE(call_path == TXM_PATH_AUTO || call_path == TXM_PATH_FP64 || call_path == TXM_PATH_INT8 || call_path == TXM_PATH_INT8_FUSED || call_path == TXM_PATH_INT8_TABLE,
+  TXM_REQUIRE(call_path == TXM_PATH_AUTO || call_path == TXM_PATH_FP64 || call_path == TXM_PATH_INT8 || call_path == TXM_PATH_INT8_FUSED || call_path == TXM_PATH_INT8_TABLE || call_path == TXM_PATH_INT8_TABLE6,
               "resample_vals_batched: opts.path %d is not a path", call_path);
   TXM_REQUIRE(!(opts && (opts->y || opts->out_y)), "resample_vals_batched: no second sample matrix on the batched entry");
   TXM_REQUIRE(states_host && out && ws, "resample_vals_batched: null pointer");
diff --git a/thermoextrap_amd/csrc/txm_resample_i8.h b/thermoextrap_amd/csrc/txm_resample_i8.h
--- a/thermoextrap_amd/csrc/txm_resample_i8.h
+++ b/thermoextrap_amd/csrc/txm_resample_i8.h
@@ -11,6 +11,7 @@
 constexpr int I8_SUB_TILES = 8;
 
 constexpr double I8_GUARD = 275.0;
+constexpr double I8_GUARD6 = I8_GUARD / 16.0;
 
 constexpr int I8_WT_INVDU = 0, I8_WT_INVW = 1, I8_WT_DSP = 2, I8_WT_SC = 12, I8_WT_DSC = 44;
 
@@ -69,6 +70,7 @@
   uint32_t *n_list;
   int sub_tiles;
   uint32_t *progress;
+  const uint32_t *plan6 = nullptr;
 };
 #ifndef TXM_I8_LEAD
 #define TXM_I8_LEAD 2
diff --git a/thermoextrap_amd/csrc/txm_resample_i8.hip b/thermoextrap_amd/csrc/txm_resample_i8.hip
--- a/thermoextrap_amd/csrc/txm_resample_i8.hip
+++ b/thermoextrap_amd/csrc/txm_resample_i8.hip
@@ -210,7 +210,8 @@
 __global__ __launch_bounds__(64) void i8_table_kernel(const double *__restrict__ stats, int nsub, int64_t nsub_total,
                                                       int64_t N, int64_t C, int64_t win_samples, bool weighted,
                                                       int J, double *__restrict__ wtab,
-                                                      uint32_t *__restrict__ wflag, const I8State *__restrict__ states) {
+                                                      uint32_t *__restrict__ wflag, const I8State *__restrict__ states,
+                                                      uint32_t *__restrict__ d6fail = nullptr) {
   if (states != nullptr) {
     const I8State e = states[blockIdx.y];
     stats = e.stats; wtab = e.wtab; wflag = e.wflag;
@@ -220,8 +221,8 @@
   const int64_t i0 = win * win_samples;
   const int64_t i1 = (i0 + win_samples < N) ? i0 + win_samples : N;
   const double kInf = __longlong_as_double(0x7ff0000000000000ll);
-  __shared__ int flagged;
-  if (tid == 0) flagged = 0;
+  __shared__ int flagged, flagged6;
+  if (tid == 0) flagged = flagged6 = 0;
   __syncthreads();
   double dumax = 0.0, wmaxv = 0.0, umin = kInf, mx = 0.0, gmin = kInf;
   bool badu = false, badx = false;
@@ -244,6 +245,7 @@
   double mtop = wmax;
   for (int q = 0; q < J; ++q) mtop *= dumax;
   const double theta = I8_GUARD * sqrt((double)(i1 - i0));
+  const double theta6 = I8_GUARD6 * sqrt((double)(i1 - i0));
   if (tid == 0) {
     wt[I8_WT_INVDU] = dumax > 0.0 ? 1.0 / dumax : 0.0;
     wt[I8_WT_INVW] = wmax > 0.0 ? 1.0 / wmax : 0.0;
@@ -253,14 +255,17 @@
       d *= dumax;
     }
     if (mtop > theta * umin) atomicOr(&flagged, 1);
+    if (mtop > theta6 * umin) atomicOr(&flagged6, 1);
   }
   if (tid < 32) {
     wt[I8_WT_SC + tid] = mx > 0.0 ? 0x1p50 / mx : 0.0;
     wt[I8_WT_DSC + tid] = badx ? __longlong_as_double(0x7ff8000000000000ll) : mx * 0x1p-50;
     if (tid < C && mtop * mx > theta * gmin) atomicOr(&flagged, 1);
+    if (tid < C && mtop * mx > theta6 * gmin) atomicOr(&flagged6, 1);
   }
   __syncthreads();
   if (tid == 0) wflag[win] = (uint32_t)flagged;
+  if (tid == 0 && d6fail != nullptr && flagged == 0 && flagged6 != 0) atomicOr(d6fail, 1u);
 }
 
 __global__ __launch_bounds__(256) void i8_list_kernel(const uint32_t *__restrict__ wflag, int64_t nwin,
@@ -324,8 +329,10 @@
     hipLaunchKernelGGL(i8_stats_kernel<false>, dim3((unsigned)nsub_total, S), dim3(256), 0, st, a.x, a.ldx_s, a.u, a.w,
                        a.N, a.C, a.col0, sub_tiles * SM_T, nsub == 1 ? 1 : 0, a.pivot, K - 1, a.stats, a.states);
   TXM_LAUNCH_CHECK();
+  if (a.states == nullptr) TXM_HIP(hipMemsetAsync(a.n_list, 0, 256, st));
   hipLaunchKernelGGL(i8_table_kernel, dim3((unsigned)a.nwin, S), dim3(64), 0, st, a.stats, nsub, nsub_total, a.N, a.C,
-                     a.win_tiles * SM_T, a.w != nullptr, K - 1, a.wtab, a.wflag, a.states);
+                     a.win_tiles * SM_T, a.w != nullptr, K - 1, a.wtab, a.wflag, a.states,
+                     a.states == nullptr ? a.n_list + 2 : (uint32_t *)nullptr);
   TXM_LAUNCH_CHECK();
   if (a.y != nullptr) {
     const bool vy = ((reinterpret_cast<uintptr_t>(a.y + a.col0) & 15) == 0) && (a.ldy_s % 2 == 0);
@@ -337,12 +344,11 @@
                          a.N, a.C, a.col0, sub_tiles * SM_T, nsub == 1 ? 1 : 0, a.ypivot, 0, a.stats, nullptr);
     TXM_LAUNCH_CHECK();
     hipLaunchKernelGGL(i8_table_kernel, dim3((unsigned)a.nwin), dim3(64), 0, st, a.stats, nsub, nsub_total, a.N, a.C,
-                       a.win_tiles * SM_T, a.w != nullptr, 0, a.ywtab, a.yflag, nullptr);
+                       a.win_tiles * SM_T, a.w != nullptr, 0, a.ywtab, a.yflag, (const I8State *)nullptr, (uint32_t *)nullptr);
     TXM_LAUNCH_CHECK();
     hipLaunchKernelGGL(i8_or_flags_kernel, dim3((unsigned)cdiv(a.nwin, 256)), dim3(256), 0, st, a.wflag, a.yflag, a.nwin);
     TXM_LAUNCH_CHECK();
   }
-  if (a.states == nullptr) TXM_HIP(hipMemsetAsync(a.n_list, 0, 256, st));
   hipLaunchKernelGGL(i8_list_kernel, dim3(S), dim3(256), 0, st, a.wflag, a.nwin, a.win_tiles, a.sub_tiles, a.list,
                      a.n_list, a.states);
   TXM_LAUNCH_CHECK();
diff --git a/thermoextrap_amd/csrc/txm_resample_i8g.hip b/thermoextrap_amd/csrc/txm_resample_i8g.hip
--- a/thermoextrap_amd/csrc/txm_resample_i8g.hip
+++ b/thermoextrap_amd/csrc/txm_resample_i8g.hip
@@ -18,12 +18,16 @@
 template <int J0, int JN, bool WEIGHTED, bool YS>
 constexpr int G_NQ = (J0 == 0 && JN == 1 && WEIGHTED && YS) ? 4 : G_QUARTERS<JN + (YS ? 1 : 0)>;
 
-template <int J0, int JN, bool WEIGHTED, bool YS>
+template <int J0, int JN, bool WEIGHTED, bool YS, int MODE = 0>
 __global__ __launch_bounds__(T_BLOCK) __attribute__((amdgpu_waves_per_eu(2, 2))) void resample_i8g_kernel(
     const I8Args a, const int K, const unsigned char *__restrict__ table, const int64_t rep_begin, const int n_grp) {
-  constexpr int NS = JN + (YS ? 1 : 0);
+  constexpr bool D6 = MODE == 1, U5 = MODE == 2;
+  static_assert(!D6 || (J0 == 0 && JN == 4 && !YS), "six-digit pass: powers 0..3");
+  static_assert(!U5 || (J0 == 4 && JN == 1 && !YS), "u-row pass: power 4");
+  constexpr int NS = D6 ? 3 : JN + (YS ? 1 : 0);
   static_assert(JN >= 1 && NS <= 3 && J0 + JN <= 8, "row sets");
-  constexpr int NPT = JN + ((YS && WEIGHTED && J0 > 0) ? 1 : 0);
+  constexpr int NPT = U5 ? 5 : JN + ((YS && WEIGHTED && J0 > 0) ? 1 : 0);
+  constexpr int FU = U5 ? 2688 : G_FU;
   constexpr int NX = YS ? 2 : 1;
   constexpr int WREG = NS * T_PB;
   constexpr int NQ = G_NQ<J0, JN, WEIGHTED, YS>;
@@ -42,8 +46,8 @@
   constexpr int OFF_Y = OFF_X + T_WAVES * XRN * 1024;
   constexpr int OFF_RAW = OFF_Y + (YS ? T_WAVES * XRN * 1024 : 0);
   constexpr int OFF_F = OFF_RAW + 3 * G_RAW;
-  constexpr int OFF_FS = OFF_F + 3 * 2 * G_FU;
-  static_assert(G_BS * 16 * NPT * 8 <= G_FU, "factor lines");
+  constexpr int OFF_FS = OFF_F + 3 * 2 * FU;
+  static_assert(G_BS * 16 * NPT * 8 <= FU && FU > 2040, "factor lines");
   extern __shared__ __attribute__((aligned(16))) unsigned char lds[];
   uint32_t *fsum = reinterpret_cast<uint32_t *>(lds + OFF_FS);
 
@@ -57,6 +61,7 @@
   const int grp = (b >> 3) % n_wgg;
   if (win >= a.nwin) return;
   if (a.wflag[win] != 0u) return;
+  if (a.plan6 != nullptr && ((*a.plan6 == 0u) != (MODE != 0))) return;
   const int64_t rep0 = rep_begin + (int64_t)grp * (32 * NQ);
   const int64_t WT = a.win_tiles;
   const int64_t t0 = win * WT;
@@ -78,14 +83,18 @@
   const int tcl = (n32 >> 2) & 3, tdg = 4 * (n32 >> 4) + (n32 & 3);
   const int ofi = wave >> 1;
   const int odig = 4 * (wave & 1) + cl;
-  const uint32_t osel = odig < 7 ? (((uint32_t)odig << 24) | 0x000c0c0cu) : 0x0c0c0c0cu;
-  const uint32_t oxor = odig < 6 ? 0x80000000u : 0u;
+  const int us = 4 * wave + cl, uj = us < 24 ? us / 6 : 4, ud = us < 24 ? us % 6 : us - 24;
+  const uint32_t osel = U5 ? (us < 31 ? (((uint32_t)ud << 24) | 0x000c0c0cu) : 0x0c0c0c0cu)
+                           : (odig < 7 ? (((uint32_t)odig << 24) | 0x000c0c0cu) : 0x0c0c0c0cu);
+  const uint32_t oxor = U5 ? ((us < 31 && ud < 6) ? 0x80000000u : 0u) : (odig < 6 ? 0x80000000u : 0u);
+  const double uscale = uj < 4 ? 0x1p46 : 0x1p50;
+  const uint32_t ju8 = (uint32_t)uj * 8u;
 
   const double *wt = a.wtab + win * I8_WT_STRIDE;
   const double pu = a.pivot[0];
   const double inv_du = wt[I8_WT_INVDU];
   const double inv_w = WEIGHTED ? wt[I8_WT_INVW] : 1.0;
-  const double sc = wt[I8_WT_SC + ccol];
+  const double sc = wt[I8_WT_SC + ccol] * (D6 ? 0x1p-4 : 1.0);
   const double px = a.pivot[1 + a.col0 + ccol];
   const double *wty = YS ? a.ywtab + win * I8_WT_STRIDE : wt;
   const double scy = YS ? wty[I8_WT_SC + ccol] : 0.0;
@@ -206,13 +215,21 @@
     const double du = (raw[e] - pu) * inv_du;
 #endif
     double pw = WEIGHTED ? raw[G_BS * 32 + e] * inv_w : 1.0;
-    double *f = reinterpret_cast<double *>(lds + OFF_F + (B % 3) * (2 * G_FU) + ((e >> 4) & 1) * G_FU) + (((e >> 5) * 16 + (e & 15)) * NPT);
+    double *f = reinterpret_cast<double *>(lds + OFF_F + (B % 3) * (2 * FU) + ((e >> 4) & 1) * FU) + (((e >> 5) * 16 + (e & 15)) * NPT);
+    if constexpr (U5) {
+#pragma unroll
+      for (int k = 0; k < 5; ++k) {
+        f[k] = pw;
+        pw *= du;
+      }
+      return;
+    }
     if constexpr (NPT > JN) f[JN] = pw;
 #pragma unroll
     for (int k = 0; k < J0; ++k) pw *= du;
 #pragma unroll
     for (int jj = 0; jj < JN; ++jj) {
-      if (WEIGHTED || J0 + jj > 0) f[jj] = pw;
+      if (WEIGHTED || D6 || J0 + jj > 0) f[jj] = pw;
       pw *= du;
     }
   };
@@ -248,6 +265,15 @@
                    "n"(off + 256 + T_PLANE + 128)
                  : "memory", "m0");
   };
+  auto store_x1 = [&](uint32_t w0, uint32_t w1, int off) {
+    asm volatile("s_mov_b32 m0, %2\n\ts_nop 0\n\t"
+                 "ds_write_addtid_b32 %0 offset:%3\n\t"
+                 "ds_write_addtid_b32 %1 offset:%4"
+                 :
+                 : "v"(w0), "v"(w1), "s"(wreg), "n"(off), "n"(off + 256)
+                 : "memory", "m0");
+  };
+  double fo0[2] = {0.0, 0.0};
   auto produce_row = [&](auto fic, double (&f)[2], const double (&d)[2], auto &&ahead) {
     constexpr int fi = decltype(fic)::value;
     uint32_t lo[2], hi[2];
@@ -260,11 +286,13 @@
 #ifdef TXM_G_NO_OVERLAY
     if (false) {
 #else
-    if (fi < JN && ofi == fi) {
+    if (U5 || (fi < JN && ofi == fi)) {
 #endif
 #pragma unroll
       for (int uu = 0; uu < 2; ++uu) {
-        const uint64_t ub = (uint64_t)__double_as_longlong(__builtin_ldexp(f[uu], 50) + T_MAGIC);
+        uint64_t ub;
+        if constexpr (U5) ub = (uint64_t)__double_as_longlong(fma(fo0[uu], uscale, T_MAGIC));
+        else ub = (uint64_t)__double_as_longlong(__builtin_ldexp(f[uu], 50) + T_MAGIC);
         uint32_t dig;
         asm volatile("v_perm_b32 %0, %1, %2, %3" : "=v"(dig) : "v"((uint32_t)(ub >> 32)), "v"((uint32_t)ub), "v"(osel));
         hi[uu] = (hi[uu] & 0x00ffffffu) | (dig ^ oxor);
@@ -274,8 +302,22 @@
     store_x2(lo[0], hi[0], lo[1], hi[1], fi * T_PB);
   };
 
+  auto d6_words = [&](const double (&fa)[2], const double (&fb)[2], const double (&d)[2], uint32_t (&la)[2], uint32_t (&lb)[2],
+                      uint32_t (&h)[2]) {
+#pragma unroll
+    for (int uu = 0; uu < 2; ++uu) {
+      const uint64_t ba = (uint64_t)__double_as_longlong(fma(fa[uu], d[uu], T_MAGIC));
+      const uint64_t bb = (uint64_t)__double_as_longlong(fma(fb[uu], d[uu], T_MAGIC));
+      la[uu] = (uint32_t)ba ^ 0x80808080u;
+      lb[uu] = (uint32_t)bb ^ 0x80808080u;
+      h[uu] = __builtin_amdgcn_perm((uint32_t)(bb >> 32), (uint32_t)(ba >> 32), 0x05040100u) ^ 0x80808080u;
+    }
+  };
+
   typedef __attribute__((address_space(3))) const double *lds_cd;
   typedef __attribute__((address_space(3))) const v4i *lds_cv4;
+  typedef double v2d __attribute__((ext_vector_type(2)));
+  typedef __attribute__((address_space(3))) const v2d *lds_cv2d;
 
   if (threadIdx.x < 32 * NQ) {
     const int64_t r = rep0 + threadIdx.x;
@@ -332,7 +374,35 @@
       dx[uu] = (*(lds_cd)(lds + xa + uu * 512) - px) * sc;
       if constexpr (YS) dy[uu] = (*(lds_cd)(lds + xa + (yring - xring) + uu * 512) - py) * scy;
     }
-    t_static_for<NS>([&](auto fic) {
+    if constexpr (D6) {
+      double fj[4][2];
+#pragma unroll
+      for (int uu = 0; uu < 2; ++uu) {
+        double pw = WEIGHTED ? d_w[uu] : 1.0;
+#pragma unroll
+        for (int j = 0; j < 4; ++j) {
+          fj[j][uu] = pw;
+          pw *= d_du[uu];
+        }
+      }
+      uint32_t la[2], lb[2], h01[2], h23[2];
+      d6_words(fj[0], fj[1], dx, la, lb, h01);
+      store_x2(la[0], lb[0], la[1], lb[1], T_PB);
+      d6_words(fj[2], fj[3], dx, la, lb, h23);
+      store_x2(la[0], lb[0], la[1], lb[1], 2 * T_PB);
+      store_x2(h01[0], h23[0], h01[1], h23[1], 0);
+    }
+    if constexpr (U5) {
+#pragma unroll
+      for (int uu = 0; uu < 2; ++uu) {
+        double pw = WEIGHTED ? d_w[uu] : 1.0;
+#pragma unroll
+        for (int k = 0; k < 4; ++k)
+          if (k < uj) pw *= d_du[uu];
+        fo0[uu] = pw;
+      }
+    }
+    if constexpr (!D6) t_static_for<NS>([&](auto fic) {
       constexpr int fi = decltype(fic)::value;
       double f[2];
 #pragma unroll
@@ -357,17 +427,31 @@
 #ifdef TXM_G_PRIO
   if (wave >= 4) __builtin_amdgcn_s_setprio(TXM_G_PRIO);
 #endif
+  double f2[2] = {0.0, 0.0}, fu[2] = {0.0, 0.0};
   auto read_factors = [&](auto pnc, auto finc, uint32_t fb, double (&f)[2]) {
     constexpr int pn = decltype(pnc)::value, fin = decltype(finc)::value;
+    if constexpr (D6) {
+#pragma unroll
+      for (int uu = 0; uu < 2; ++uu) {
+        const v2d v = *(lds_cv2d)(lds + fb + uu * FU + (pn * 16 * NPT + 2 * fin) * 8);
+        f[uu] = v.x;
+        f2[uu] = v.y;
+      }
+      return;
+    }
+    if constexpr (U5) {
+#pragma unroll
+      for (int uu = 0; uu < 2; ++uu) fu[uu] = *(lds_cd)(lds + fb + ju8 + uu * FU + pn * 16 * NPT * 8);
+    }
 #pragma unroll
     for (int uu = 0; uu < 2; ++uu) {
       if constexpr (YS && fin == JN) {
-        if constexpr (WEIGHTED) f[uu] = *(lds_cd)(lds + fb + uu * G_FU + (pn * 16 * NPT + (J0 == 0 ? 0 : JN)) * 8);
+        if constexpr (WEIGHTED) f[uu] = *(lds_cd)(lds + fb + uu * FU + (pn * 16 * NPT + (J0 == 0 ? 0 : JN)) * 8);
         else f[uu] = 1.0;
       } else if constexpr (!WEIGHTED && J0 == 0 && fin == 0) {
         f[uu] = 1.0;
       } else {
-        f[uu] = *(lds_cd)(lds + fb + uu * G_FU + (pn * 16 * NPT + fin) * 8);
+        f[uu] = *(lds_cd)(lds + fb + uu * FU + (pn * 16 * NPT + (U5 ? J0 : 0) + fin) * 8);
       }
     }
   };
@@ -513,11 +597,11 @@
         }
         auto ahead = [&]() {
           if constexpr (!last) {
-            read_factors(pc, std::integral_constant<int, fi + 1>{}, f_va, f);
+            if constexpr (!D6 || fi == 0) read_factors(pc, std::integral_constant<int, fi + 1>{}, f_va, f);
           } else if constexpr (p < G_BS - 1) {
             read_factors(std::integral_constant<int, p + 1>{}, std::integral_constant<int, 0>{}, f_va, f);
           } else {
-            f_va = (uint32_t)(OFF_F + ((B + 1) % 3) * (2 * G_FU) + ps * NPT * 8);
+            f_va = (uint32_t)(OFF_F + ((B + 1) % 3) * (2 * FU) + ps * NPT * 8);
             asm volatile("" : "+v"(f_va));
             read_factors(std::integral_constant<int, 0>{}, std::integral_constant<int, 0>{}, f_va, f);
           }
@@ -577,7 +661,10 @@
 #pragma unroll
           for (int uu = 0; uu < 2; ++uu) dy[uu] = (yr[uu] - py) * scy;
         }
-        uint32_t lo[2], hi[2];
+        uint32_t lo[2], hi[2], hp[2];
+        if constexpr (D6) {
+          if constexpr (fi < 2) d6_words(f, f2, dx, lo, hi, hp);
+        } else {
 #pragma unroll
         for (int uu = 0; uu < 2; ++uu) {
 #ifdef TXM_G_NO_SLICE
@@ -591,19 +678,30 @@
           hi[uu] = (uint32_t)(bits >> 32);
 #endif
         }
+        }
         G_PIN();
         t_static_for<(1 + 1) * NQ / 4 - 1 * NQ / 4>([&](auto jc) { mfma_q(std::integral_constant<int, 1 * NQ / 4 + decltype(jc)::value>{}); });
         G_PIN();
 #ifndef TXM_G_NO_SLICE
-#pragma unroll
-        for (int uu = 0; uu < 2; ++uu) {
-          lo[uu] ^= 0x80808080u;
-          hi[uu] ^= 0x00008080u;
+        if constexpr (!D6) {
+#pragma unroll
+          for (int uu = 0; uu < 2; ++uu) {
+            lo[uu] ^= 0x80808080u;
+            hi[uu] ^= 0x00008080u;
+          }
         }
 #endif
         G_PIN();
 #if !defined(TXM_G_NO_OVERLAY) && !defined(TXM_G_NO_SLICE)
-        if (fi < JN && ofi == fi) {
+        if constexpr (U5) {
+#pragma unroll
+          for (int uu = 0; uu < 2; ++uu) {
+            const uint64_t ub = (uint64_t)__double_as_longlong(fma(fu[uu], uscale, T_MAGIC));
+            const uint32_t dig = __builtin_amdgcn_perm((uint32_t)(ub >> 32), (uint32_t)ub, osel);
+            hi[uu] = (hi[uu] & 0x00ffffffu) | (dig ^ oxor);
+          }
+        }
+        if (!D6 && !U5 && fi < JN && ofi == fi) {
 #ifdef TXM_G_OVERLAY_RECOMPUTE
           const uint32_t od_l = 4u * (uint32_t)(wave & 1) + (g_lane_now() & 3u);
           const uint32_t osel_l = od_l < 7u ? ((od_l << 24) | 0x000c0c0cu) : 0x0c0c0c0cu;
@@ -628,7 +726,14 @@
         t_static_for<(2 + 1) * NQ / 4 - 2 * NQ / 4>([&](auto jc) { mfma_q(std::integral_constant<int, 2 * NQ / 4 + decltype(jc)::value>{}); });
         G_PIN();
 #ifndef TXM_G_NO_PRODUCE
-        store_x2(lo[0], hi[0], lo[1], hi[1], fi * T_PB);
+        if constexpr (D6) {
+          if constexpr (fi < 2) {
+            store_x2(lo[0], hi[0], lo[1], hi[1], (fi + 1) * T_PB);
+            store_x1(hp[0], hp[1], fi * (T_PLANE + 128));
+          }
+        } else {
+          store_x2(lo[0], hi[0], lo[1], hi[1], fi * T_PB);
+        }
 #else
         asm volatile("" ::"v"(lo[0]), "v"(hi[0]), "v"(lo[1]), "v"(hi[1]));
 #endif
@@ -707,6 +812,18 @@
           }
           a.part_x[(((size_t)win * a.nrep_pad + rrow) * K + j) * a.cpad + c + opq] = sum;
         }
+        if constexpr (U5) {
+          const int s_ = 4 * wave + q4;
+          if (s_ < 31) {
+            const int pj = s_ < 24 ? s_ / 6 : 4, pd = s_ < 24 ? s_ % 6 : s_ - 24;
+            const int v7 = (int)src[16 + 3] - (pd == I8_NSL - 1 ? T_D6_BIAS * fs : 0);
+            const double dsc = (wt[I8_WT_DSP + pj] * (pj < 4 ? 0x1p-46 : 0x1p-50)) * (double)((int64_t)1 << (8 * pd));
+            double *pu_ = a.part_u + ((size_t)win * a.nrep_pad + rrow) * K * 8 + (size_t)pj * 8 + opq;
+            pu_[pd] = (double)v7 * dsc;
+            if (pj < 4 && pd == 5) pu_[6] = 0.0;
+          }
+          continue;
+        }
         const int dgt = odig_of(wave, q4);
         if (ofi == rs && dgt < 7) {
           const int v7 = (int)src[16 + 3] - (dgt == I8_NSL - 1 ? T_D6_BIAS * fs : 0);
@@ -716,10 +833,54 @@
       }
     }
   };
-#pragma unroll
-  for (int fi = 0; fi < NS; ++fi)
-#pragma unroll
-    for (int q = 0; q < NQ; ++q) flush_tile(acc[fi][q], q, fi);
+  auto flush_d6 = [&](int q) {
+    static_assert(T_WAVES * 3 * XT * 4 <= OFF_RAW, "six-digit flush scratch");
+    uint32_t *xw6 = reinterpret_cast<uint32_t *>(lds) + wave * 3 * XT;
+#pragma unroll
+    for (int t = 0; t < 3; ++t)
+#pragma unroll
+      for (int r = 0; r < 16; ++r) xw6[t * XT + r * XS + lane] = (uint32_t)acc[t][q][r];
+    uint32_t z = 0;
+    asm volatile("" : "+v"(z));
+    const int64_t opq = (int64_t)z;
+#pragma unroll
+    for (int i = 0; i < 2; ++i) {
+      const int o = lane + 64 * i, m = o >> 2, q4 = o & 3;
+      const int rr = ((m >> 3) << 2) | (m & 3), hh = (m >> 2) & 1;
+      const int64_t rrow = rep0 + 32 * q + m;
+      const int c = 4 * wave + q4;
+      if (rrow < a.nrep && c < a.C) {
+        const uint32_t *src = xw6 + rr * XS + 32 * hh + 4 * q4;
+        const double dscx = wt[I8_WT_DSC + c] * 0x1p4;
+#pragma unroll
+        for (int j = 0; j < 4; ++j) {
+          int v[6];
+#pragma unroll
+          for (int d = 0; d < 4; ++d) v[d] = (int)src[(1 + (j >> 1)) * XT + 16 * (j & 1) + d];
+#pragma unroll
+          for (int d = 4; d < 6; ++d) v[d] = (int)src[16 * (j >> 1) + 2 * (j & 1) + d - 4];
+          const double dsc0 = wt[I8_WT_DSP + j] * dscx;
+          double sum = 0.0;
+#pragma unroll
+          for (int d = 0; d < 6; ++d) {
+            double pd = (double)v[d] * (dsc0 * (double)((int64_t)1 << (8 * d)));
+            asm volatile("" : "+v"(pd));
+            sum = d == 0 ? pd : sum + pd;
+          }
+          a.part_x[(((size_t)win * a.nrep_pad + rrow) * K + j) * a.cpad + c + opq] = sum;
+        }
+      }
+    }
+  };
+  if constexpr (D6) {
+#pragma unroll
+    for (int q = 0; q < NQ; ++q) flush_d6(q);
+  } else {
+#pragma unroll
+    for (int fi = 0; fi < NS; ++fi)
+#pragma unroll
+      for (int q = 0; q < NQ; ++q) flush_tile(acc[fi][q], q, fi);
+  }
 #ifdef TXM_G_CLOCKS
   if (lane == 0 && (blockIdx.x == 0 || blockIdx.x == 1064)) {
     double *o = a.wtab + a.nwin * I8_WT_STRIDE + ((blockIdx.x ? 1 : 0) * T_WAVES + wave) * 8;
@@ -734,16 +895,17 @@
 #endif
 }
 
-template <int J0, int JN, bool WEIGHTED, bool YS>
+template <int J0, int JN, bool WEIGHTED, bool YS, int MODE = 0>
 static int launch_pass_g(const I8Args &a, int K, const unsigned char *table, int64_t rep_begin, int n_grp, hipStream_t st) {
-  constexpr int NS = JN + (YS ? 1 : 0);
+  constexpr int NS = MODE == 1 ? 3 : JN + (YS ? 1 : 0);
   constexpr int NQ = G_NQ<J0, JN, WEIGHTED, YS>;
+  constexpr int FU = MODE == 2 ? 2688 : G_FU;
   const size_t lds = (size_t)T_WAVES * NS * T_PB + 2 * G_BS * NQ * 1024 + (size_t)(YS ? 2 * G_XR : G_XRB) * T_WAVES * 1024 + 3 * G_RAW +
-                     3 * 2 * G_FU + 32 * NQ * sizeof(uint32_t);
+                     3 * 2 * FU + 32 * NQ * sizeof(uint32_t);
   const dim3 grid((unsigned)(cdiv(a.nwin, 8) * 8 * cdiv(4 * (int64_t)n_grp, NQ)));
   if (a.progress != nullptr) TXM_HIP(hipMemsetAsync(a.progress, 0, (size_t)cdiv(a.nwin, 8) * 8 * 16 * sizeof(uint32_t), st));
-  TXM_SET_MAX_LDS((&resample_i8g_kernel<J0, JN, WEIGHTED, YS>), lds);
-  hipLaunchKernelGGL((resample_i8g_kernel<J0, JN, WEIGHTED, YS>), grid, dim3(T_BLOCK), lds, st, a, K, table, rep_begin, n_grp);
+  TXM_SET_MAX_LDS((&resample_i8g_kernel<J0, JN, WEIGHTED, YS, MODE>), lds);
+  hipLaunchKernelGGL((resample_i8g_kernel<J0, JN, WEIGHTED, YS, MODE>), grid, dim3(T_BLOCK), lds, st, a, K, table, rep_begin, n_grp);
   TXM_LAUNCH_CHECK();
   return TXM_OK;
 }
@@ -759,6 +921,18 @@
 int launch_resample_i8g(const I8Args &a, int K, bool weighted, const unsigned char *table, int64_t rep_begin, int n_grp,
                         hipStream_t st) {
   const bool ys = a.y != nullptr;
+  if (a.plan6 != nullptr) {
+    TXM_REQUIRE(K == 5 && !ys && a.C == I8_CPAD, "resample_i8g: the six-digit plan serves order 4, 32 columns, no second matrix");
+    int rc = weighted ? launch_pass_g<0, 4, true, false, 1>(a, K, table, rep_begin, n_grp, st)
+                      : launch_pass_g<0, 4, false, false, 1>(a, K, table, rep_begin, n_grp, st);
+    if (rc == TXM_OK) rc = weighted ? launch_pass_g<4, 1, true, false, 2>(a, K, table, rep_begin, n_grp, st)
+                                    : launch_pass_g<4, 1, false, false, 2>(a, K, table, rep_begin, n_grp, st);
+    if (rc == TXM_OK) rc = weighted ? launch_pass_g<0, 3, true, false>(a, K, table, rep_begin, n_grp, st)
+                                    : launch_pass_g<0, 3, false, false>(a, K, table, rep_begin, n_grp, st);
+    if (rc == TXM_OK) rc = weighted ? launch_pass_g<3, 2, true, false>(a, K, table, rep_begin, n_grp, st)
+                                    : launch_pass_g<3, 2, false, false>(a, K, table, rep_begin, n_grp, st);
+    return rc;
+  }
   const int rows = K + (ys ? 1 : 0), np = (rows + 2) / 3;
 #ifdef TXM_G_EVEN_SPLIT
   const bool greedy = false;
diff --git a/thermoextrap_amd/engine.py b/thermoextrap_amd/engine.py
--- a/thermoextrap_amd/engine.py
+++ b/thermoextrap_amd/engine.py
@@ -338,7 +338,7 @@
 
 def _call_path(path) -> int:
     eff = path if path is not None else _forced
-    if eff in ("fp64", "int8", "int8_fused", "int8_table"):
+    if eff in ("fp64", "int8", "int8_fused", "int8_table", "int8_table6"):
         return _PATHS[eff]
     return -1
 
@@ -589,12 +589,12 @@
     L = _L()
     if _forced == "fp64":
         return "fp64"
-    if _forced in ("int8", "int8_fused", "int8_table"):
+    if _forced in ("int8", "int8_fused", "int8_table", "int8_table6"):
         return "int8" if L.txm_resample_i8_supported(int(N), int(C), int(nrep), int(order)) == 1 else "fp64"
     return "int8" if L.txm_resample_path(int(N), int(C), int(nrep), int(order)) == 1 else "fp64"
 
 
-_PATHS = {None: -1, "auto": -1, "fp64": 0, "int8": 1, "int8_fused": 2, "int8_table": 3}
+_PATHS = {None: -1, "auto": -1, "fp64": 0, "int8": 1, "int8_fused": 2, "int8_table": 3, "int8_table6": 4}
 _forced: str | None = None
 
 
@@ -619,7 +619,8 @@
         raise RuntimeError("no resample_vals call has been made on this stream")
     v = info.cpu().tolist()
     return {"path": "int8" if v[0] == 1 else "fp64", "windows": int(v[1]), "windows_fp64": int(v[2]),
-            "prep_reused": bool(v[3] & 1), "kernel": ("fp64" if v[0] != 1 else "int8_table" if v[3] & 2 else "int8_fused")}
+            "prep_reused": bool(v[3] & 1), "kernel": ("fp64" if v[0] != 1 else "int8_table" if v[3] & 2 else "int8_fused"),
+            "digits": None if v[0] != 1 else (6 if v[3] & 4 else 7)}
 
 
 def resample_data(data: torch.Tensor, freq: torch.Tensor | None, order: int) -> torch.Tensor:
```

After: 748.9 million samples/s, median of 6. 19.5% higher.
